# szpajder/dumphfdl

Measured on AMD Instinct MI355X. Metric: wideband I/Q Msamples/s (cf32 ingest -> decoded HFDL PDUs) at fixed channel count, higher is better.
Workload: dtype f32

## Files before the change

### dumphfdl_amd/csrc/fft_core.h

```cpp
#pragma once
#include "kernels.h"

namespace hfdl {

__device__ __forceinline__ float2 cmul(float2 a, float2 b)
{
	return make_float2(a.x * b.x - a.y * b.y, a.x * b.y + a.y * b.x);
}

template <int DIR, bool SKEW = false>
__device__ void lds_fft_columns(float2 *s, int R, int logR, int pitch, int log_cols, const float2 *tw)
{
	const int cols_mask = (1 << log_cols) - 1;
	int len = R, loglen = logR;
	while (len >= 4) {
		const int q = len >> 2, logq = loglen - 2;
		const int nb = (R >> 2) << log_cols;
		const int tstep = R >> loglen;
		for (int t = threadIdx.x; t < nb; t += blockDim.x) {
			const int col = t & cols_mask, b = t >> log_cols;
			const int j = b & (q - 1), blk = b >> logq;
			const int r0 = (blk << loglen) + j;
			float2 *p = s + (size_t)r0 * pitch + (SKEW ? 0 : col);
			const int qs = q * pitch;
			const int c0 = SKEW ? ((col + r0) & cols_mask) : 0, c1 = SKEW ? ((col + r0 + q) & cols_mask) : qs;
			const int c2 = SKEW ? (2 * qs + ((col + r0 + 2 * q) & cols_mask)) : 2 * qs, c3 = SKEW ? (3 * qs + ((col + r0 + 3 * q) & cols_mask)) : 3 * qs;
			const int c1s = SKEW ? qs + c1 : c1;
			float2 a = p[c0], bb = p[c1s], c = p[c2], d = p[c3];
			float2 w1 = tw[j * tstep], w2 = tw[2 * j * tstep], w3 = tw[3 * j * tstep];
			if (DIR > 0) { w1.y = -w1.y; w2.y = -w2.y; w3.y = -w3.y; }
			float2 apc = make_float2(a.x + c.x, a.y + c.y), amc = make_float2(a.x - c.x, a.y - c.y);
			float2 bpd = make_float2(bb.x + d.x, bb.y + d.y), bmd = make_float2(bb.x - d.x, bb.y - d.y);
			float2 jb = (DIR < 0) ? make_float2(bmd.y, -bmd.x) : make_float2(-bmd.y, bmd.x);
			float2 y0 = make_float2(apc.x + bpd.x, apc.y + bpd.y);
			float2 y2 = cmul(make_float2(apc.x - bpd.x, apc.y - bpd.y), w2);
			float2 y1 = cmul(make_float2(amc.x + jb.x, amc.y + jb.y), w1);
			float2 y3 = cmul(make_float2(amc.x - jb.x, amc.y - jb.y), w3);
			p[c0] = y0; p[c1s] = y2; p[c2] = y1; p[c3] = y3;
		}
		__syncthreads();
		len = q; loglen = logq;
	}
	if (len == 2) {
		const int nb = (R >> 1) << log_cols;
		for (int t = threadIdx.x; t < nb; t += blockDim.x) {
			const int col = t & cols_mask, b = t >> log_cols;
			float2 *p = s + (size_t)(2 * b) * pitch + (SKEW ? 0 : col);
			const int c0 = SKEW ? ((col + 2 * b) & cols_mask) : 0, c1 = pitch + (SKEW ? ((col + 2 * b + 1) & cols_mask) : 0);
			float2 a = p[c0], bb = p[c1];
			p[c0] = make_float2(a.x + bb.x, a.y + bb.y);
			p[c1] = make_float2(a.x - bb.x, a.y - bb.y);
		}
		__syncthreads();
	}
}

__device__ __forceinline__ int bitrev(int x, int bits) { return bits ? (int)(__brev((unsigned)x) >> (32 - bits)) : 0; }

__device__ __forceinline__ float2 unit_twiddle(unsigned e, int logn)
{
	float frac = (float)e * __builtin_ldexpf(1.0f, -logn + 1);
	float sn, cs;
	sincospif(-frac, &sn, &cs);
	return make_float2(cs, sn);
}

__device__ __forceinline__ void nco_phasor_step(float &cphi, float &sphi, float cd, float sd)
{
#pragma clang fp contract(off)
	const float c0 = cphi, s0 = sphi;
	cphi = c0 * cd - s0 * sd;
	sphi = s0 * cd + c0 * sd;
}

__device__ __forceinline__ float2 nco_phasor_seed(float starting_phase)
{
	return make_float2((float)cos((double)starting_phase), (float)sin((double)starting_phase));
}

__device__ __forceinline__ int nco_output_count(const NcoState &st, int input_size, int q)
{
	return st.decimation_remain < input_size ? (input_size - st.decimation_remain + q - 1) / q : 0;
}

__device__ __forceinline__ void nco_advance(NcoState &st, int cnt, int q, int input_size, float rate)
{
	const int last = st.decimation_remain + q * cnt;
	st.decimation_remain = last - input_size;
	const double phase = (double)st.starting_phase + (double)rate * M_PI * (double)cnt;
	float fp = (float)phase;
	while ((double)fp > M_PI) fp = (float)((double)fp - 2 * M_PI);
	while ((double)fp < -M_PI) fp = (float)((double)fp + 2 * M_PI);
	st.starting_phase = fp;
	st.output_size = cnt;
}

__device__ __forceinline__ void nco_table_segment(const NcoJob &job, int c)
{
	if (c >= job.nch) return;
	const ChanConst k = job.cc[c];
	NcoState st = job.chain[c];
	if (job.seg == 0) job.snap[c] = st;
	const int cnt = nco_output_count(st, job.post_input_size, job.post);
	const int per = (job.outs + job.nseg - 1) / job.nseg;
	const int i0 = job.seg * per, i1 = (job.seg + 1) * per < cnt ? (job.seg + 1) * per : cnt;
	float2 p = job.seg == 0 ? nco_phasor_seed(st.starting_phase) : job.cont[c];
	float2 *dst = job.ph + (size_t)i0 * job.nch + c;
	for (int i = i0; i < i1; i++, dst += job.nch) {
		*dst = p;
		nco_phasor_step(p.x, p.y, k.nco_cosdelta, k.nco_sindelta);
	}
	job.cont[c] = p;
	if (job.seg == job.nseg - 1) {
		nco_advance(st, cnt, job.post, job.post_input_size, k.nco_rate);
		job.chain[c] = st;
	}
}

}
```

### dumphfdl_amd/csrc/fft_kernels.hip

```cpp
#include <hip/hip_ext.h>
#include "kernels.h"
#include "retune_launch.h"
#include "fft_core.h"
#include "fft_regs.h"

namespace hfdl {

template <int FMT>
__device__ __forceinline__ float2 load_sample(const void *__restrict__ raw, int i)
{
	if (FMT == SFMT_CS16) {
		const short2 v = ((const short2 *)raw)[i];
		return make_float2((float)v.x / 32767.5f, (float)v.y / 32767.5f);
	} else if (FMT == SFMT_CU8) {
		const uchar2 v = ((const uchar2 *)raw)[i];
		return make_float2(((float)v.x - 63.5f) / 127.0f, ((float)v.y - 63.5f) / 127.0f);
	}
	return ((const float2 *)raw)[i];
}

__device__ __forceinline__ void store_out(float2 *out, const FftOutLayout &lay, unsigned i, size_t at, float2 v)
{
	if (lay.kind == TAPL_PLAIN) { out[at] = v; return; }
	float *o = (float *)out + tap_index_f(lay.kind, 1 << lay.row_log, (size_t)(2 * lay.row_stride), lay.chan, (int)(i >> lay.row_log), (int)(i & ((1u << lay.row_log) - 1u)), 0);
	o[0] = v.x;
	o[4] = v.y;
}

template <int FMT>
__global__ __launch_bounds__(FFT_THREADS) void fft_pass1(const float2 *__restrict__ hist, FftInputs in,
		int split, float2 *__restrict__ hist_next, float2 *__restrict__ out, FftPlan p, NcoJob job, int riders)
{
	if ((int)blockIdx.x < riders) { if (blockIdx.y == 0) nco_table_segment(job, (int)blockIdx.x * FFT_THREADS + (int)threadIdx.x); return; }
	const int bid = (int)blockIdx.x - riders;
	const int rx = (int)blockIdx.y;
	const void *__restrict__ fresh = in.fresh[rx];
	if (hist != nullptr) hist += rx * in.hist_stride;
	if (hist_next != nullptr) hist_next += rx * in.hist_stride;
	out += (size_t)rx * (size_t)p.n;
	extern __shared__ float2 sm[];
	const int cs = p.n >> p.l1;
	const int c0 = bid * FFT_TILE;
	const int total = p.r1 * FFT_TILE;
	for (int e = threadIdx.x; e < total; e += FFT_THREADS) {
		const int r = e >> FFT_TILE_LOG, col = e & (FFT_TILE - 1);
		const int c = c0 + col;
		float2 v = make_float2(0.f, 0.f);
		if (c < cs) {
			const int idx = r * cs + c;
			v = idx < split ? hist[idx] : load_sample<FMT>(fresh, idx - split);
			if (hist_next != nullptr && idx >= p.n - split) hist_next[idx - (p.n - split)] = v;
		}
		sm[e] = v;
	}
	float2 *ltw = sm + total;
	for (int t = threadIdx.x; t < p.r1; t += FFT_THREADS) ltw[t] = p.tw1[t];
	__syncthreads();
	lds_fft_columns<-1>(sm, p.r1, p.l1, FFT_TILE, FFT_TILE_LOG, ltw);
	for (int e = threadIdx.x; e < total; e += FFT_THREADS) {
		const int k1 = e >> FFT_TILE_LOG, col = e & (FFT_TILE - 1);
		const int c = c0 + col;
		if (c >= cs) continue;
		float2 v = sm[bitrev(k1, p.l1) * FFT_TILE + col];
		const unsigned ex = ((unsigned)k1 * (unsigned)c) & (unsigned)(p.n - 1);
		out[(size_t)k1 * cs + c] = cmul(v, unit_twiddle(ex, p.logn));
	}
}

__global__ __launch_bounds__(FFT_THREADS) void fft_pass2(float2 *__restrict__ buf, FftPlan p, NcoJob job, int riders)
{
	if ((int)blockIdx.x < riders) { if (blockIdx.y == 0) nco_table_segment(job, (int)blockIdx.x * FFT_THREADS + (int)threadIdx.x); return; }
	const int bid = (int)blockIdx.x - riders;
	buf += (size_t)blockIdx.y * (size_t)p.n;
	extern __shared__ float2 sm[];
	const int r23 = p.n >> p.l1, ncol = p.r1 * p.r3;
	const int cc0 = bid * FFT_TILE;
	const int total = p.r2 * FFT_TILE;
	for (int e = threadIdx.x; e < total; e += FFT_THREADS) {
		const int r = e >> FFT_TILE_LOG, col = e & (FFT_TILE - 1);
		const int cc = cc0 + col;
		float2 v = make_float2(0.f, 0.f);
		if (cc < ncol) {
			const int k1 = cc >> p.l3, n3 = cc & (p.r3 - 1);
			v = buf[(size_t)k1 * r23 + (size_t)r * p.r3 + n3];
		}
		sm[e] = v;
	}
	float2 *ltw = sm + total;
	for (int t = threadIdx.x; t < p.r2; t += FFT_THREADS) ltw[t] = p.tw2[t];
	__syncthreads();
	lds_fft_columns<-1>(sm, p.r2, p.l2, FFT_TILE, FFT_TILE_LOG, ltw);
	for (int e = threadIdx.x; e < total; e += FFT_THREADS) {
		const int k2 = e >> FFT_TILE_LOG, col = e & (FFT_TILE - 1);
		const int cc = cc0 + col;
		if (cc >= ncol) continue;
		const int k1 = cc >> p.l3, n3 = cc & (p.r3 - 1);
		float2 v = sm[bitrev(k2, p.l2) * FFT_TILE + col];
		const unsigned ex = ((unsigned)k2 * (unsigned)n3) & (unsigned)(r23 - 1);
		buf[(size_t)k1 * r23 + (size_t)k2 * p.r3 + n3] = cmul(v, unit_twiddle(ex, p.l2 + p.l3));
	}
}

__global__ __launch_bounds__(FFT_THREADS) void fft_pass3(const float2 *__restrict__ in, float2 *__restrict__ out, FftPlan p, int shifted,
		FftOutLayout lay, NcoJob job, int riders, int64_t out_rx_stride)
{
	if ((int)blockIdx.x < riders) { if (blockIdx.y == 0) nco_table_segment(job, (int)blockIdx.x * FFT_THREADS + (int)threadIdx.x); return; }
	const int bid = (int)blockIdx.x - riders;
	in += (size_t)blockIdx.y * (size_t)p.n;
	out += blockIdx.y * out_rx_stride;
	extern __shared__ float2 sm[];
	const int r23 = p.n >> p.l1, ncol = p.r1 * p.r2;
	const int cc0 = bid * FFT_TILE;
	const int total = p.r3 * FFT_TILE;
	for (int e = threadIdx.x; e < total; e += FFT_THREADS) {
		const int col = e >> p.l3, n3 = e & (p.r3 - 1);
		const int cc = cc0 + col;
		float2 v = make_float2(0.f, 0.f);
		if (cc < ncol) {
			const int k2 = cc >> p.l1, k1 = cc & (p.r1 - 1);
			v = in[(size_t)k1 * r23 + (size_t)k2 * p.r3 + n3];
		}
		sm[n3 * FFT_TILE + ((col + n3) & (FFT_TILE - 1))] = v;
	}
	float2 *ltw = sm + total;
	for (int t = threadIdx.x; t < p.r3; t += FFT_THREADS) ltw[t] = p.tw3[t];
	__syncthreads();
	lds_fft_columns<-1, true>(sm, p.r3, p.l3, FFT_TILE, FFT_TILE_LOG, ltw);
	const unsigned half = shifted ? (unsigned)(p.n >> 1) : 0u;
	for (int e = threadIdx.x; e < total; e += FFT_THREADS) {
		const int k3 = e >> FFT_TILE_LOG, col = e & (FFT_TILE - 1);
		const int cc = cc0 + col;
		if (cc >= ncol) continue;
		const int k2 = cc >> p.l1, k1 = cc & (p.r1 - 1);
		const unsigned k = (unsigned)k1 + ((unsigned)k2 << p.l1) + ((unsigned)k3 << (p.l1 + p.l2));
		const unsigned i = (k + half) & (unsigned)(p.n - 1);
		const size_t at = lay.row_log ? (size_t)(i >> lay.row_log) * (size_t)lay.row_stride + (i & ((1u << lay.row_log) - 1u)) : (size_t)i;
		const int r = bitrev(k3, p.l3);
		store_out(out, lay, i, at, sm[r * FFT_TILE + ((col + r) & (FFT_TILE - 1))]);
	}
}


template <int B, int FMT, bool AHEAD>
__global__ __launch_bounds__(16 * B) void fft_rpass1(const float2 *__restrict__ hist, FftInputs in,
		int split, float2 *__restrict__ hist_next, float2 *__restrict__ out, FftPlan p, NcoJob job, int riders, int tpw)
{
	constexpr int NT = 16 * B;
	if ((int)blockIdx.x < riders) { if (blockIdx.y == 0) nco_table_segment(job, (int)blockIdx.x * NT + (int)threadIdx.x); return; }
	const int rx = (int)blockIdx.y;
	const void *__restrict__ fresh = in.fresh[rx];
	if (hist != nullptr) hist += rx * in.hist_stride;
	if (hist_next != nullptr) hist_next += rx * in.hist_stride;
	out += (size_t)rx * (size_t)p.n;
	__shared__ float2 ex[B * FR_PITCH];
	__shared__ float2 ltw[16 * B];
	const int bid = ((int)blockIdx.x - riders) * tpw, tid = (int)threadIdx.x;
	const int cs = p.n >> p.l1;
	const int col = tid & 15, n2 = tid >> 4;
	float2 x[16], xn[16];
	auto load = [&](float2 (&v)[16], int tile) {
		const int c = tile * 16 + col;
#pragma unroll
		for (int n1 = 0; n1 < 16; n1++) {
			const int idx = (n2 + B * n1) * cs + c;
			v[n1] = idx < split ? hist[idx] : load_sample<FMT>(fresh, idx - split);
		}
	};
	load(x, bid);
	ltw[tid] = p.tw1[tid];
	for (int t = 0; t < (AHEAD ? tpw : 1); t++) {
		const int tile = bid + t;
		if (AHEAD && t + 1 < tpw) load(xn, tile + 1);
		if (hist_next != nullptr) {
			const int c = tile * 16 + col;
#pragma unroll
			for (int n1 = 0; n1 < 16; n1++) {
				const int idx = (n2 + B * n1) * cs + c;
				if (idx >= p.n - split) hist_next[idx - (p.n - split)] = x[n1];
			}
		}
		__syncthreads();
		stage_a(x, ex, ltw, n2, col);
		__syncthreads();
#pragma unroll
		for (int i = 0; i < 256 / NT; i++) {
			const int tt = tid + i * NT, tcol = tt & 15, k1 = tt >> 4, tc = tile * 16 + tcol;
			float2 z[B], w[B];
			stage_b<B>(z, ex, k1, tcol);
			twiddle_run<B>(w, (unsigned)k1 * (unsigned)tc, 16u * (unsigned)tc, p.logn);
#pragma unroll
			for (int k2 = 0; k2 < B; k2++) out[(size_t)(k1 + 16 * k2) * cs + tc] = cmul(z[slot_small<B>(k2)], w[k2]);
		}
		if (AHEAD) {
#pragma unroll
			for (int n1 = 0; n1 < 16; n1++) x[n1] = xn[n1];
		}
	}
}

template <int B, bool AHEAD>
__global__ __launch_bounds__(16 * B) void fft_rpass2(float2 *__restrict__ buf, FftPlan p, NcoJob job, int riders, int tpw)
{
	constexpr int NT = 16 * B;
	if ((int)blockIdx.x < riders) { if (blockIdx.y == 0) nco_table_segment(job, (int)blockIdx.x * NT + (int)threadIdx.x); return; }
	buf += (size_t)blockIdx.y * (size_t)p.n;
	__shared__ float2 ex[B * FR_PITCH];
	__shared__ float2 ltw[16 * B];
	const int bid = ((int)blockIdx.x - riders) * tpw, tid = (int)threadIdx.x;
	const int r23 = p.n >> p.l1;
	const int col = tid & 15, n2 = tid >> 4;
	auto base_of = [&](int tile) {
		const int cc0 = tile * 16;
		return buf + (size_t)(cc0 >> p.l3) * r23 + (cc0 & (p.r3 - 1));
	};
	float2 x[16], xn[16];
	auto load = [&](float2 (&v)[16], int tile) {
		const float2 *base = base_of(tile);
#pragma unroll
		for (int n1 = 0; n1 < 16; n1++) v[n1] = base[(size_t)(n2 + B * n1) * p.r3 + col];
	};
	load(x, bid);
	ltw[tid] = p.tw2[tid];
	for (int t = 0; t < (AHEAD ? tpw : 1); t++) {
		const int tile = bid + t;
		if (AHEAD && t + 1 < tpw) load(xn, tile + 1);
		float2 *base = base_of(tile);
		const int n30 = (tile * 16) & (p.r3 - 1);
		__syncthreads();
		stage_a(x, ex, ltw, n2, col);
		__syncthreads();
#pragma unroll
		for (int i = 0; i < 256 / NT; i++) {
			const int tt = tid + i * NT, tcol = tt & 15, k1 = tt >> 4, n3 = n30 + tcol;
			float2 z[B], w[B];
			stage_b<B>(z, ex, k1, tcol);
			twiddle_run<B>(w, (unsigned)k1 * (unsigned)n3, 16u * (unsigned)n3, p.l2 + p.l3);
#pragma unroll
			for (int k2 = 0; k2 < B; k2++) base[(size_t)(k1 + 16 * k2) * p.r3 + tcol] = cmul(z[slot_small<B>(k2)], w[k2]);
		}
		if (AHEAD) {
#pragma unroll
			for (int n1 = 0; n1 < 16; n1++) x[n1] = xn[n1];
		}
	}
}

template <int B>
__global__ __launch_bounds__(16 * B) void fft_rpass3(const float2 *__restrict__ in, float2 *__restrict__ out, FftPlan p, int shifted,
		FftOutLayout lay, NcoJob job, int riders, int tpw, int64_t out_rx_stride)
{
	constexpr int NT = 16 * B, R = 16 * B;
	if ((int)blockIdx.x < riders) { if (blockIdx.y == 0) nco_table_segment(job, (int)blockIdx.x * NT + (int)threadIdx.x); return; }
	in += (size_t)blockIdx.y * (size_t)p.n;
	out += blockIdx.y * out_rx_stride;
	__shared__ float2 ex[B * FR_PITCH];
	__shared__ float2 ltw[16 * B];
	const int bid = ((int)blockIdx.x - riders) * tpw, tid = (int)threadIdx.x;
	const int r23 = p.n >> p.l1;
	const int col = tid & 15, n2 = tid >> 4;
	float2 pre[16], pn[16];
	auto load = [&](float2 (&v)[16], int tile) {
		const int cc0 = tile * 16;
		const float2 *src = in + (size_t)(cc0 >> p.l1) * R + (size_t)(cc0 & (p.r1 - 1)) * r23;
#pragma unroll
		for (int i = 0; i < 16; i++) {
			const int e = tid + i * NT;
			v[i] = src[(size_t)(e / R) * r23 + (e % R)];
		}
	};
	load(pre, bid);
	ltw[tid] = p.tw3[tid];
	const unsigned half = shifted ? (unsigned)(p.n >> 1) : 0u;
	for (int t = 0; t < tpw; t++) {
		const int tile = bid + t;
		const int k2g = (tile * 16) >> p.l1, k10 = (tile * 16) & (p.r1 - 1);
		__syncthreads();
#pragma unroll
		for (int i = 0; i < 16; i++) {
			const int e = tid + i * NT, tcol = e / R, n3 = e % R;
			ex[n3 * 16 + ((tcol + n3) & 15)] = pre[i];
		}
		if (t + 1 < tpw) load(pn, tile + 1);
		__syncthreads();
		float2 x[16];
#pragma unroll
		for (int n1 = 0; n1 < 16; n1++) {
			const int r = n2 + B * n1;
			x[n1] = ex[r * 16 + ((col + r) & 15)];
		}
		__syncthreads();
		stage_a(x, ex, ltw, n2, col);
		__syncthreads();
#pragma unroll
		for (int i = 0; i < 256 / NT; i++) {
			const int tt = tid + i * NT, tcol = tt & 15, ka = tt >> 4;
			float2 z[B];
			stage_b<B>(z, ex, ka, tcol);
			const unsigned kbase = (unsigned)(k10 + tcol) + ((unsigned)k2g << p.l1);
#pragma unroll
			for (int kb = 0; kb < B; kb++) {
				const unsigned k = kbase + ((unsigned)(ka + 16 * kb) << (p.l1 + p.l2));
				const unsigned i2 = (k + half) & (unsigned)(p.n - 1);
				const size_t at = lay.row_log ? (size_t)(i2 >> lay.row_log) * (size_t)lay.row_stride + (i2 & ((1u << lay.row_log) - 1u)) : (size_t)i2;
				store_out(out, lay, i2, at, z[slot_small<B>(kb)]);
			}
		}
#pragma unroll
		for (int i = 0; i < 16; i++) pre[i] = pn[i];
	}
}

template <int B>
static void launch_rpass1(int fmt, dim3 grid, hipStream_t st, hipEvent_t start, hipEvent_t input_read, const float2 *hist, const FftInputs &in, int split, float2 *hist_next,
		float2 *work, const FftPlan &p, const NcoJob &nco, int riders, int tpw)
{
	const dim3 blk(16 * B);
	if (fmt == SFMT_CS16) hipExtLaunchKernelGGL((fft_rpass1<B, SFMT_CS16, false>), grid, blk, 0, st, start, input_read, 0, hist, in, split, hist_next, work, p, nco, riders, tpw);
	else if (fmt == SFMT_CU8) hipExtLaunchKernelGGL((fft_rpass1<B, SFMT_CU8, false>), grid, blk, 0, st, start, input_read, 0, hist, in, split, hist_next, work, p, nco, riders, tpw);
	else hipExtLaunchKernelGGL((fft_rpass1<B, SFMT_CF32, false>), grid, blk, 0, st, start, input_read, 0, hist, in, split, hist_next, work, p, nco, riders, tpw);
}

__global__ void retune_channelizer_kernel(ChanConst *cc, NcoState *chain, float2 *cont, int c, ChanConst k)
{
	if (blockIdx.x != 0 || threadIdx.x != 0) return;
	cc[c] = k;
	chain[c] = NcoState{ 0, 0.f, 0, 0 };
	cont[c] = make_float2(0.f, 0.f);
}

void launch_retune_channelizer(ChanConst *cc, NcoState *chain, float2 *cont, int c, const ChanConst &k, hipStream_t st, hipEvent_t done)
{
	hipExtLaunchKernelGGL(retune_channelizer_kernel, dim3(1), dim3(64), 0, st, nullptr, done, 0, cc, chain, cont, c, k);
}

static bool fast_plan(const FftPlan &p) { return p.l1 >= 6 && p.l1 <= 8 && p.l2 >= 6 && p.l2 <= 8 && p.l3 >= 6 && p.l3 <= 8; }

void launch_fft_forward(const FftPlan &p, const float2 *hist, const FftInputs &in, int fmt, int split, float2 *hist_next,
		float2 *work, float2 *out, bool shifted, hipStream_t st, FftOutLayout lay, hipEvent_t done, NcoJob nco, hipEvent_t input_read, hipEvent_t start)
{
	const unsigned nrx = (unsigned)in.nrx;
	const int64_t ors = in.out_stride;
	const int c1 = (p.n >> p.l1), c2 = p.r1 * p.r3, c3 = p.r1 * p.r2;
	const int g1 = (c1 + FFT_TILE - 1) / FFT_TILE, g2 = (c2 + FFT_TILE - 1) / FFT_TILE, g3 = (c3 + FFT_TILE - 1) / FFT_TILE;
	nco.nseg = 3;
	if (fast_plan(p)) {
		auto riders_of = [&](int l) { const int nt = 1 << l; return nco.cc ? (nco.nch + nt - 1) / nt : 0; };
		const int rd1 = riders_of(p.l1), rd2 = riders_of(p.l2), rd3 = riders_of(p.l3);
		auto tpw_of = [](int tiles) { return tiles % 4 == 0 && tiles >= 4096 ? 4 : tiles % 2 == 0 && tiles >= 1024 ? 2 : 1; };
		const int t1 = 1, t2 = 1, t3 = tpw_of(g3);
		nco.seg = 0;
		switch (p.l1) {
		case 6: launch_rpass1<4>(fmt, dim3(g1 / t1 + rd1, nrx), st, start, input_read, hist, in, split, hist_next, work, p, nco, rd1, t1); break;
		case 7: launch_rpass1<8>(fmt, dim3(g1 / t1 + rd1, nrx), st, start, input_read, hist, in, split, hist_next, work, p, nco, rd1, t1); break;
		default: launch_rpass1<16>(fmt, dim3(g1 / t1 + rd1, nrx), st, start, input_read, hist, in, split, hist_next, work, p, nco, rd1, t1); break;
		}
		nco.seg = 1;
		switch (p.l2) {
		case 6: hipLaunchKernelGGL((fft_rpass2<4, false>), dim3(g2 / t2 + rd2, nrx), dim3(64), 0, st, work, p, nco, rd2, t2); break;
		case 7: hipLaunchKernelGGL((fft_rpass2<8, false>), dim3(g2 / t2 + rd2, nrx), dim3(128), 0, st, work, p, nco, rd2, t2); break;
		default: hipLaunchKernelGGL((fft_rpass2<16, false>), dim3(g2 / t2 + rd2, nrx), dim3(256), 0, st, work, p, nco, rd2, t2); break;
		}
		nco.seg = 2;
		switch (p.l3) {
		case 6: hipExtLaunchKernelGGL(fft_rpass3<4>, dim3(g3 / t3 + rd3, nrx), dim3(64), 0, st, nullptr, done, 0, (const float2 *)work, out, p, shifted ? 1 : 0, lay, nco, rd3, t3, ors); break;
		case 7: hipExtLaunchKernelGGL(fft_rpass3<8>, dim3(g3 / t3 + rd3, nrx), dim3(128), 0, st, nullptr, done, 0, (const float2 *)work, out, p, shifted ? 1 : 0, lay, nco, rd3, t3, ors); break;
		default: hipExtLaunchKernelGGL(fft_rpass3<16>, dim3(g3 / t3 + rd3, nrx), dim3(256), 0, st, nullptr, done, 0, (const float2 *)work, out, p, shifted ? 1 : 0, lay, nco, rd3, t3, ors); break;
		}
		return;
	}
	const int riders = nco.cc ? (nco.nch + FFT_THREADS - 1) / FFT_THREADS : 0;
	const dim3 blk(FFT_THREADS);
	const size_t l1 = (size_t)p.r1 * (FFT_TILE + 1) * sizeof(float2), l2 = (size_t)p.r2 * (FFT_TILE + 1) * sizeof(float2);
	nco.seg = 0;
	if (fmt == SFMT_CS16) hipExtLaunchKernelGGL(fft_pass1<SFMT_CS16>, dim3(g1 + riders, nrx), blk, l1, st, start, input_read, 0, hist, in, split, hist_next, work, p, nco, riders);
	else if (fmt == SFMT_CU8) hipExtLaunchKernelGGL(fft_pass1<SFMT_CU8>, dim3(g1 + riders, nrx), blk, l1, st, start, input_read, 0, hist, in, split, hist_next, work, p, nco, riders);
	else hipExtLaunchKernelGGL(fft_pass1<SFMT_CF32>, dim3(g1 + riders, nrx), blk, l1, st, start, input_read, 0, hist, in, split, hist_next, work, p, nco, riders);
	nco.seg = 1;
	hipLaunchKernelGGL(fft_pass2, dim3(g2 + riders, nrx), blk, l2, st, work, p, nco, riders);
	nco.seg = 2;
	hipExtLaunchKernelGGL(fft_pass3, dim3(g3 + riders, nrx), blk, (size_t)p.r3 * (FFT_TILE + 1) * sizeof(float2), st, nullptr, done, 0,
			(const float2 *)work, out, p, shifted ? 1 : 0, lay, nco, riders, ors);
}

}
```

### dumphfdl_amd/csrc/fft_regs.h

```cpp
#pragma once
#include "kernels.h"
#include "fft_core.h"

namespace hfdl {

constexpr int FR_PITCH = 16 * 16 + 16;

__device__ __forceinline__ float2 cadd(float2 a, float2 b) { return make_float2(a.x + b.x, a.y + b.y); }
__device__ __forceinline__ float2 csub(float2 a, float2 b) { return make_float2(a.x - b.x, a.y - b.y); }
__device__ __forceinline__ float2 mul_mj(float2 a) { return make_float2(a.y, -a.x); }

__device__ __forceinline__ void dft4(float2 &a, float2 &b, float2 &c, float2 &d)
{
	const float2 t0 = cadd(a, c), t1 = csub(a, c), t2 = cadd(b, d), t3 = mul_mj(csub(b, d));
	a = cadd(t0, t2); c = csub(t0, t2);
	b = cadd(t1, t3); d = csub(t1, t3);
}

__device__ __forceinline__ void dft16(float2 (&x)[16])
{
	constexpr float C1 = 0.92387953251128674f, S1 = 0.38268343236508977f, H = 0.70710678118654752f;
#pragma unroll
	for (int b = 0; b < 4; b++) dft4(x[b], x[4 + b], x[8 + b], x[12 + b]);
	x[5] = cmul(x[5], make_float2(C1, -S1));  x[6] = cmul(x[6], make_float2(H, -H));    x[7] = cmul(x[7], make_float2(S1, -C1));
	x[9] = cmul(x[9], make_float2(H, -H));    x[10] = mul_mj(x[10]);                     x[11] = cmul(x[11], make_float2(-H, -H));
	x[13] = cmul(x[13], make_float2(S1, -C1)); x[14] = cmul(x[14], make_float2(-H, -H)); x[15] = cmul(x[15], make_float2(-C1, S1));
#pragma unroll
	for (int c = 0; c < 4; c++) dft4(x[4 * c], x[4 * c + 1], x[4 * c + 2], x[4 * c + 3]);
}
__device__ __forceinline__ constexpr int slot16(int k) { return 4 * (k & 3) + (k >> 2); }

__device__ __forceinline__ void dft8(float2 (&x)[8])
{
	constexpr float H = 0.70710678118654752f;
#pragma unroll
	for (int b = 0; b < 4; b++) { const float2 s = cadd(x[b], x[4 + b]), d = csub(x[b], x[4 + b]); x[b] = s; x[4 + b] = d; }
	x[5] = cmul(x[5], make_float2(H, -H)); x[6] = mul_mj(x[6]); x[7] = cmul(x[7], make_float2(-H, -H));
	dft4(x[0], x[1], x[2], x[3]);
	dft4(x[4], x[5], x[6], x[7]);
}
__device__ __forceinline__ constexpr int slot8(int k) { return 4 * (k & 1) + (k >> 1); }

template <int B> __device__ __forceinline__ void dft_small(float2 (&z)[B])
{
	if constexpr (B == 16) dft16(z);
	else if constexpr (B == 8) dft8(z);
	else { static_assert(B == 4, "B = 4, 8 or 16"); dft4(z[0], z[1], z[2], z[3]); }
}
template <int B> __device__ __forceinline__ constexpr int slot_small(int k) { return B == 16 ? slot16(k) : B == 8 ? slot8(k) : k; }

__device__ __forceinline__ void stage_a(float2 (&x)[16], float2 *ex, const float2 *ltw, int n2, int col)
{
	dft16(x);
	float2 *dst = ex + n2 * FR_PITCH + col;
	dst[0] = x[0];
#pragma unroll
	for (int k1 = 1; k1 < 16; k1++) dst[k1 * 16] = cmul(x[slot16(k1)], ltw[n2 * k1]);
}

template <int B> __device__ __forceinline__ void stage_b(float2 (&z)[B], const float2 *ex, int k1, int col)
{
	const float2 *src = ex + k1 * 16 + col;
#pragma unroll
	for (int n2 = 0; n2 < B; n2++) z[n2] = src[n2 * FR_PITCH];
	dft_small<B>(z);
}

template <int B> __device__ __forceinline__ void twiddle_run(float2 (&w)[B], unsigned e0, unsigned es, int logn)
{
	const unsigned mask = (1u << logn) - 1u;
	const float2 base = unit_twiddle(e0 & mask, logn), s1 = unit_twiddle(es & mask, logn);
	const float2 s2 = cmul(s1, s1), s3 = cmul(s2, s1);
	float2 s4 = make_float2(1.f, 0.f);
	if constexpr (B > 4) s4 = unit_twiddle((4u * es) & mask, logn);
	float2 q = base;
#pragma unroll
	for (int g = 0; g < B / 4; g++) {
		if (g > 0) q = cmul(q, s4);
		w[4 * g] = q; w[4 * g + 1] = cmul(q, s1); w[4 * g + 2] = cmul(q, s2); w[4 * g + 3] = cmul(q, s3);
	}
}

}
```

### dumphfdl_amd/csrc/fold_kernels.hip

```cpp
#include <hip/hip_ext.h>
#include <type_traits>
#include "kernels.h"
#include "fft_core.h"

namespace hfdl {

constexpr int FOLD_THREADS = 256;

typedef float v4f __attribute__((ext_vector_type(4)));
typedef float v2f __attribute__((ext_vector_type(2)));


__device__ __forceinline__ float2 tap_at(const float *taps, size_t row_stride_f, int m, int layout, int c, int row, int j)
{
	const float *p = taps + tap_index_f(layout, m, row_stride_f, c, row, j, 0);
	return make_float2(p[0], p[layout == TAPL_PLAIN ? 1 : 4]);
}

__device__ __forceinline__ void cmac_quad(float2 &a, const float2 *h, const float2 *x, int n)
{
	for (int k = 0; k < n; k++) { a.x = __builtin_fmaf(h[k].x, x[k].x, a.x); a.y = __builtin_fmaf(h[k].y, x[k].x, a.y); }
	for (int k = 0; k < n; k++) { a.x = __builtin_fmaf(-h[k].y, x[k].y, a.x); a.y = __builtin_fmaf(h[k].x, x[k].y, a.y); }
}

__device__ __forceinline__ int rx_of_channel(const int4 *__restrict__ rx_tab, int nrx, int c)
{
	int r = 0;
	while (r + 1 < nrx && c >= rx_tab[r + 1].z) r++;
	return r;
}

__global__ __launch_bounds__(FOLD_THREADS) void fold_ref_kernel(const float *__restrict__ taps, const float2 *__restrict__ spec, float2 *__restrict__ partial,
		size_t row_stride_f, size_t spec_stride, size_t partial_stride, int m, int slices, int rows, int layout, int nb,
		const int4 *__restrict__ rx_tab, int nrx, size_t spec_rx_stride)
{
	const int s = blockIdx.x % slices, c = blockIdx.x / slices;
	const int rxi = rx_of_channel(rx_tab, nrx, c);
	const int4 rt = rx_tab[rxi];
	const int slot = rt.x + (c - rt.z);
	spec += (size_t)rxi * spec_rx_stride;
	for (int b0 = 0; b0 < nb; b0 += 4)
		for (int j = threadIdx.x; j < m; j += FOLD_THREADS) {
			const float2 *sp = spec + (size_t)b0 * spec_stride + (size_t)s * rows * (size_t)m + j;
			float2 acc[4] = { make_float2(0.f, 0.f), make_float2(0.f, 0.f), make_float2(0.f, 0.f), make_float2(0.f, 0.f) };
			for (int r = 0; r < rows; r += 4) {
				const int n = rows - r < 4 ? rows - r : 4;
				float2 h[4], x[4];
				for (int k = 0; k < n; k++) h[k] = tap_at(taps, row_stride_f, m, layout, slot, s * rows + r + k, j);
#pragma unroll
				for (int b = 0; b < 4; b++)
					if (b0 + b < nb) {
						for (int k = 0; k < n; k++) x[k] = sp[(size_t)b * spec_stride + (size_t)(r + k) * m];
						cmac_quad(acc[b], h, x, n);
					}
			}
#pragma unroll
			for (int k = 0; k < 4; k++)
				if (b0 + k < nb) partial[(size_t)(b0 + k) * partial_stride + ((size_t)c * slices + s) * (size_t)m + j] = acc[k];
		}
}

__device__ __forceinline__ float rot90(float a, int sign_mask)
{
	const int v = __builtin_amdgcn_update_dpp(0, __float_as_int(a), 0xB1, 0xF, 0xF, true);
	return __int_as_float(v ^ sign_mask);
}

#ifdef HFDL_LAB
__device__ unsigned long long hfdl_fold_clk_probe[1024 * 4];
__device__ unsigned hfdl_fold_clk_probe_n;
#endif

constexpr int fold16_waves(int p, int w, int d, bool small = false, int cg = 1)
{
	const int loads = 8 * cg, mine = w >= loads ? 1 : loads / w;
	const int regs = (small ? 16 : 64) * p * cg + 16 * p * d + 4 * mine * d + 4 * mine + 8 + 28;
	if (small) return regs <= 168 ? 2 : 1;
	if (cg > 1) return 1;
	return regs <= 96 ? 5 : regs <= 128 ? 4 : regs <= 168 ? 3 : regs <= 256 ? 2 : 1;
}

template <int P, int W, int D, bool WIN = false, bool SMALL = false, int CG = 1>
__device__ __forceinline__ void fold_mfma16_body(
		const float *__restrict__ taps, const float2 *__restrict__ spec, float2 *__restrict__ partial,
		size_t row_stride_f, size_t spec_stride, size_t partial_stride, int m, int slices, int rows, int nb,
		const int2 *__restrict__ win, const int4 *__restrict__ grp_tab, size_t spec_rx_stride)
{
	static_assert(!WIN || W == 1, "windows are per wave: no spectrum tile is shared");
	static_assert(D == 2 || D == 4, "the LDS stage of a trip is a compile-time constant for even D");
	static_assert(CG == 1 || (CG == 2 && !SMALL && !WIN), "two column groups: the sixteen-column instruction, every row");
#ifdef HFDL_LAB
	unsigned long long clk_c0 = 0, clk_r0 = 0;
	const bool clk_me = blockIdx.x == gridDim.x / 2 && threadIdx.x == 0;
	if (clk_me) { clk_c0 = __builtin_amdgcn_s_memtime(); clk_r0 = __builtin_amdgcn_s_memrealtime(); }
#endif
	constexpr int NLOADS = 8 * CG;
	constexpr int MINE = W >= NLOADS ? 1 : NLOADS / W;
	constexpr int XPITCH = 64 * CG + 1;
	__shared__ v4f xt[2][8][XPITCH];
	const int ngrp = m >> 4;
	const int ntile = ngrp * slices, groups = (int)gridDim.x / ntile;
	int tile_id, grp;
	if ((ntile & 7) == 0) {
		const int xcd = (int)blockIdx.x & 7, i = (int)blockIdx.x >> 3;
		grp = i % groups;
		tile_id = (i / groups) * 8 + xcd;
	} else {
		tile_id = (int)blockIdx.x % ntile;
		grp = (int)blockIdx.x / ntile;
	}
	const int g = tile_id % ngrp, s = tile_id / ngrp;
	const int wave = __builtin_amdgcn_readfirstlane((int)(threadIdx.x >> 6)), lane = (int)(threadIdx.x & 63);
	const int n = lane & 15, k = lane >> 4;
	const int4 ge = grp_tab[grp];
	const int octet0 = __builtin_amdgcn_readfirstlane(ge.x) + wave * P;
	const int slot_end = __builtin_amdgcn_readfirstlane(ge.z), to_chan = __builtin_amdgcn_readfirstlane(ge.w);
	spec += (size_t)__builtin_amdgcn_readfirstlane(ge.y) * spec_rx_stride;
	const int sign_mask = (lane & 1) ? 0 : (int)0x80000000;
	const int quads = rows >> 2;
	int next_quad = 0, trips = quads;
	if constexpr (WIN) {
		const int2 wn = win[octet0 / P];
		next_quad = __builtin_amdgcn_readfirstlane(wn.x);
		trips = __builtin_amdgcn_readfirstlane(wn.y);
	}
	const char *tb = (const char *)(taps + (size_t)s * rows * row_stride_f + (size_t)octet0 * 64 * m + (size_t)g * 1024) + lane * 16;
	const size_t qs_b = row_stride_f * 16, os_b = (size_t)m * 256, xquad_b = (size_t)m * 32;
	const char *xp[MINE], *xp0[MINE];
	int xseg[MINE];
#pragma unroll
	for (int i = 0; i < MINE; i++) {
		const int item = (((wave * MINE) % NLOADS) + i) * 64 + lane, seg = item >> 3, part = item & 7;
		const int sn = (seg & 15) + 16 * (seg >> 6), sk = (seg >> 4) & 3;
		const int bi = sn < nb ? sn : nb - 1;
		xp[i] = xp0[i] = (const char *)(spec + (size_t)bi * spec_stride + ((size_t)s * rows + sk) * (size_t)m + g * 16 + 2 * part);
		xseg[i] = part * XPITCH + seg;
	}
	const char *const tb0 = tb;
	constexpr int NACC = SMALL ? 4 : 16;
	v4f acc[P * CG][NACC];
#pragma unroll
	for (int p = 0; p < P * CG; p++)
#pragma unroll
		for (int j = 0; j < NACC; j++) acc[p][j] = v4f{ 0.f, 0.f, 0.f, 0.f };
	v4f h[D][P][4];
	v4f xs[D][MINE];
	auto issue = [&](int slot) {
		if constexpr (WIN) {
			tb = tb0 + (size_t)next_quad * qs_b;
#pragma unroll
			for (int i = 0; i < MINE; i++) xp[i] = xp0[i] + (size_t)next_quad * xquad_b;
			next_quad = next_quad + 1 == quads ? 0 : next_quad + 1;
		}
#pragma unroll
		for (int i = 0; i < MINE; i++) xs[slot][i] = *(const v4f *)xp[i];
#pragma unroll
		for (int p = 0; p < P; p++)
#pragma unroll
			for (int q = 0; q < 4; q++) h[slot][p][q] = __builtin_nontemporal_load((const v4f *)(tb + (size_t)p * os_b + 1024 * q));
		if constexpr (!WIN) {
#pragma unroll
			for (int i = 0; i < MINE; i++) xp[i] += xquad_b;
			tb += qs_b;
		}
	};
	auto stash = [&](int slot, int stage) {
#pragma unroll
		for (int i = 0; i < MINE; i++) (&xt[stage][0][0])[xseg[i]] = xs[slot][i];
	};
	auto multiply = [&](int slot, int stage) {
		if constexpr (SMALL) {
			const float *xl = (const float *)&xt[stage][0][0] + (size_t)((k >> 1) * XPITCH + (lane & 3)) * 4 + 2 * (k & 1);
#pragma unroll
			for (int q = 0; q < 4; q++) {
				v2f x[4];
#pragma unroll
				for (int kk = 0; kk < 4; kk++) x[kk] = *(const v2f *)(xl + (size_t)(2 * q * XPITCH + 16 * kk) * 4);
#pragma unroll
				for (int p = 0; p < P; p++) {
					typedef unsigned v2u __attribute__((ext_vector_type(2)));
					const v4f hv = h[slot][p][q];
					const v2u a02 = __builtin_amdgcn_permlane32_swap(__float_as_uint(hv[0]), __float_as_uint(hv[2]), false, false);
					const v2u a13 = __builtin_amdgcn_permlane32_swap(__float_as_uint(hv[1]), __float_as_uint(hv[3]), false, false);
					const v2u t01 = __builtin_amdgcn_permlane16_swap(a02[0], a13[0], false, false);
					const v2u t23 = __builtin_amdgcn_permlane16_swap(a02[1], a13[1], false, false);
					const float t[4] = { __uint_as_float(t01[0]), __uint_as_float(t01[1]), __uint_as_float(t23[0]), __uint_as_float(t23[1]) };
#pragma unroll
					for (int kk = 0; kk < 4; kk++) acc[p][q] = __builtin_amdgcn_mfma_f32_4x4x1f32(t[kk], x[kk].x, acc[p][q], 0, 0, 0);
#pragma unroll
					for (int kk = 0; kk < 4; kk++) acc[p][q] = __builtin_amdgcn_mfma_f32_4x4x1f32(rot90(t[kk], sign_mask), x[kk].y, acc[p][q], 0, 0, 0);
				}
			}
			return;
		}
#pragma unroll
		for (int b = 0; b < 8; b++) {
			v4f x[CG];
#pragma unroll
			for (int cg = 0; cg < CG; cg++) x[cg] = xt[stage][b][64 * cg + lane];
#pragma unroll
			for (int p = 0; p < P; p++)
#pragma unroll
				for (int cg = 0; cg < CG; cg++) {
					v4f *a = acc[p * CG + cg];
					a[2 * b] = __builtin_amdgcn_mfma_f32_16x16x4f32(h[slot][p][b >> 1][(2 * b) & 3], x[cg][0], a[2 * b], 0, 0, 0);
					a[2 * b + 1] = __builtin_amdgcn_mfma_f32_16x16x4f32(h[slot][p][b >> 1][(2 * b + 1) & 3], x[cg][2], a[2 * b + 1], 0, 0, 0);
				}
#pragma unroll
			for (int p = 0; p < P; p++) {
				const float r0 = rot90(h[slot][p][b >> 1][(2 * b) & 3], sign_mask), r1 = rot90(h[slot][p][b >> 1][(2 * b + 1) & 3], sign_mask);
#pragma unroll
				for (int cg = 0; cg < CG; cg++) {
					v4f *a = acc[p * CG + cg];
					a[2 * b] = __builtin_amdgcn_mfma_f32_16x16x4f32(r0, x[cg][1], a[2 * b], 0, 0, 0);
					a[2 * b + 1] = __builtin_amdgcn_mfma_f32_16x16x4f32(r1, x[cg][3], a[2 * b + 1], 0, 0, 0);
				}
			}
		}
	};
#pragma unroll
	for (int d = 0; d < D; d++) {
		issue(d);
		__builtin_amdgcn_sched_barrier(0);
	}
	stash(0, 0);
	__syncthreads();
	for (int r = 0; r < trips - D; r += D) {
#pragma unroll
		for (int d = 0; d < D; d++) {
			multiply(d, d & 1);
			issue(d);
			stash((d + 1) % D, (d + 1) & 1);
			__builtin_amdgcn_sched_barrier(0);
			__syncthreads();
		}
	}
#pragma unroll
	for (int d = 0; d < D; d++) {
		multiply(d, d & 1);
		if (d + 1 < D) {
			stash(d + 1, (d + 1) & 1);
			__builtin_amdgcn_sched_barrier(0);
			__syncthreads();
		}
	}
	if constexpr (SMALL) {
		const int j = lane & 3, cpq = (lane >> 2) & 3;
		if (j < nb) {
#pragma unroll
			for (int p = 0; p < P; p++)
#pragma unroll
				for (int cp = 0; cp < 2; cp++) {
					const int sl = 8 * (octet0 + p) + 2 * cpq + cp;
					if (sl >= slot_end) continue;
					const int c = sl + to_chan;
					float2 *po = partial + (size_t)j * partial_stride + ((size_t)c * slices + s) * (size_t)m + g * 16 + k;
#pragma unroll
					for (int q = 0; q < 4; q++) po[4 * q] = make_float2(acc[p][q][2 * cp], acc[p][q][2 * cp + 1]);
				}
		}
	} else
	{
#pragma unroll
		for (int cg = 0; cg < CG; cg++) {
			const int blk = 16 * cg + n;
			if (blk >= nb) continue;
#pragma unroll
			for (int p = 0; p < P; p++)
#pragma unroll
				for (int cp = 0; cp < 2; cp++) {
					const int sl = 8 * (octet0 + p) + 2 * k + cp;
					if (sl >= slot_end) continue;
					const int c = sl + to_chan;
					const v4f *a = acc[p * CG + cg];
					float2 *po = partial + (size_t)blk * partial_stride + ((size_t)c * slices + s) * (size_t)m + g * 16;
#pragma unroll
					for (int j = 0; j < 16; j += 2)
						*(v4f *)(po + j) = v4f{ a[j][2 * cp], a[j][2 * cp + 1], a[j + 1][2 * cp], a[j + 1][2 * cp + 1] };
				}
		}
	}
#ifdef HFDL_LAB
	if (clk_me) {
		const unsigned slot = atomicAdd(&hfdl_fold_clk_probe_n, 1u) & 1023u;
		hfdl_fold_clk_probe[4 * slot] = (SMALL ? 4ull : 16ull * CG) * 100ull + (unsigned long long)nb;
		hfdl_fold_clk_probe[4 * slot + 1] = __builtin_amdgcn_s_memtime() - clk_c0;
		hfdl_fold_clk_probe[4 * slot + 2] = __builtin_amdgcn_s_memrealtime() - clk_r0;
		hfdl_fold_clk_probe[4 * slot + 3] = clk_r0;
	}
#endif
}

template <int P, int W, int D, bool WIN = false, bool SMALL = false, int CG = 1>
__global__ __launch_bounds__(64 * W) __attribute__((amdgpu_waves_per_eu(fold16_waves(P, W, D, SMALL, CG), fold16_waves(P, W, D, SMALL, CG)))) void fold_mfma16_kernel(
		const float *__restrict__ taps, const float2 *__restrict__ spec, float2 *__restrict__ partial,
		size_t row_stride_f, size_t spec_stride, size_t partial_stride, int m, int slices, int rows, int nb,
		const int2 *__restrict__ win, const int4 *__restrict__ grp_tab, size_t spec_rx_stride)
{
	fold_mfma16_body<P, W, D, WIN, SMALL, CG>(taps, spec, partial, row_stride_f, spec_stride, partial_stride, m, slices, rows, nb, win, grp_tab, spec_rx_stride);
}

#ifdef HFDL_LAB
__global__ __launch_bounds__(512) __attribute__((amdgpu_waves_per_eu(2, 2))) __attribute__((amdgpu_num_vgpr(104))) void fold32_two_waves_kernel(
		const float *__restrict__ taps, const float2 *__restrict__ spec, float2 *__restrict__ partial,
		size_t row_stride_f, size_t spec_stride, size_t partial_stride, int m, int slices, int rows, int nb,
		const int2 *__restrict__ win, const int4 *__restrict__ grp_tab, size_t spec_rx_stride)
{
	fold_mfma16_body<1, 8, 2, false, false, 2>(taps, spec, partial, row_stride_f, spec_stride, partial_stride, m, slices, rows, nb, win, grp_tab, spec_rx_stride);
}
#endif

#ifdef HFDL_LAB
template <int L, bool SPAN>
__global__ __launch_bounds__(FOLD_THREADS) void stream_read_kernel(const float4 *__restrict__ src, size_t chunks, float *__restrict__ sink)
{
	float acc = 0.f;
	const size_t per_block = chunks / gridDim.x;
	const size_t first = SPAN ? (size_t)blockIdx.x * per_block : blockIdx.x, step = SPAN ? 1 : gridDim.x;
	const size_t last = SPAN ? first + per_block : chunks;
	for (size_t ch = first; ch < last; ch += step) {
		const v4f *p = (const v4f *)src + ch * (L * FOLD_THREADS) + threadIdx.x;
		v4f v[L];
#pragma unroll
		for (int i = 0; i < L; i++) v[i] = __builtin_nontemporal_load(p + i * FOLD_THREADS);
#pragma unroll
		for (int i = 0; i < L; i++) acc += v[i].x + v[i].w;
	}
	if (acc == 1.2345e33f) *sink = acc;
}

hipError_t fold_clock_probe_ring(ClockProbeRing &r)
{
	r.len = 1024;
	const hipError_t e = hipGetSymbolAddress((void **)&r.records, HIP_SYMBOL(hfdl_fold_clk_probe));
	return e != hipSuccess ? e : hipGetSymbolAddress((void **)&r.count, HIP_SYMBOL(hfdl_fold_clk_probe_n));
}

int stream_read_variants() { return 4; }

void launch_stream_read(int variant, const float2 *src, size_t bytes, float *sink, hipStream_t st)
{
	const dim3 block(FOLD_THREADS);
	switch (variant) {
	case 0: hipLaunchKernelGGL((stream_read_kernel<4, false>), dim3(2048), block, 0, st, (const float4 *)src, bytes / (64 * FOLD_THREADS), sink); break;
	case 1: hipLaunchKernelGGL((stream_read_kernel<8, false>), dim3(2048), block, 0, st, (const float4 *)src, bytes / (128 * FOLD_THREADS), sink); break;
	case 2: hipLaunchKernelGGL((stream_read_kernel<4, true>), dim3((unsigned)(bytes >> 22)), block, 0, st, (const float4 *)src, bytes / (64 * FOLD_THREADS), sink); break;
	default: hipLaunchKernelGGL((stream_read_kernel<8, true>), dim3((unsigned)(bytes >> 22)), block, 0, st, (const float4 *)src, bytes / (128 * FOLD_THREADS), sink); break;
	}
}
#endif

struct FoldArgs {
	const float *taps;
	const float2 *spec;
	float2 *partial;
	size_t rs_f, ss, ps;
	int m, slices, rows, nch, ngroups, nb;
	const int4 *grp_tab, *rx_host;
	int nrx;
	size_t spec_rx_stride;
	void split(int pw, int &groups, int &rest) const
	{
		groups = rest = 0;
		for (int r = 0; r < nrx; r++) { const int noct = rx_host[r].y >> 3; groups += noct / pw; rest += noct % pw; }
	}
	const int4 *table(int pw) const { return grp_tab + (size_t)(pw - 1) * (size_t)(ngroups); }
	hipStream_t st;
	hipEvent_t start, stop;
};

template <int P, int W, int D, bool SMALL = false, int CG = 1>
static int fold16_go(const FoldArgs &a)
{
	static_assert(P * W <= FOLD_GROUP_MAX, "the group tables of the front end go up to FOLD_GROUP_MAX octets per workgroup");
	const int ntile = (a.m >> 4) * a.slices;
	int groups, rest;
	a.split(P * W, groups, rest);
	int launches = 0;
	if (groups > 0) {
		hipExtLaunchKernelGGL((fold_mfma16_kernel<P, W, D, false, SMALL, CG>), dim3((unsigned)(groups * ntile)), dim3(64 * W), 0, a.st, a.start, rest ? nullptr : a.stop, 0,
			a.taps, a.spec, a.partial, a.rs_f, a.ss, a.ps, a.m, a.slices, a.rows, a.nb, (const int2 *)nullptr, a.table(P * W), a.spec_rx_stride);
		launches++;
	}
	if (rest > 0) {
		constexpr int DR = CG > 1 ? 2 : D;
		hipExtLaunchKernelGGL((fold_mfma16_kernel<1, 1, DR, false, SMALL, CG>), dim3((unsigned)(rest * ntile)), dim3(64), 0, a.st, groups > 0 ? nullptr : a.start, a.stop, 0,
			a.taps, a.spec, a.partial, a.rs_f, a.ss, a.ps, a.m, a.slices, a.rows, a.nb, (const int2 *)nullptr, a.table(P * W) + groups, a.spec_rx_stride);
		launches++;
	}
	return launches;
}

#ifdef HFDL_LAB
static int fold32_two_waves_go(const FoldArgs &a)
{
	const int ntile = (a.m >> 4) * a.slices;
	int groups, rest;
	a.split(8, groups, rest);
	int launches = 0;
	if (groups > 0) {
		hipExtLaunchKernelGGL(fold32_two_waves_kernel, dim3((unsigned)(groups * ntile)), dim3(512), 0, a.st, a.start, rest ? nullptr : a.stop, 0,
			a.taps, a.spec, a.partial, a.rs_f, a.ss, a.ps, a.m, a.slices, a.rows, a.nb, (const int2 *)nullptr, a.table(8), a.spec_rx_stride);
		launches++;
	}
	if (rest > 0) {
		hipExtLaunchKernelGGL((fold_mfma16_kernel<1, 1, 2, false, false, 2>), dim3((unsigned)(rest * ntile)), dim3(64), 0, a.st, groups > 0 ? nullptr : a.start, a.stop, 0,
			a.taps, a.spec, a.partial, a.rs_f, a.ss, a.ps, a.m, a.slices, a.rows, a.nb, (const int2 *)nullptr, a.table(8) + groups, a.spec_rx_stride);
		launches++;
	}
	return launches;
}
#endif

template <int D>
static int fold16_go_win(const FoldArgs &a, const int2 *win)
{
	const int ntile = a.m >> 4;
	hipExtLaunchKernelGGL((fold_mfma16_kernel<1, 1, D, true>), dim3((unsigned)(a.ngroups * ntile)), dim3(64), 0, a.st, a.start, a.stop, 0,
		a.taps, a.spec, a.partial, a.rs_f, a.ss, a.ps, a.m, 1, a.rows, a.nb, win, a.table(1), a.spec_rx_stride);
	return 1;
}

struct FoldVariant { int layout, p, q, w, d; int (*go)(const FoldArgs &); };
#define F16(P, W, D) { TAPL_OCTET, P, 4, W, D, fold16_go<P, W, D> }
#define F4(P, W, D) { TAPL_OCTET, P, 1, W, D, fold16_go<P, W, D, true> }
#define F32(P, W, D) { TAPL_OCTET, P, 8, W, D, fold16_go<P, W, D, false, 2> }
static const FoldVariant fold_variants[] = {
	F16(2, 4, 4), F16(2, 4, 2),
	F4(2, 4, 2),
	F32(1, 4, 4), F32(1, 4, 2),
#ifdef HFDL_LAB
	F32(1, 8, 2), F32(1, 8, 4), F32(1, 2, 2), F32(2, 4, 2),
	F4(2, 4, 4), F4(4, 4, 2), F4(1, 8, 4), F4(2, 8, 2), F4(2, 8, 4), F4(4, 2, 2), F4(1, 4, 4),
	F16(1, 4, 2), F16(1, 4, 4), F16(1, 8, 2), F16(1, 8, 4), F16(2, 2, 2), F16(2, 8, 2), F16(1, 2, 2), F16(1, 2, 4), F16(3, 4, 2),
	{ TAPL_OCTET, 1, 8, 8, 2, fold32_two_waves_go },
#endif
};
#undef F32
#undef F4
#undef F16
constexpr int N_FOLD_VARIANTS = (int)(sizeof(fold_variants) / sizeof(fold_variants[0]));

int fold_variant_count() { return N_FOLD_VARIANTS; }

int fold_variant_describe(int v, int desc[6])
{
	if (v < 0 || v >= N_FOLD_VARIANTS) return -1;
	const FoldVariant &f = fold_variants[v];
	desc[0] = f.p; desc[1] = f.q; desc[2] = f.w; desc[3] = f.d; desc[4] = 4 * f.q; desc[5] = f.layout;
	return 0;
}

static bool variant_fits(const FoldVariant &f, const Geometry &g)
{
	return g.tap_layout == f.layout && (g.rows_per_slice & 3) == 0 && (g.rows_per_slice >> 2) % f.d == 0;
}

static const FoldVariant *pick_variant(const Geometry &g, int nb)
{
	if (g.fold_tile >= 0 && g.fold_tile < N_FOLD_VARIANTS && 4 * fold_variants[g.fold_tile].q >= nb && variant_fits(fold_variants[g.fold_tile], g)) return &fold_variants[g.fold_tile];
	for (const FoldVariant &f : fold_variants)
		if (nb <= 4 && f.q == 1 && variant_fits(f, g)) return &f;
	for (const FoldVariant &f : fold_variants)
		if (f.q == (nb <= 16 ? 4 : 8) && variant_fits(f, g)) return &f;
	return nullptr;
}

int fold_launch_blocks(const Geometry &g, int remaining, int nb_max)
{
	int take = remaining < nb_max ? remaining : nb_max;
	if (take > FOLD_MAX_BLOCKS) take = FOLD_MAX_BLOCKS;
	if (take > 16 && g.fold_win && g.tap_layout == TAPL_OCTET) take = 16;
	if (take > 16 && take <= 20) take = 16;
	if (take > 16 && !pick_variant(g, take)) take = 16;
	return take;
}

static FoldArgs fold_args(const Geometry &g, const float2 *taps, const float2 *spectrum, size_t spec_stride, float2 *partial, size_t partial_stride,
		int nb, hipStream_t st, hipEvent_t start, hipEvent_t stop)
{
	FoldArgs a;
	a.taps = (const float *)taps; a.spec = spectrum; a.partial = partial;
	a.rs_f = (size_t)g.tap_row_stride * 2; a.ss = spec_stride; a.ps = partial_stride;
	a.m = g.m; a.slices = g.slices; a.rows = g.rows_per_slice; a.nch = g.nch; a.ngroups = g.nch_pad / tap_layout_group(g.tap_layout); a.nb = nb;
	a.grp_tab = g.grp_tab; a.rx_host = g.rx_host; a.nrx = g.nrx; a.spec_rx_stride = (size_t)g.spec_rx_stride;
	a.st = st; a.start = start; a.stop = stop;
	return a;
}

static void launch_fold_ref(const Geometry &g, const float2 *taps, const float2 *spectrum, size_t spec_stride, float2 *partial, size_t partial_stride,
		int nb, hipStream_t st, hipEvent_t start, hipEvent_t stop)
{
	hipExtLaunchKernelGGL(fold_ref_kernel, dim3((unsigned)(g.nch * g.slices)), dim3(FOLD_THREADS), 0, st, start, stop, 0,
		(const float *)taps, spectrum, partial, (size_t)g.tap_row_stride * 2, spec_stride, partial_stride, g.m, g.slices, g.rows_per_slice, g.tap_layout, nb,
		g.rx_tab, g.nrx, (size_t)g.spec_rx_stride);
}

int launch_fold_variant(int v, const Geometry &g, const float2 *taps, const float2 *spectrum, size_t spec_stride, float2 *partial,
		size_t partial_stride, int nb, hipStream_t st, hipEvent_t start, hipEvent_t stop)
{
	if (v == -1) { launch_fold_ref(g, taps, spectrum, spec_stride, partial, partial_stride, nb, st, start, stop); return 1; }
	if (v < 0 || v >= N_FOLD_VARIANTS || !variant_fits(fold_variants[v], g) || nb < 1 || nb > 4 * fold_variants[v].q) return -1;
	return fold_variants[v].go(fold_args(g, taps, spectrum, spec_stride, partial, partial_stride, nb, st, start, stop));
}

int launch_fold(const Geometry &g, const float2 *taps, const float2 *spectrum, size_t spec_stride, float2 *partial, size_t partial_stride,
		int nb, hipStream_t st, hipEvent_t start, hipEvent_t stop)
{
	if (nb < 1 || nb > fold_launch_blocks(g, nb, FOLD_MAX_BLOCKS)) return -1;
	const FoldArgs a = fold_args(g, taps, spectrum, spec_stride, partial, partial_stride, nb, st, start, stop);
	if (g.fold_win && g.tap_layout == TAPL_OCTET) return fold16_go_win<2>(a, g.fold_win);
	if (const FoldVariant *f = pick_variant(g, nb)) return f->go(a);
	launch_fold_ref(g, taps, spectrum, spec_stride, partial, partial_stride, nb, st, start, stop);
	return 1;
}

__global__ __launch_bounds__(FOLD_THREADS) void tap_row_energy_kernel(const float *__restrict__ taps, float *__restrict__ energy, size_t row_stride_f, int m, int noct, int nch_pad)
{
	const int oct = blockIdx.x % noct, quad = blockIdx.x / noct;
	const v4f *base = (const v4f *)(taps + (size_t)quad * 4 * row_stride_f + (size_t)oct * 64 * m);
	float acc = 0.f;
	for (int e = threadIdx.x; e < (m >> 2) * 64; e += FOLD_THREADS) {
		const v4f v = base[e];
		acc += v.x * v.x + v.y * v.y + v.z * v.z + v.w * v.w;
	}
	const int lane = threadIdx.x & 63;
	atomicAdd(energy + (size_t)(4 * quad + (lane >> 4)) * nch_pad + oct * 8 + ((lane & 15) >> 1), acc);
}

void launch_tap_row_energy(const float2 *taps, const Geometry &g, float *energy, hipStream_t st)
{
	const int noct = g.nch_pad / 8;
	hipLaunchKernelGGL(tap_row_energy_kernel, dim3((unsigned)((g.pre >> 2) * noct)), dim3(FOLD_THREADS), 0, st, (const float *)taps, energy, (size_t)g.tap_row_stride * 2, g.m, noct, g.nch_pad);
}

__global__ __launch_bounds__(FOLD_THREADS) void tap_extract_kernel(const float *__restrict__ taps, float2 *__restrict__ dst, size_t row_stride_f, int m, int pre, int layout, int c)
{
	const size_t n = (size_t)m * pre;
	for (size_t e = (size_t)blockIdx.x * FOLD_THREADS + threadIdx.x; e < n; e += (size_t)gridDim.x * FOLD_THREADS)
		dst[e] = tap_at(taps, row_stride_f, m, layout, c, (int)(e / m), (int)(e % m));
}

void launch_tap_extract(const float2 *taps, const Geometry &g, int slot, float2 *dst, hipStream_t st)
{
	hipLaunchKernelGGL(tap_extract_kernel, dim3(1024), dim3(FOLD_THREADS), 0, st, (const float *)taps, dst, (size_t)g.tap_row_stride * 2, g.m, g.pre, g.tap_layout, slot);
}

constexpr int IFFT_THREADS = 1024;

__device__ __forceinline__ void nco_phasor_run(float2 *ph, int cnt, float starting_phase, float cd, float sd)
{
	float2 p = nco_phasor_seed(starting_phase);
	for (int i = 0; i < cnt; i++) {
		ph[i] = p;
		nco_phasor_step(p.x, p.y, cd, sd);
	}
}

__device__ __forceinline__ float2 nco_rotate(float2 p, float2 v)
{
#pragma clang fp contract(off)
	const float re = p.x * v.x - p.y * v.y, im = p.y * v.x + p.x * v.y;
	return make_float2(re, im);
}

__global__ __launch_bounds__(IFFT_THREADS) void ifft_nco_kernel(const float2 *__restrict__ partial, size_t partial_stride, const ChanConst *__restrict__ cc,
		const NcoState *__restrict__ snap, const float2 *__restrict__ ph, size_t ph_stride, const float2 *__restrict__ tw, float2 *__restrict__ chan_out,
		int *__restrict__ out_count, Geometry g, int logm)
{
	extern __shared__ float2 sm[];
	const int c = blockIdx.x % g.nch, b = blockIdx.x / g.nch;
	const ChanConst k = cc[c];
	const int m = g.m, mask = m - 1;
	const NcoState st = snap[(size_t)b * g.nch + c];
	const int q = g.post;
	const int cnt = nco_output_count(st, g.post_input_size, q);
	{
		const int h0 = (int)(((long long)g.n - k.offsetbin + m / 2) % m);
		const float2 *pc = partial + (size_t)b * partial_stride + (size_t)c * g.slices * (size_t)m;
		for (int u = threadIdx.x; u < m; u += IFFT_THREADS) {
			const int j = (u - h0 - m / 2) & mask;
			float2 acc = make_float2(0.f, 0.f);
			for (int s = 0; s < g.slices; s++) {
				float2 v = pc[(size_t)s * m + j];
				acc.x += v.x; acc.y += v.y;
			}
			sm[u] = acc;
		}
	}
	__syncthreads();
	lds_fft_columns<+1>(sm, m, logm, 1, 0, tw);

	const float norm = (float)g.pre * (float)m;
	float2 *o = chan_out + ((size_t)b * g.nch + c) * g.outs;
	const float2 *phb = ph + (size_t)b * ph_stride;
	for (int i = threadIdx.x; i < cnt; i += IFFT_THREADS) {
		const int idx = g.scrap + st.decimation_remain + q * i;
		float2 v = sm[(int)(__brev((unsigned)idx) >> (32 - logm))];
		v.x = __fdiv_rn(v.x, norm); v.y = __fdiv_rn(v.y, norm);
		o[i] = nco_rotate(phb[(size_t)i * g.nch + c], v);
	}
	if (threadIdx.x == 0) out_count[(size_t)b * g.nch + c] = cnt;
}

__global__ __launch_bounds__(IFFT_THREADS) void nco_decimate_kernel(const float2 *__restrict__ in, int input_size, float cd, float sd, float rate,
		int q, NcoState *__restrict__ state, float2 *__restrict__ ph, float2 *__restrict__ out)
{
	NcoState st = *state;
	const int cnt = nco_output_count(st, input_size, q);
	if (threadIdx.x == 0) nco_phasor_run(ph, cnt, st.starting_phase, cd, sd);
	__syncthreads();
	for (int i = threadIdx.x; i < cnt; i += IFFT_THREADS) out[i] = nco_rotate(ph[i], in[st.decimation_remain + q * i]);
	__syncthreads();
	if (threadIdx.x == 0) {
		nco_advance(st, cnt, q, input_size, rate);
		*state = st;
	}
}

void launch_nco_decimate(const float2 *in, int input_size, float cd, float sd, float rate, int q, NcoState *state, float2 *ph, float2 *out, hipStream_t st)
{
	hipLaunchKernelGGL(nco_decimate_kernel, dim3(1), dim3(IFFT_THREADS), 0, st, in, input_size, cd, sd, rate, q, state, ph, out);
}

hipError_t prepare_ifft_nco(int m)
{
	const size_t lds = sizeof(float2) * ((size_t)m + 1);
	if (lds <= 64 * 1024) return hipSuccess;
	return hipFuncSetAttribute((const void *)ifft_nco_kernel, hipFuncAttributeMaxDynamicSharedMemorySize, (int)lds);
}

void launch_ifft_nco(const Geometry &g, const float2 *partial, size_t partial_stride, const ChanConst *cc, const NcoState *snap, const float2 *ph,
		size_t ph_stride, const float2 *tw_m, float2 *chan_out, int *out_count, int nb, hipStream_t st, hipEvent_t done, hipEvent_t start)
{
	int logm = 0;
	while ((1 << logm) < g.m) logm++;
	size_t lds = sizeof(float2) * ((size_t)g.m + 1);
	hipExtLaunchKernelGGL(ifft_nco_kernel, dim3((unsigned)(g.nch * nb)), dim3(IFFT_THREADS), (unsigned)lds, st, start, done, 0, partial, partial_stride, cc, snap, ph, ph_stride,
			tw_m, chan_out, out_count, g, logm);
}

}
```

### dumphfdl_amd/csrc/frontend.h

```cpp
#pragma once
#include <hip/hip_runtime.h>
#include <complex>
#include <deque>
#include <memory>
#include <vector>
#include "../../include/hfdl_gpu.h"
#include "hip_handles.h"
#include "kernels.h"
#include "planner.h"
#include "retune_launch.h"
#include "launch_timers.h"
#include "demod.h"
#include "spectrum.h"
#include "export_ring.h"
#include "blanker.h"
#include "notch.h"

namespace hfdl {

int select_device(int device);
int check_channel_span(int32_t sample_rate, int32_t nrx, int c, int32_t freq, int r, int32_t centre);
long env_long(const char *name, long lo, long hi, long otherwise);
inline int ilog2(int x) { int l = 0; while ((1 << l) < x) l++; return l; }
inline size_t sample_bytes(int fmt) { return fmt == SFMT_CS16 ? 4 : fmt == SFMT_CU8 ? 2 : 8; }
bool is_library_pinned(const void *p, size_t bytes);

struct LabConfig {
	int fold_tile = -1;
	int fold_slices = 0;
	int cu_split = 0;
	bool cu_partition = false;
	int fft_stream = -1;
	bool decode_stream = true;
	int fold_bound = -1;
	bool fold_ramp = true;
};
LabConfig read_lab_config();

struct HostFftPlan {
	FftPlan p{};
	DevBuf tw[3];
	int build(int n);
};
int upload_twiddles(int r, DevBuf &out);

int finish_stage();
struct StageFrames {
	DevBuf frames, data, scrambler;
	int upload(const float *symbols, const int32_t *modes, const int32_t *bitmask_lsb, int32_t nframes);
};


struct SpectrumHistory {
	static constexpr int CHUNK = 8;
	int rows = 0, interval = 0;
	DevBuf acc, peak;
	PinnedBuf<float> host;
	std::vector<Event> ev;
	std::vector<hfdl_gpu_spectrum_row> info;
	uint64_t open = 0;
	uint64_t open_first = 0;
	uint32_t open_blocks = 0;
	uint64_t oldest() const { const uint64_t kept = (uint64_t)rows - (open_blocks ? 1 : 0); return open > kept ? open - kept : 0; }
	void close()
	{
		info[open % (uint64_t)rows] = hfdl_gpu_spectrum_row{ open, open_first, open_blocks, 0 };
		open++;
		open_blocks = 0;
	}
};

struct SpectrumMonitor {
	int bins = 0;
	uint32_t flags = 0;
	DevBuf acc;
	DevBuf peak;
	PinnedBuf<float> host;
	Event ev;
	hipEvent_t last = nullptr;
	hipEvent_t newest() const { return last ? last : ev.e; }
	uint64_t fresh = 0;
	std::vector<uint64_t> blocks, first;
	std::unique_ptr<SpectrumHistory> hist;
};

struct ChannelExport {
	int nsel = 0, format = 0;
	float scale = 1.f;
	ExportRing ring;
	DevBuf channels;
	DevBuf samples, counts, power, clipped;
	size_t chunk = 1;
	PinnedBuf<char> host;
	std::vector<Event> ev;
	std::vector<uint64_t> last_of;
	hipEvent_t newest = nullptr;
};

struct Blanker {
	float k2 = 0.f;
	DevBuf scratch;
	DevBuf partial;
	DevBuf rec;
	PinnedBuf<BlankRecord> host;
	Event ev;
	uint64_t blocks = 0;
};

struct Notch {
	float mu = 0.f;
	int nsel = 0;
	std::vector<bool> selected;
	DevBuf out;
	DevBuf sel;
	DevBuf state;
	DevBuf rec;
	PinnedBuf<NotchRecord> host;
	PinnedBuf<int32_t> host_sel;
	Event staged;
	bool staging = false;
	Event ev;
	bool launched = false;
};

struct Retune {
	DevBuf pad, work;
	PinnedBuf<float2> stage[2];
	Event staged[2];
	DoneEvent done;
	uint64_t calls = 0;
	std::vector<float> lp;
	float lp_cut = -1.f;
};

}

bool design_channel(const hfdl_gpu_frontend *fe, int rx, int32_t freq, hfdl::ChanConst &k, std::complex<float> *taps, std::vector<float> &lp, float &lp_cut);

struct hfdl_gpu_frontend {
	int device = 0;
	hfdl::Stream stream;
	hfdl::Stream stream_b;
	hfdl::Stream stream_d;
	hfdl::Stream stream_c;
	hfdl::Stream stream_f;
	bool cu_partitioned = false;
	bool own_decode_stream() const { return stream_d.owned; }
	hfdl::FftRule fft_rule = hfdl::FFT_RULE_INPUT;
	hfdl::FftOrder order;
	int side_of(bool on_device) const { return hfdl::fft_side(fft_rule, on_device); }
	hipStream_t fft_stream(int side) const { return side == hfdl::FFT_SERIAL ? stream.s : stream_f.owned ? stream_f.s : stream_c.s; }
	static constexpr int MAX_HALF = hfdl::FOLD_MAX_BLOCKS;
	static constexpr int MAX_STAGE = HFDL_GPU_PREFETCH_MAX + 1;
	static_assert(MAX_HALF == hfdl::PLAN_MAX_HALF && MAX_STAGE == hfdl::PLAN_MAX_STAGE && HFDL_GPU_FOLD_BATCH_MAX == MAX_HALF, "include/hfdl_gpu.h, kernels.h and planner.h name the same limits");

	std::deque<hfdl::DevBuf> mem;
	template <typename T> hipError_t alloc(T *&view, size_t count)
	{
		mem.emplace_back();
		const hipError_t e = mem.back().alloc(sizeof(T) * count);
		view = mem.back().as<T>();
		return e;
	}
	hfdl::HostFftPlan fft;
	hfdl::Demod demod;
	int4 *d_rx = nullptr, *d_grp = nullptr;
	float2 *d_hist[2] = { nullptr, nullptr }, *d_work = nullptr, *d_spec = nullptr, *d_taps = nullptr, *d_partial = nullptr;
	float2 *d_tw_m = nullptr;
	int n_stage = 0;
	std::unique_ptr<hfdl::DevBuf> d_stage[MAX_STAGE];
	size_t stage_cap[MAX_STAGE] = {};
	float2 *d_chan_all = nullptr;
	int *d_cnt_all = nullptr;
	hfdl::ChanConst *d_cc = nullptr;
	int2 *d_win = nullptr;
	hfdl::NcoState *d_nco = nullptr;
	hfdl::NcoState *d_nco_snap = nullptr;
	float2 *d_ph = nullptr, *d_ph_cont = nullptr;
	std::unique_ptr<hfdl::SpectrumMonitor> mon;
	std::unique_ptr<hfdl::ChannelExport> exp;
	std::unique_ptr<hfdl::Retune> retune;
	std::unique_ptr<hfdl::Blanker> blank;
	std::unique_ptr<hfdl::Notch> notch;

	hfdl::DoneEvent chan[2];
	hfdl::DoneEvent fft_done;
	hfdl::DoneEvent spec[2];
	hfdl::Event ev_switch;
	hfdl::Event ev_stage_ready[MAX_STAGE];
	hfdl::Event ev_stage_free[MAX_STAGE];
	hfdl::LaunchTimers timers;
	int settle_events();

	uint64_t host_blocks = 0;
	uint64_t host_pushed = 0;
	const void *pf_ptr[MAX_STAGE] = {};
	int pf_fmt[MAX_STAGE] = {};
	hipEvent_t input_event(uint64_t host_block) const
	{
		const uint64_t newest = host_blocks - 1, span = (uint64_t)n_stage - 1;
		return ev_stage_ready[(newest - host_block <= span ? host_block : newest - span) % (uint64_t)n_stage];
	}
	int32_t sample_rate = 0, decimation = 0;
	float tbw = 0;
	hfdl::Plan plan{};
	hfdl::Geometry geo{};
	std::vector<int32_t> freqs;
	int nrx = 1;
	std::vector<int32_t> rx_center;
	std::vector<int32_t> rx_of;
	std::vector<hfdl::RxSpan> rx_span;
	std::vector<int4> rx_host;
	int slot_of(int c) const { return hfdl::receiver_slot(rx_span[(size_t)rx_of[(size_t)c]], c); }
	std::vector<hfdl::ChanConst> cc;
	int batch = 1;
	int fold_nb = 1;
	int half_blocks = 1;
	int half_first = 1, half_target = 1;
	int cur_half = 0, batch_fill = 0;
	int last_slot = 0;
	int last_index = 0;
	float2 *chan_slot(int slot) const { return d_chan_all + (size_t)slot * (size_t)geo.nch * (size_t)geo.outs; }
	int *cnt_slot(int slot) const { return d_cnt_all + (size_t)slot * (size_t)geo.nch; }
	int last_set = 0;
	float2 *spec_slot(int set, int i) const { return d_spec + ((size_t)set * (size_t)half_blocks + (size_t)i) * spec_stride(); }
	size_t spec_stride() const { return (size_t)nrx * (size_t)geo.n; }
	float2 *ph_slot(int set, int i) const { return d_ph + ((size_t)set * (size_t)half_blocks + (size_t)i) * ph_stride(); }
	hfdl::NcoState *snap_slot(int set, int i) const { return d_nco_snap + ((size_t)set * (size_t)half_blocks + (size_t)i) * (size_t)geo.nch; }
	size_t partial_stride() const { return (size_t)geo.nch * (size_t)geo.slices * (size_t)geo.m; }
	size_t ph_stride() const { return (size_t)geo.nch * (size_t)geo.outs; }
	double prune_tol = 0.0;
	int fold_rows_max = 0;
	bool fold_bound = false;
	uint64_t blocks = 0;
	hfdl::FftOutLayout tap_layout;
	int pending_demod_buf = -1;
	int pending_demod_nblk = 0;

	~hfdl_gpu_frontend();
};
```

### dumphfdl_amd/csrc/frontend_create.cpp

```cpp
#include <atomic>
#include <cmath>
#include <complex>
#include <cstring>
#include <thread>
#include "frontend.h"

using namespace hfdl;

extern "C" int hfdl_gpu_device_count(void)
{
	int n = 0;
	if (hipGetDeviceCount(&n) != hipSuccess) return 0;
	return n;
}

int hfdl::select_device(int device)
{
	int n = 0;
	if (hipGetDeviceCount(&n) != hipSuccess || n <= 0)
		return fail(HFDL_GPU_ENODEV, "no HIP device visible: the HFDL front end has no CPU fallback");
	if (device < 0 || device >= n) return fail(HFDL_GPU_EINVAL, "device %d out of range (%d visible)", device, n);
	HIP_TRY(hipSetDevice(device));
	hipDeviceProp_t prop;
	HIP_TRY(hipGetDeviceProperties(&prop, device));
	if (strncmp(prop.gcnArchName, "gfx950", 6) != 0)
		return fail(HFDL_GPU_ENODEV, "device %d is %s; this library carries gfx950 code only", device, prop.gcnArchName);
	return 0;
}


int hfdl::upload_twiddles(int r, DevBuf &out)
{
	std::vector<float2> h((size_t)r);
	for (int t = 0; t < r; t++) {
		double a = -2.0 * M_PI * (double)t / (double)r;
		h[t] = make_float2((float)std::cos(a), (float)std::sin(a));
	}
	HIP_TRY(out.alloc(sizeof(float2) * (size_t)r));
	HIP_TRY(hipMemcpy(out.p, h.data(), sizeof(float2) * (size_t)r, hipMemcpyHostToDevice));
	return 0;
}

int HostFftPlan::build(int n)
{
	int logn = ilog2(n);
	if ((1 << logn) != n || logn < 9 || logn > 24) return fail(HFDL_GPU_ERANGE, "fft size %d unsupported (need 2^9..2^24)", n);
	int l1 = (logn + 2) / 3, l2 = (logn - l1 + 1) / 2, l3 = logn - l1 - l2;
	p.n = n; p.logn = logn;
	p.l1 = l1; p.l2 = l2; p.l3 = l3;
	p.r1 = 1 << l1; p.r2 = 1 << l2; p.r3 = 1 << l3;
	const int radix[3] = { p.r1, p.r2, p.r3 };
	for (int i = 0; i < 3; i++) if (int rc = upload_twiddles(radix[i], tw[i])) return rc;
	p.tw1 = tw[0].as<float2>(); p.tw2 = tw[1].as<float2>(); p.tw3 = tw[2].as<float2>();
	return 0;
}


long hfdl::env_long(const char *name, long lo, long hi, long otherwise)
{
	const char *e = getenv(name);
	if (!e || !*e) return otherwise;
	char *end = nullptr;
	const long v = strtol(e, &end, 10);
	return (end != e && v >= lo && v <= hi) ? v : otherwise;
}

static double env_double(const char *name, double lo, double hi, double otherwise)
{
	const char *e = getenv(name);
	if (!e || !*e) return otherwise;
	char *end = nullptr;
	const double v = strtod(e, &end);
	return (end != e && v >= lo && v <= hi) ? v : otherwise;
}

static int build_fold_windows(hfdl_gpu_frontend *fe)
{
	Geometry &g = fe->geo;
	DevBuf d_en;
	std::vector<float> en((size_t)g.pre * (size_t)g.nch_pad);
	HIP_TRY(d_en.alloc(sizeof(float) * en.size()));
	HIP_TRY(hipMemsetAsync(d_en.p, 0, sizeof(float) * en.size(), fe->stream));
	launch_tap_row_energy(fe->d_taps, g, d_en.as<float>(), fe->stream);
	HIP_TRY(hipMemcpyAsync(en.data(), d_en.p, sizeof(float) * en.size(), hipMemcpyDeviceToHost, fe->stream));
	HIP_TRY(hipStreamSynchronize(fe->stream));
	const std::vector<RowWindow> w = fold_row_windows(en, g.pre, g.nch_pad, g.nch, fe->prune_tol, &fe->fold_rows_max);
	static_assert(sizeof(RowWindow) == sizeof(int2), "a window is what the fold kernels load as an int2 { first quad, count }");
	HIP_TRY(fe->alloc(fe->d_win, w.size()));
	HIP_TRY(hipMemcpy(fe->d_win, w.data(), sizeof(int2) * w.size(), hipMemcpyHostToDevice));
	g.fold_win = fe->d_win;
	return 0;
}

bool design_channel(const hfdl_gpu_frontend *fe, int rx, int32_t freq, ChanConst &k, std::complex<float> *taps, std::vector<float> &lp, float &lp_cut)
{
	float shift = (float)(fe->rx_center[(size_t)rx] - (freq + 1440)) / (float)fe->sample_rate;
	Plan cp;
	if (!plan_block(cp, fe->tbw, fe->decimation, shift)) return false;
	k = ChanConst{};
	k.offsetbin = cp.offsetbin;
	k.nco_sindelta = cp.sindelta; k.nco_cosdelta = cp.cosdelta; k.nco_rate = cp.rate;
	k.frequency = freq;
	if (taps == nullptr) return true;
	float half_bw = 0.5f / fe->decimation;
	design_bandpass(taps, fe->plan.taps_length, (-shift) - half_bw, (-shift) + half_bw, lp, lp_cut);
	return true;
}

static int build_taps(hfdl_gpu_frontend *fe)
{
	const Plan &pl = fe->plan;
	const int nch = (int)fe->freqs.size();
	const size_t n = (size_t)pl.n;
	std::vector<std::complex<float>> host((size_t)nch * (size_t)pl.taps_length);
	fe->cc.resize((size_t)nch);
	unsigned nthreads = std::max(1u, std::min((unsigned)nch, std::thread::hardware_concurrency()));
	nthreads = std::min(nthreads, (unsigned)env_long("HFDL_GPU_HOST_THREADS", 1, 1 << 16, (long)nthreads));
	std::atomic<int> next{0};
	std::atomic<int> bad{0};
	auto work = [&]() {
		std::vector<float> lp;
		float lp_cut = -1.f;
		for (;;) {
			int c = next.fetch_add(1);
			if (c >= nch) break;
			if (!design_channel(fe, fe->rx_of[(size_t)c], fe->freqs[c], fe->cc[c], host.data() + (size_t)c * pl.taps_length, lp, lp_cut)) bad++;
		}
	};
	std::vector<std::thread> pool;
	for (unsigned t = 1; t < nthreads; t++) pool.emplace_back(work);
	work();
	for (auto &t : pool) t.join();
	if (bad) return fail(HFDL_GPU_EINVAL, "fastddc planning failed for %d channel(s)", (int)bad);

	DevBuf pad;
	HIP_TRY(pad.alloc(sizeof(float2) * n));
	float2 *d_pad = pad.as<float2>();
	HIP_TRY(hipMemsetAsync(d_pad, 0, sizeof(float2) * n, fe->stream));
	if (fe->geo.nch_pad > nch)
		HIP_TRY(hipMemsetAsync(fe->d_taps, 0, sizeof(float2) * n * (size_t)fe->geo.nch_pad, fe->stream));
	for (int c = 0; c < nch; c++) {
		HIP_TRY(hipMemcpyAsync(d_pad, host.data() + (size_t)c * pl.taps_length, sizeof(float2) * (size_t)pl.taps_length,
				hipMemcpyHostToDevice, fe->stream));
		const int slot = fe->slot_of(c);
		FftOutLayout lay = fe->tap_layout;
		lay.chan = slot;
		float2 *dst = lay.kind == TAPL_PLAIN ? fe->d_taps + (size_t)slot * (size_t)fe->geo.tap_chan_stride : fe->d_taps;
		launch_fft_forward(fe->fft.p, nullptr, d_pad, SFMT_CF32, 0, nullptr, fe->d_work, dst, true, fe->stream, lay);
	}
	HIP_TRY(hipStreamSynchronize(fe->stream));
	HIP_TRY(hipGetLastError());
	return 0;
}

int hfdl::check_channel_span(int32_t sample_rate, int32_t nrx, int c, int32_t freq, int r, int32_t centre)
{
	if (std::abs((int64_t)centre - freq) < sample_rate / 2) return 0;
	return nrx == 1 ? fail(HFDL_GPU_EINVAL, "channel %d Hz outside +-fs/2 of centre %d", freq, centre)
	                : fail(HFDL_GPU_EINVAL, "channel %d (%d Hz) outside +-fs/2 of the centre %d of its receiver %d", c, freq, centre, r);
}

static int check_create_args(hfdl_gpu_frontend **out, int32_t sample_rate, int32_t nrx, const int32_t *centerfreqs, const int32_t *freqs,
		const int32_t *nch_per_rx)
{
	if (!out || !centerfreqs || !freqs || !nch_per_rx) return fail(HFDL_GPU_EINVAL, "bad arguments: null pointer");
	*out = nullptr;
	if (nrx < 1 || nrx > HFDL_GPU_RECEIVERS_MAX) return fail(HFDL_GPU_EINVAL, "bad arguments: %d receivers (1 .. %d)", nrx, HFDL_GPU_RECEIVERS_MAX);
	for (int r = 0; r < nrx; r++)
		if (nch_per_rx[r] <= 0) return fail(HFDL_GPU_EINVAL, "bad arguments: receiver %d has %d channels", r, nch_per_rx[r]);
	if (sample_rate < 5400) return fail(HFDL_GPU_EINVAL, "sample rate must be >= 5400 (src/main.c:638-641)");
	for (int r = 0, c = 0; r < nrx; r++)
		for (int i = 0; i < nch_per_rx[r]; i++, c++)
			if (int rc = check_channel_span(sample_rate, nrx, c, freqs[c], r, centerfreqs[r])) return rc;
	return 0;
}

extern "C" int hfdl_gpu_frontend_create(hfdl_gpu_frontend **out, int device, int32_t sample_rate, int32_t centerfreq,
		const int32_t *freqs, int32_t nch)
{
	if (!out || !freqs || nch <= 0) return fail(HFDL_GPU_EINVAL, "bad arguments");
	return hfdl_gpu_frontend_create_multi(out, device, sample_rate, 1, &centerfreq, freqs, &nch);
}

static int create_streams(hfdl_gpu_frontend *fe, const LabConfig &lab)
{
	CuPartition part = plan_cu_partition((int)fe->freqs.size(), Demod::workgroup_lds(), fe->fold_bound);
	if (!lab.cu_partition || lab.cu_split) part.on = false;
	if (part.on) {
		const hipError_t ea = fe->stream.create_on_cus(part.mask_fold), eb = fe->stream_b.create_on_cus(part.mask_demod);
		if (ea != hipSuccess || eb != hipSuccess) {
			fe->stream.reset(); fe->stream_b.reset();
			(void)hipGetLastError();
			(void)fail(0, "CU-masked streams refused (%s): the demodulators share the fold's CUs", hipGetErrorString(ea != hipSuccess ? ea : eb));
			part.on = false;
		}
	}
	fe->cu_partitioned = part.on;
	if (part.on) {
	} else if (lab.cu_split) {
		uint32_t mask_a[8] = {}, mask_b[8] = {};
		for (int i = 0; i < 256; i++)
			((((i >> 3) + i) % lab.cu_split) == 0 ? mask_b : mask_a)[i >> 5] |= 1u << (i & 31);
		CREATE_TRY(fe->stream.create_on_cus(mask_a));
		CREATE_TRY(fe->stream_b.create_on_cus(mask_b));
	} else {
		CREATE_TRY(fe->stream.create());
		CREATE_TRY(fe->stream_b.create());
	}
	if (lab.decode_stream) CREATE_TRY(fe->stream_d.create());
	else fe->stream_d.alias(fe->stream_b);
	fe->demod.order.own_decode = fe->own_decode_stream();
	if (lab.fft_stream < 0 ? part.on : lab.fft_stream != 0) {
		if (part.on) CREATE_TRY(fe->stream_f.create_on_cus(part.mask_fold));
		else CREATE_TRY(fe->stream_f.create());
		fe->fft_rule = FFT_RULE_OWN;
	} else if (lab.fft_stream == 0) fe->fft_rule = FFT_RULE_SERIAL;
	CREATE_TRY(fe->stream_c.create());
	return 0;
}

static int create_frontend(hfdl_gpu_frontend *fe, int32_t nrx, const int32_t *nch_per_rx)
{
	const int nch = (int)fe->freqs.size();
	const LabConfig lab = read_lab_config();
	if (!plan_block(fe->plan, fe->tbw, fe->decimation, 0.f)) return fail(HFDL_GPU_EINVAL, "fastddc planning failed");
	const Plan &pl = fe->plan;
	Geometry &g = fe->geo;
	g.n = pl.n; g.m = pl.m; g.pre = pl.pre; g.post = pl.post; g.scrap = pl.scrap; g.post_input_size = pl.post_input_size;
	g.overlap = pl.overlap; g.input_size = pl.input_size; g.outs = (pl.post_input_size + pl.post - 1) / pl.post + 1;
	g.nch = nch;
	g.tap_layout = (pl.m % 16) == 0 && (pl.pre % 8) == 0 ? TAPL_OCTET : TAPL_PLAIN;
	g.nch_pad = plan_receiver_slots(nch_per_rx, nrx, tap_layout_group(g.tap_layout), fe->rx_span);
	for (const RxSpan &r : fe->rx_span) fe->rx_host.push_back(make_int4(r.slot0, r.slots, r.chan0, r.nch));
	g.nrx = nrx;
	g.spec_rx_stride = pl.n;
	g.rx_host = fe->rx_host.data();
	g.tap_chan_stride = pl.m; g.tap_row_stride = (int64_t)g.nch_pad * pl.m;
	g.fold_tile = lab.fold_tile;
	fe->tap_layout.kind = g.tap_layout;
	fe->tap_layout.row_log = ilog2(pl.m); fe->tap_layout.row_stride = g.tap_row_stride;
	fe->prune_tol = g.tap_layout == TAPL_OCTET && nrx == 1 ? env_double("HFDL_GPU_FOLD_PRUNE", 1e-12, 1e-3, 0.0) : 0.0;
	fe->fold_bound = lab.fold_bound < 0 ? nch >= 128 : lab.fold_bound != 0;
	const float resamp_rate = (float)(1800 * 3) / ((float)fe->sample_rate / (float)fe->decimation);
	BatchOverrides ov;
	ov.demod_batch = (int)env_long("HFDL_GPU_DEMOD_BATCH", 1, hfdl_gpu_frontend::MAX_HALF, 0);
	ov.fold_batch = (int)env_long("HFDL_GPU_FOLD_BATCH", 1, hfdl_gpu_frontend::MAX_HALF, 0);
	ov.pruned = fe->prune_tol > 0;
	ov.fold_slices = lab.fold_slices;
	ov.no_ramp = !lab.fold_ramp;
	const BatchPlan bp = plan_batches(nch, nrx, pl.n, pl.input_size, fe->sample_rate, pl.pre, fe->fold_bound,
			[&](int want) { return Demod::fit_batch(g.outs, resamp_rate, want); }, ov);
	g.slices = bp.slices;
	g.rows_per_slice = pl.pre / g.slices;
	if (pl.m > 8192 || pl.m < 16) return fail(HFDL_GPU_ERANGE, "inverse FFT size %d unsupported", pl.m);

	if (int rc = create_streams(fe, lab)) return rc;
	for (int i = 0; i < 2; i++) {
		CREATE_TRY(fe->spec[i].own.create(EV_NO_TIMING));
		CREATE_TRY(fe->chan[i].own.create(EV_NO_TIMING));
	}
	CREATE_TRY(fe->fft_done.own.create(EV_NO_TIMING));
	CREATE_TRY(fe->ev_switch.create(EV_NO_TIMING));
	if (int rc = fe->fft.build(pl.n)) return rc;
	const size_t n = (size_t)pl.n;
	const size_t K = (size_t)nrx;
	for (int i = 0; i < 2; i++) {
		CREATE_TRY(fe->alloc(fe->d_hist[i], (size_t)pl.overlap * K));
		CREATE_TRY(hipMemsetAsync(fe->d_hist[i], 0, sizeof(float2) * (size_t)pl.overlap * K, fe->stream));
	}
	CREATE_TRY(fe->alloc(fe->d_work, n * K));
	CREATE_TRY(fe->alloc(fe->d_rx, K));
	CREATE_TRY(hipMemcpy(fe->d_rx, fe->rx_host.data(), sizeof(int4) * K, hipMemcpyHostToDevice));
	g.rx_tab = fe->d_rx;
	if (g.tap_layout == TAPL_OCTET) {
		static_assert(sizeof(FoldGroup) == sizeof(int4), "a FoldGroup entry is what the fold kernels load as an int4");
		const std::vector<FoldGroup> t = fold_group_tables(fe->rx_span, g.nch_pad / 8, FOLD_GROUP_MAX);
		CREATE_TRY(fe->alloc(fe->d_grp, t.size()));
		CREATE_TRY(hipMemcpy(fe->d_grp, t.data(), sizeof(int4) * t.size(), hipMemcpyHostToDevice));
		g.grp_tab = fe->d_grp;
	}
	CREATE_TRY(fe->alloc(fe->d_taps, n * (size_t)g.nch_pad));
	CREATE_TRY(fe->alloc(fe->d_nco, (size_t)nch));
	CREATE_TRY(hipMemsetAsync(fe->d_nco, 0, sizeof(NcoState) * (size_t)nch, fe->stream));
	CREATE_TRY(fe->alloc(fe->d_ph_cont, (size_t)nch));
	CREATE_TRY(hipMemsetAsync(fe->d_ph_cont, 0, sizeof(float2) * (size_t)nch, fe->stream));
	CREATE_TRY(fe->alloc(fe->d_cc, (size_t)nch));
	fe->mem.emplace_back();
	if (int rc = upload_twiddles(pl.m, fe->mem.back())) return rc;
	fe->d_tw_m = fe->mem.back().as<float2>();
	if (prepare_ifft_nco(pl.m) != hipSuccess)
		return fail(HFDL_GPU_EHIP, "inverse FFT of %d points: LDS attribute refused: %s", pl.m, hipGetErrorString(hipGetLastError()));
	if (int rc = build_taps(fe)) return rc;
	if (fe->prune_tol > 0 && g.tap_layout == TAPL_OCTET)
		if (int rc = build_fold_windows(fe)) return rc;
	CREATE_TRY(hipMemcpy(fe->d_cc, fe->cc.data(), sizeof(ChanConst) * (size_t)nch, hipMemcpyHostToDevice));
	fe->fold_nb = bp.fold_nb;
	if (int rc = fe->demod.init(nch, g.outs, resamp_rate, fe->freqs.data(), fe->stream, bp.batch_want)) return rc;
	fe->batch = fe->demod.batch;
	fe->half_blocks = bp.half_blocks;
	fe->half_first = fe->half_target = bp.half_first;
	fe->n_stage = bp.n_stage;
	for (int i = 0; i < fe->n_stage; i++) {
		CREATE_TRY(fe->ev_stage_ready[i].create(EV_NO_TIMING));
		CREATE_TRY(fe->ev_stage_free[i].create(EV_NO_TIMING));
	}
	const size_t hb = (size_t)fe->half_blocks;
	CREATE_TRY(fe->alloc(fe->d_spec, fe->spec_stride() * 2 * hb));
	CREATE_TRY(fe->alloc(fe->d_partial, fe->partial_stride() * hb));
	CREATE_TRY(fe->alloc(fe->d_ph, fe->ph_stride() * 2 * hb));
	CREATE_TRY(fe->alloc(fe->d_nco_snap, (size_t)nch * 2 * hb));
	CREATE_TRY(fe->alloc(fe->d_chan_all, 2 * hb * (size_t)nch * g.outs));
	CREATE_TRY(fe->alloc(fe->d_cnt_all, 2 * hb * (size_t)nch));
	CREATE_TRY(hipMemsetAsync(fe->d_cnt_all, 0, sizeof(int) * 2 * hb * (size_t)nch, fe->stream));
	CREATE_TRY(hipStreamSynchronize(fe->stream));
	return 0;
}

extern "C" int hfdl_gpu_frontend_create_multi(hfdl_gpu_frontend **out, int device, int32_t sample_rate, int32_t nrx,
		const int32_t *centerfreqs, const int32_t *freqs, const int32_t *nch_per_rx)
{
	int rc = check_create_args(out, sample_rate, nrx, centerfreqs, freqs, nch_per_rx);
	if (rc || (rc = select_device(device))) return rc;
	int32_t nch = 0;
	for (int r = 0; r < nrx; r++) nch += nch_per_rx[r];
	auto fe = std::make_unique<hfdl_gpu_frontend>();
	fe->device = device;
	fe->sample_rate = sample_rate;
	fe->decimation = fft_decimation_rate(sample_rate, 1800 * 3);
	fe->tbw = relative_transition_bw(sample_rate, 250);
	fe->freqs.assign(freqs, freqs + nch);
	fe->nrx = nrx;
	fe->rx_center.assign(centerfreqs, centerfreqs + nrx);
	for (int r = 0; r < nrx; r++) fe->rx_of.insert(fe->rx_of.end(), (size_t)nch_per_rx[r], r);
	if ((rc = create_frontend(fe.get(), nrx, nch_per_rx))) return rc;
	*out = fe.release();
	return 0;
}

hfdl_gpu_frontend::~hfdl_gpu_frontend()
{
	(void)hipSetDevice(device);
	for (const hfdl::Stream *s : { &stream, &stream_b, &stream_d, &stream_c, &stream_f, &demod.st_collect }) (void)s->sync();
	if (mon) (void)hipEventSynchronize(mon->newest());
}

extern "C" void hfdl_gpu_frontend_destroy(hfdl_gpu_frontend *fe) { delete fe; }
```

### dumphfdl_amd/csrc/frontend_query.cpp

```cpp
#include <algorithm>
#include <cstdarg>
#include <cstdio>
#include <cstring>
#include <mutex>
#include "frontend.h"
#include "demod_lds.h"

using namespace hfdl;

static thread_local char g_err[512] = "";

int hfdl::fail(int code, const char *fmt, ...)
{
	va_list ap;
	va_start(ap, fmt);
	vsnprintf(g_err, sizeof(g_err), fmt, ap);
	va_end(ap);
	return code;
}

int hfdl::fail_hip(hipError_t e, bool alloc, const char *expr, const char *file, int line)
{
	return fail(alloc && e == hipErrorOutOfMemory ? HFDL_GPU_ENOMEM : HFDL_GPU_EHIP, "%s: %s (%s:%d)", expr, hipGetErrorString(e), file, line);
}

extern "C" const char *hfdl_gpu_last_error(void) { return g_err; }


static void fill_block_geometry(const Plan &p, hfdl_gpu_geometry *g)
{
	g->pre_decimation = p.pre; g->post_decimation = p.post;
	g->taps_length = p.taps_length; g->overlap_length = p.overlap;
	g->fft_size = p.n; g->fft_inv_size = p.m; g->input_size = p.input_size;
	g->post_input_size = p.post_input_size; g->scrap = p.scrap;
	g->outputs_per_block = p.post_input_size / p.post;
	g->max_outputs_per_block = (p.post_input_size + p.post - 1) / p.post;
}

extern "C" int hfdl_gpu_frontend_geometry(const hfdl_gpu_frontend *fe, hfdl_gpu_geometry *g)
{
	if (!fe || !g) return fail(HFDL_GPU_EINVAL, "null argument");
	fill_block_geometry(fe->plan, g);
	g->sample_rate = fe->sample_rate; g->decimation = fe->decimation;
	g->channels = fe->geo.nch; g->fold_slices = fe->geo.slices;
	g->demod_batch = fe->batch;
	g->fold_batch = fe->fold_nb;
	g->prefetch_depth = fe->n_stage - 1;
	g->fold_rows = fe->fold_rows_max ? fe->fold_rows_max : fe->plan.pre;
	g->transition_bw = fe->tbw;
	g->resamp_rate = (float)(1800 * 3) / ((float)fe->sample_rate / (float)fe->decimation);
	return 0;
}

extern "C" int hfdl_gpu_plan_geometry(int32_t decimation, float transition_bw, hfdl_gpu_geometry *g)
{
	if (!g || decimation < 1 || !(transition_bw > 0.f)) return fail(HFDL_GPU_EINVAL, "bad arguments");
	Plan p;
	if (!plan_block(p, transition_bw, decimation, 0.f)) return fail(HFDL_GPU_EINVAL, "fastddc planning failed");
	memset(g, 0, sizeof(*g));
	fill_block_geometry(p, g);
	g->decimation = decimation;
	g->transition_bw = transition_bw;
	return 0;
}

extern "C" int hfdl_gpu_frontend_channel_receiver(const hfdl_gpu_frontend *fe, int32_t channel, int32_t *rx, int32_t *centerfreq)
{
	if (!fe || !rx || !centerfreq) return fail(HFDL_GPU_EINVAL, "null argument");
	if (channel < 0 || channel >= fe->geo.nch) return fail(HFDL_GPU_EINVAL, "channel %d out of range (%d channels)", channel, fe->geo.nch);
	*rx = fe->rx_of[(size_t)channel];
	*centerfreq = fe->rx_center[(size_t)*rx];
	return 0;
}


static std::mutex g_pinned_lock;
static std::vector<std::pair<const char *, size_t>> g_pinned;

bool hfdl::is_library_pinned(const void *p, size_t bytes)
{
	std::lock_guard<std::mutex> lk(g_pinned_lock);
	for (auto &r : g_pinned)
		if ((const char *)p >= r.first && (const char *)p + bytes <= r.first + r.second) return true;
	return false;
}

extern "C" int hfdl_gpu_host_alloc(void **ptr, size_t bytes)
{
	if (!ptr || !bytes) return fail(HFDL_GPU_EINVAL, "bad arguments");
	HIP_TRY(hipHostMalloc(ptr, bytes, hipHostMallocDefault));
	std::lock_guard<std::mutex> lk(g_pinned_lock);
	g_pinned.emplace_back((const char *)*ptr, bytes);
	return 0;
}

extern "C" void hfdl_gpu_host_free(void *ptr)
{
	if (!ptr) return;
	{
		std::lock_guard<std::mutex> lk(g_pinned_lock);
		for (size_t i = 0; i < g_pinned.size(); i++)
			if (g_pinned[i].first == (const char *)ptr) { g_pinned.erase(g_pinned.begin() + (long)i); break; }
	}
	(void)hipHostFree(ptr);
}


extern "C" int hfdl_gpu_frontend_input_done(hfdl_gpu_frontend *fe)
{
	if (!fe) return fail(HFDL_GPU_EINVAL, "null argument");
	HIP_TRY(hipSetDevice(fe->device));
	if (fe->host_blocks) HIP_TRY(hipEventSynchronize(fe->input_event(fe->host_blocks - 1)));
	return 0;
}

static int check_host_block(const hfdl_gpu_frontend *fe, uint64_t host_block)
{
	if (!fe) return fail(HFDL_GPU_EINVAL, "null argument");
	if (host_block >= fe->host_blocks) return fail(HFDL_GPU_EINVAL, "host block %llu has not been pushed (%llu so far)", (unsigned long long)host_block, (unsigned long long)fe->host_blocks);
	HIP_TRY(hipSetDevice(fe->device));
	return 0;
}

extern "C" int hfdl_gpu_frontend_input_done_upto(hfdl_gpu_frontend *fe, uint64_t host_block)
{
	if (int rc = check_host_block(fe, host_block)) return rc;
	HIP_TRY(hipEventSynchronize(fe->input_event(host_block)));
	return 0;
}

extern "C" int hfdl_gpu_frontend_input_copied(hfdl_gpu_frontend *fe, uint64_t host_block)
{
	if (int rc = check_host_block(fe, host_block)) return rc;
	const hipError_t e = hipEventQuery(fe->input_event(host_block));
	if (e == hipSuccess) return 1;
	if (e == hipErrorNotReady) { (void)hipGetLastError(); return 0; }
	return fail(HFDL_GPU_EHIP, "hipEventQuery: %s", hipGetErrorString(e));
}


static int sync_to_read(hfdl_gpu_frontend *fe, bool args_ok = true)
{
	if (!fe || !args_ok) return fail(HFDL_GPU_EINVAL, "null argument");
	return hfdl_gpu_frontend_sync(fe);
}

extern "C" int hfdl_gpu_frontend_reset_timers(hfdl_gpu_frontend *fe, int enable)
{
	if (int rc = sync_to_read(fe)) return rc;
	return fe->timers.reset(enable != 0);
}

static int stage_totals(hfdl_gpu_frontend *fe, Stage s, double *ms, int64_t *launches, int64_t *blocks)
{
	if (int rc = sync_to_read(fe)) return rc;
	const LaunchTimers::Totals &t = fe->timers.stage[s];
	if (ms) *ms = t.ms;
	if (launches) *launches = t.launches;
	if (blocks) *blocks = t.blocks;
	return 0;
}

extern "C" int hfdl_gpu_frontend_fold_time_ms(hfdl_gpu_frontend *fe, double *total_ms, int64_t *launches) { return stage_totals(fe, ST_FOLD, total_ms, launches, nullptr); }

extern "C" int hfdl_gpu_frontend_fold_blocks(hfdl_gpu_frontend *fe, int64_t *blocks)
{
	if (!blocks) return fail(HFDL_GPU_EINVAL, "null argument");
	return stage_totals(fe, ST_FOLD, nullptr, nullptr, blocks);
}

extern "C" int hfdl_gpu_frontend_demod_time_ms(hfdl_gpu_frontend *fe, double *total_ms, int64_t *launches, int64_t *blocks) { return stage_totals(fe, ST_DEMOD, total_ms, launches, blocks); }

extern "C" int hfdl_gpu_frontend_fold_launch_shapes(hfdl_gpu_frontend *fe, int64_t counts[HFDL_GPU_FOLD_BATCH_MAX + 1], double ms[HFDL_GPU_FOLD_BATCH_MAX + 1])
{
	if (int rc = sync_to_read(fe, counts)) return rc;
	for (int i = 0; i <= FOLD_MAX_BLOCKS; i++) counts[i] = fe->timers.fold_shapes[i];
	if (ms) for (int i = 0; i <= FOLD_MAX_BLOCKS; i++) ms[i] = fe->timers.fold_shape_ms[i];
	return 0;
}

extern "C" int hfdl_gpu_frontend_stage_times(hfdl_gpu_frontend *fe, double ms[5], int64_t launches[5])
{
	if (int rc = sync_to_read(fe, ms && launches)) return rc;
	for (int s = 0; s < ST_N; s++) { ms[s] = fe->timers.stage[s].ms; launches[s] = fe->timers.stage[s].launches; }
	return 0;
}

extern "C" int hfdl_gpu_frontend_step_period_ms(hfdl_gpu_frontend *fe, double *period_ms)
{
	if (int rc = sync_to_read(fe, period_ms)) return rc;
	const LaunchTimers &t = fe->timers;
	const int64_t covered = t.stage[ST_FOLD].blocks - t.fold_last_blocks;
	*period_ms = (t.stage[ST_FOLD].launches > 1 && covered > 0) ? t.span_ms / (double)covered : 0.0;
	return 0;
}


extern "C" int hfdl_gpu_frontend_all_channel_stats(hfdl_gpu_frontend *fe, hfdl_gpu_channel_stats *out, int32_t cap, int32_t *n)
{
	if (!fe || !out || !n) return fail(HFDL_GPU_EINVAL, "null argument");
	if (cap < fe->geo.nch) return fail(HFDL_GPU_ERANGE, "%d channels, buffer holds %d", fe->geo.nch, cap);
	HIP_TRY(hipSetDevice(fe->device));
	memset(out, 0, sizeof(*out) * (size_t)fe->geo.nch);
	if (int rc = fe->demod.stats_all(out, fe->geo.nch)) return rc;
	for (int i = 0; i < fe->geo.nch; i++) out[i].freq = fe->freqs[(size_t)i];
	*n = fe->geo.nch;
	return 0;
}

extern "C" int hfdl_gpu_frontend_channel_stats(hfdl_gpu_frontend *fe, int32_t channel, hfdl_gpu_channel_stats *out)
{
	if (!fe || !out) return fail(HFDL_GPU_EINVAL, "null argument");
	if (channel < 0 || channel >= fe->geo.nch) return fail(HFDL_GPU_EINVAL, "channel out of range");
	int rc = hfdl_gpu_frontend_sync(fe);
	if (rc) return rc;
	memset(out, 0, sizeof(*out));
	out->freq = fe->freqs[(size_t)channel];
	return fe->demod.stats(channel, out);
}

extern "C" int hfdl_gpu_frontend_counters(hfdl_gpu_frontend *fe, hfdl_gpu_frontend_counters_t *out)
{
	if (!fe || !out) return fail(HFDL_GPU_EINVAL, "null argument");
	memset(out, 0, sizeof(*out));
	out->blocks = fe->blocks;
	out->pdus_taken = fe->demod.taken;
	out->pdus_dropped = fe->demod.dropped;
	out->pdu_ring_capacity = (uint32_t)fe->demod.pdu_cap;
	return 0;
}

extern "C" int hfdl_gpu_frontend_enable_taps(hfdl_gpu_frontend *fe, int enable)
{
	if (int rc = sync_to_read(fe)) return rc;
	fe->demod.taps_enabled = enable != 0;
	return 0;
}

extern "C" int hfdl_gpu_frontend_read_tap_block(hfdl_gpu_frontend *fe, int what, int32_t channel, int32_t back, float *dst, size_t cap, size_t *n_floats)
{
	if (int rc = sync_to_read(fe, dst && n_floats)) return rc;
	const Geometry &g = fe->geo;
	if (back < 0 || back > fe->last_index) return fail(HFDL_GPU_ERANGE, "block %d back is not held any more (%d are)", back, fe->last_index);
	if (back && what != HFDL_GPU_TAP_SPECTRUM && what != HFDL_GPU_TAP_CHAN_OUT && what != HFDL_GPU_TAP_NCO_PHASORS && what != HFDL_GPU_TAP_NOTCH_OUT)
		return fail(HFDL_GPU_EINVAL, "tap %d holds the last launch only", what);
	const int slot = fe->last_slot - back, index = fe->last_index - back;
	if ((what != HFDL_GPU_TAP_SPECTRUM || fe->nrx > 1) && (channel < 0 || channel >= g.nch)) return fail(HFDL_GPU_EINVAL, "channel out of range");
	const void *src = nullptr;
	size_t nf = 0;
	switch (what) {
	case HFDL_GPU_TAP_SPECTRUM:
		src = fe->spec_slot(fe->last_set, index) + (fe->nrx > 1 ? (size_t)fe->rx_of[(size_t)channel] * (size_t)g.n : 0);
		nf = 2 * (size_t)g.n;
		break;
	case HFDL_GPU_TAP_FILTER: {
		if (2 * (size_t)g.n > cap) return fail(HFDL_GPU_ERANGE, "tap needs %zu floats, buffer holds %zu", 2 * (size_t)g.n, cap);
		DevBuf plain;
		HIP_TRY(plain.alloc(sizeof(float2) * (size_t)g.n));
		launch_tap_extract(fe->d_taps, g, fe->slot_of(channel), plain.as<float2>(), fe->stream);
		HIP_TRY(hipStreamSynchronize(fe->stream));
		HIP_TRY(hipMemcpy(dst, plain.p, sizeof(float2) * (size_t)g.n, hipMemcpyDeviceToHost));
		*n_floats = 2 * (size_t)g.n;
		return 0; }
	case HFDL_GPU_TAP_CHAN_OUT:
	case HFDL_GPU_TAP_NOTCH_OUT: {
		const Notch *nt = fe->notch.get();
		if (what == HFDL_GPU_TAP_NOTCH_OUT && !(nt && nt->mu > 0.f)) return fail(HFDL_GPU_EINVAL, "tap %d: the canceller is off", what);
		int cnt = 0;
		HIP_TRY(hipMemcpy(&cnt, fe->cnt_slot(slot) + channel, sizeof(cnt), hipMemcpyDeviceToHost));
		src = (what == HFDL_GPU_TAP_CHAN_OUT ? fe->chan_slot(slot) : nt->out.as<float2>() + (size_t)slot * (size_t)g.nch * (size_t)g.outs) + (size_t)channel * g.outs;
		nf = 2 * (size_t)cnt; break; }
	case HFDL_GPU_TAP_NCO_PHASORS: {
		int cnt = 0;
		HIP_TRY(hipMemcpy(&cnt, fe->cnt_slot(slot) + channel, sizeof(cnt), hipMemcpyDeviceToHost));
		if (2 * (size_t)cnt > cap) return fail(HFDL_GPU_ERANGE, "tap needs %zu floats, buffer holds %zu", 2 * (size_t)cnt, cap);
		if (cnt) HIP_TRY(hipMemcpy2D(dst, sizeof(float2), fe->ph_slot(fe->last_set, index) + channel, sizeof(float2) * (size_t)g.nch, sizeof(float2), (size_t)cnt, hipMemcpyDeviceToHost));
		*n_floats = 2 * (size_t)cnt;
		return 0; }
	case HFDL_GPU_TAP_PHASE_CYCLES: src = fe->demod.d_tap_lvl + (size_t)channel * fe->demod.cap + phase_slot(fe->demod.cap, PHASE_AHEAD); nf = DM_PHASE_SLOTS; break;
	default:
		if (int rc = fe->demod.tap(what, channel, &src, &nf)) return rc;
	}
	if (nf > cap) return fail(HFDL_GPU_ERANGE, "tap needs %zu floats, buffer holds %zu", nf, cap);
	if (nf) HIP_TRY(hipMemcpy(dst, src, sizeof(float) * nf, hipMemcpyDeviceToHost));
	*n_floats = nf;
	return 0;
}

extern "C" int hfdl_gpu_frontend_read_tap(hfdl_gpu_frontend *fe, int what, int32_t channel, float *dst, size_t cap, size_t *n_floats)
{
	return hfdl_gpu_frontend_read_tap_block(fe, what, channel, 0, dst, cap, n_floats);
}


static_assert(HFDL_GPU_SPECTRUM_HANN == SPECMON_HANN && HFDL_GPU_SPECTRUM_MAXHOLD == SPECMON_MAXHOLD, "include/hfdl_gpu.h and spectrum.h name the same flags");
static_assert(HFDL_GPU_RECEIVERS_MAX <= 64, "SpecmonJob::fresh is one bit per receiver");

extern "C" int hfdl_gpu_frontend_spectrum_enable(hfdl_gpu_frontend *fe, int32_t bins, uint32_t flags)
{
	if (!fe) return fail(HFDL_GPU_EINVAL, "null argument");
	if (flags & ~(HFDL_GPU_SPECTRUM_HANN | HFDL_GPU_SPECTRUM_MAXHOLD)) return fail(HFDL_GPU_EINVAL, "unknown spectrum flags 0x%x", flags);
	if (bins != 0 && (bins < 16 || (bins & (bins - 1)) != 0)) return fail(HFDL_GPU_EINVAL, "spectrum bins %d: a power of two >= 16 (or 0 = off)", bins);
	if (bins > fe->geo.n / 16) return fail(HFDL_GPU_ERANGE, "spectrum bins %d: at most fft_size / 16 = %d", bins, fe->geo.n / 16);
	HIP_TRY(hipSetDevice(fe->device));
	if (fe->mon) (void)hipEventSynchronize(fe->mon->newest());
	fe->mon.reset();
	if (bins == 0) return 0;
	const size_t nb = (size_t)bins, K = (size_t)fe->nrx;
	auto mon = std::make_unique<SpectrumMonitor>();
	hipError_t e = mon->acc.alloc(sizeof(float2) * nb * K);
	if (e == hipSuccess && (flags & HFDL_GPU_SPECTRUM_MAXHOLD)) e = mon->peak.alloc(sizeof(float) * nb * K);
	if (e == hipSuccess) e = mon->host.alloc(3 * nb);
	if (e == hipSuccess) e = mon->ev.create(EV_NO_TIMING);
	if (e != hipSuccess) return fail(e == hipErrorOutOfMemory ? HFDL_GPU_ENOMEM : HFDL_GPU_EHIP, "spectrum monitor buffers: %s", hipGetErrorString(e));
	mon->bins = bins;
	mon->flags = flags;
	mon->fresh = ~(uint64_t)0;
	mon->blocks.assign(K, 0);
	mon->first.assign(K, 0);
	fe->mon = std::move(mon);
	return 0;
}

static void mean_of(const float *h, size_t nb, uint64_t T, float *mean)
{
	for (size_t b = 0; b < nb; b++) mean[b] = (float)(((double)h[2 * b] - (double)h[2 * b + 1]) / (double)T);
}

extern "C" int hfdl_gpu_frontend_spectrum_read(hfdl_gpu_frontend *fe, int32_t rx, float *mean, float *peak, int32_t cap,
		uint64_t *blocks, uint64_t *first_block, int reset)
{
	if (!fe || !mean || !blocks || !first_block) return fail(HFDL_GPU_EINVAL, "null argument");
	SpectrumMonitor *mon = fe->mon.get();
	if (!mon) return fail(HFDL_GPU_EINVAL, "the spectrum monitor is off: hfdl_gpu_frontend_spectrum_enable() first");
	if (rx < 0 || rx >= fe->nrx) return fail(HFDL_GPU_EINVAL, "receiver %d out of range (%d receivers)", rx, fe->nrx);
	if (peak && !(mon->flags & HFDL_GPU_SPECTRUM_MAXHOLD)) return fail(HFDL_GPU_EINVAL, "peak asked for, but the monitor was enabled without HFDL_GPU_SPECTRUM_MAXHOLD");
	if (cap < mon->bins) return fail(HFDL_GPU_ERANGE, "%d bands, buffer holds %d", mon->bins, cap);
	const bool pending = (mon->fresh >> rx) & 1;
	const uint64_t T = pending ? 0 : mon->blocks[(size_t)rx];
	*blocks = T;
	*first_block = pending ? fe->blocks : mon->first[(size_t)rx];
	if (T == 0) return 0;
	HIP_TRY(hipSetDevice(fe->device));
	const size_t nb = (size_t)mon->bins;
	float *h = mon->host.p;
	hipStream_t st = fe->demod.st_collect;
	HIP_TRY(hipStreamWaitEvent(st, mon->newest(), 0));
	HIP_TRY(hipMemcpyAsync(h, mon->acc.as<float2>() + (size_t)rx * nb, sizeof(float2) * nb, hipMemcpyDeviceToHost, st));
	if (peak) HIP_TRY(hipMemcpyAsync(h + 2 * nb, mon->peak.as<float>() + (size_t)rx * nb, sizeof(float) * nb, hipMemcpyDeviceToHost, st));
	HIP_TRY(hipStreamSynchronize(st));
	mean_of(h, nb, T, mean);
	if (peak) memcpy(peak, h + 2 * nb, sizeof(float) * nb);
	if (reset) mon->fresh |= (uint64_t)1 << rx;
	return 0;
}


extern "C" int hfdl_gpu_frontend_spectrum_history(hfdl_gpu_frontend *fe, int32_t rows, int32_t interval_blocks)
{
	if (rows != 0 && (rows < 2 || rows > HFDL_GPU_SPECTRUM_ROWS_MAX)) return fail(HFDL_GPU_EINVAL, "spectrum history rows %d: 2 .. %d (or 0 = off)", rows, HFDL_GPU_SPECTRUM_ROWS_MAX);
	if (interval_blocks < 0) return fail(HFDL_GPU_EINVAL, "spectrum history interval of %d blocks", interval_blocks);
	if (!fe) return fail(HFDL_GPU_EINVAL, "null argument");
	SpectrumMonitor *mon = fe->mon.get();
	if (!mon) return fail(HFDL_GPU_EINVAL, "the spectrum monitor is off: hfdl_gpu_frontend_spectrum_enable() first");
	const size_t set = (size_t)fe->nrx * (size_t)mon->bins, R = (size_t)rows;
	if (R * set * 12 > ((size_t)1 << 30)) return fail(HFDL_GPU_ERANGE, "spectrum history of %d rows x %d receivers x %d bands: more than 1 GiB", rows, fe->nrx, mon->bins);
	HIP_TRY(hipSetDevice(fe->device));
	if (mon->hist) {
		(void)hipEventSynchronize(mon->newest());
		mon->last = nullptr;
		mon->hist.reset();
	}
	if (rows == 0) return 0;
	auto h = std::make_unique<SpectrumHistory>();
	hipError_t e = h->acc.alloc(sizeof(float2) * R * set);
	if (e == hipSuccess && (mon->flags & HFDL_GPU_SPECTRUM_MAXHOLD)) e = h->peak.alloc(sizeof(float) * R * set);
	if (e == hipSuccess) e = h->host.alloc((size_t)SpectrumHistory::CHUNK * 3 * (size_t)mon->bins);
	h->ev.resize(R);
	for (size_t i = 0; i < R && e == hipSuccess; i++) e = h->ev[i].create(EV_NO_TIMING);
	if (e != hipSuccess) return fail(e == hipErrorOutOfMemory ? HFDL_GPU_ENOMEM : HFDL_GPU_EHIP, "spectrum history buffers: %s", hipGetErrorString(e));
	h->rows = rows;
	h->interval = interval_blocks;
	h->info.resize(R);
	mon->hist = std::move(h);
	return 0;
}

extern "C" int hfdl_gpu_frontend_spectrum_row_close(hfdl_gpu_frontend *fe, uint64_t *row)
{
	if (!fe || !row) return fail(HFDL_GPU_EINVAL, "null argument");
	SpectrumHistory *h = fe->mon ? fe->mon->hist.get() : nullptr;
	if (!h) return fail(HFDL_GPU_EINVAL, "the spectrum history is off: hfdl_gpu_frontend_spectrum_history() first");
	*row = h->open;
	if (h->open_blocks) h->close();
	return 0;
}

extern "C" int hfdl_gpu_frontend_spectrum_rows(hfdl_gpu_frontend *fe, int32_t rx, uint64_t from_row, int32_t max_rows,
		float *mean, float *peak, hfdl_gpu_spectrum_row *info, int32_t *n, uint64_t *next_row, int wait)
{
	if (!fe || !n || !next_row) return fail(HFDL_GPU_EINVAL, "null argument");
	SpectrumMonitor *mon = fe->mon.get();
	SpectrumHistory *h = mon ? mon->hist.get() : nullptr;
	if (!h) return fail(HFDL_GPU_EINVAL, "the spectrum history is off: hfdl_gpu_frontend_spectrum_history() first");
	if (rx < 0 || rx >= fe->nrx) return fail(HFDL_GPU_EINVAL, "receiver %d out of range (%d receivers)", rx, fe->nrx);
	if (max_rows < 0) return fail(HFDL_GPU_EINVAL, "max_rows %d", max_rows);
	if (max_rows > 0 && (!mean || !info)) return fail(HFDL_GPU_EINVAL, "null argument");
	if (peak && !(mon->flags & HFDL_GPU_SPECTRUM_MAXHOLD)) return fail(HFDL_GPU_EINVAL, "peak asked for, but the monitor was enabled without HFDL_GPU_SPECTRUM_MAXHOLD");
	const uint64_t R = (uint64_t)h->rows;
	uint64_t from = std::min(std::max(from_row, h->oldest()), h->open);
	uint64_t end = std::min(h->open, from + (uint64_t)max_rows);
	*n = 0;
	*next_row = from;
	if (end == from) return 0;
	HIP_TRY(hipSetDevice(fe->device));
	if (wait) HIP_TRY(hipEventSynchronize(h->ev[(end - 1) % R]));
	else for (uint64_t r = from; r < end; r++) {
		const hipError_t e = hipEventQuery(h->ev[r % R]);
		if (e == hipSuccess) continue;
		if (e != hipErrorNotReady) return fail(HFDL_GPU_EHIP, "hipEventQuery: %s", hipGetErrorString(e));
		(void)hipGetLastError();
		end = r;
	}
	const size_t nb = (size_t)mon->bins, K = (size_t)fe->nrx;
	hipStream_t st = fe->demod.st_collect;
	for (uint64_t r0 = from; r0 < end; r0 += SpectrumHistory::CHUNK) {
		const size_t cnt = (size_t)std::min<uint64_t>(SpectrumHistory::CHUNK, end - r0);
		for (size_t i = 0; i < cnt; i++) {
			const size_t at = ((size_t)((r0 + i) % R) * K + (size_t)rx) * nb;
			float *hb = h->host.p + i * 3 * nb;
			HIP_TRY(hipMemcpyAsync(hb, h->acc.as<float2>() + at, sizeof(float2) * nb, hipMemcpyDeviceToHost, st));
			if (peak) HIP_TRY(hipMemcpyAsync(hb + 2 * nb, h->peak.as<float>() + at, sizeof(float) * nb, hipMemcpyDeviceToHost, st));
		}
		HIP_TRY(hipStreamSynchronize(st));
		for (size_t i = 0; i < cnt; i++) {
			const size_t o = (size_t)(r0 + i - from);
			const float *hb = h->host.p + i * 3 * nb;
			info[o] = h->info[(size_t)((r0 + i) % R)];
			mean_of(hb, nb, info[o].blocks, mean + o * nb);
			if (peak) memcpy(peak + o * nb, hb + 2 * nb, sizeof(float) * nb);
		}
	}
	*n = (int32_t)(end - from);
	*next_row = end;
	return 0;
}


extern "C" int hfdl_gpu_frontend_blanker_enable(hfdl_gpu_frontend *fe, float threshold_db)
{
	if (!(threshold_db == 0.f || (threshold_db >= BLANK_DB_MIN && threshold_db <= BLANK_DB_MAX))) return fail(HFDL_GPU_EINVAL, "blanker threshold %g dB", (double)threshold_db);
	if (!fe) return fail(HFDL_GPU_EINVAL, "null argument");
	if (!fe->blank) {
		if (threshold_db == 0.f) return 0;
		HIP_TRY(hipSetDevice(fe->device));
		const size_t K = (size_t)fe->nrx, n = (size_t)fe->geo.input_size;
		auto b = std::make_unique<Blanker>();
		hipError_t e = b->scratch.alloc(sizeof(float2) * K * n);
		if (e == hipSuccess) e = b->partial.alloc(sizeof(float) * K * (size_t)blank_chunks((int)n));
		if (e == hipSuccess) e = b->rec.zeroed(sizeof(BlankRecord) * K);
		if (e == hipSuccess) e = hipStreamSynchronize(nullptr);
		if (e == hipSuccess) e = b->host.alloc(1);
		if (e == hipSuccess) e = b->ev.create(EV_NO_TIMING);
		if (e != hipSuccess) return fail(e == hipErrorOutOfMemory ? HFDL_GPU_ENOMEM : HFDL_GPU_EHIP, "blanker buffers: %s", hipGetErrorString(e));
		fe->blank = std::move(b);
	}
	fe->blank->k2 = threshold_db == 0.f ? 0.f : blank_k2(threshold_db);
	return 0;
}

extern "C" int hfdl_gpu_frontend_blanker_stats(hfdl_gpu_frontend *fe, int32_t rx, hfdl_gpu_blanker_stats *out)
{
	if (!fe || !out) return fail(HFDL_GPU_EINVAL, "null argument");
	Blanker *b = fe->blank.get();
	if (!b) return fail(HFDL_GPU_EINVAL, "the blanker was never enabled");
	if (rx < 0 || rx >= fe->nrx) return fail(HFDL_GPU_EINVAL, "receiver %d out of range (%d receivers)", rx, fe->nrx);
	memset(out, 0, sizeof(*out));
	if (b->blocks == 0) return 0;
	HIP_TRY(hipSetDevice(fe->device));
	hipStream_t st = fe->demod.st_collect;
	hipError_t e = hipStreamWaitEvent(st, b->ev, 0);
	if (e == hipSuccess) e = hipMemcpyAsync(b->host.p, b->rec.as<BlankRecord>() + rx, sizeof(BlankRecord), hipMemcpyDeviceToHost, st);
	if (e == hipSuccess) e = hipStreamSynchronize(st);
	HIP_TRY(e);
	out->blocks = b->blocks;
	out->samples_blanked = b->host.p->blanked;
	out->last_power = b->host.p->power;
	out->last_threshold = b->host.p->threshold;
	return 0;
}


static_assert(HFDL_GPU_NOTCH_STATE_FLOATS == NOTCH_STATE_FLOATS, "include/hfdl_gpu.h and notch.h name the same state");

extern "C" int hfdl_gpu_frontend_notch_stats(hfdl_gpu_frontend *fe, int32_t channel, hfdl_gpu_notch_stats *out)
{
	if (!fe || !out) return fail(HFDL_GPU_EINVAL, "null argument");
	Notch *n = fe->notch.get();
	if (!n) return fail(HFDL_GPU_EINVAL, "the canceller was never enabled");
	if (channel < 0 || channel >= fe->geo.nch || !n->selected[(size_t)channel]) return fail(HFDL_GPU_EINVAL, "channel %d is out of range or not selected", channel);
	memset(out, 0, sizeof(*out));
	if (!n->launched) return 0;
	HIP_TRY(hipSetDevice(fe->device));
	hipStream_t st = fe->demod.st_collect;
	hipError_t e = hipStreamWaitEvent(st, n->ev, 0);
	if (e == hipSuccess) e = hipMemcpyAsync(n->host.p, n->rec.as<NotchRecord>() + channel, sizeof(NotchRecord), hipMemcpyDeviceToHost, st);
	if (e == hipSuccess) e = hipStreamSynchronize(st);
	HIP_TRY(e);
	out->blocks = n->host.p->blocks;
	out->resets = n->host.p->resets;
	out->last_in_power = n->host.p->in_power;
	out->last_out_power = n->host.p->out_power;
	out->tap_energy = n->host.p->tap_energy;
	return 0;
}


static_assert(HFDL_GPU_EXPORT_CF32 == EXPORT_CF32 && HFDL_GPU_EXPORT_CS16 == EXPORT_CS16, "include/hfdl_gpu.h and spectrum.h name the same formats");

extern "C" int hfdl_gpu_frontend_export_enable(hfdl_gpu_frontend *fe, const int32_t *channels, int32_t nsel, int format, float scale, int32_t ring_blocks)
{
	if (!fe || (!channels && nsel > 0)) return fail(HFDL_GPU_EINVAL, "null argument");
	const size_t S = (size_t)nsel, R = (size_t)ring_blocks, P = (size_t)fe->geo.outs - 1;
	const size_t es = format == HFDL_GPU_EXPORT_CS16 ? sizeof(short2) : sizeof(float2);
	if (nsel > 0) {
		bool ok = nsel <= fe->geo.nch && (format == HFDL_GPU_EXPORT_CF32 || format == HFDL_GPU_EXPORT_CS16) && ring_blocks >= 2 && ring_blocks <= HFDL_GPU_EXPORT_RING_MAX
			&& (format == HFDL_GPU_EXPORT_CF32 || (scale > 0.f && scale <= 3.402823466e38f));
		std::vector<bool> seen((size_t)fe->geo.nch);
		for (size_t i = 0; ok && i < S; i++) {
			ok = channels[i] >= 0 && channels[i] < fe->geo.nch && !seen[(size_t)channels[i]];
			if (ok) seen[(size_t)channels[i]] = true;
		}
		if (!ok) return fail(HFDL_GPU_EINVAL, "export: bad channels, format, scale or ring");
		if (R * S * (P * es + 12) > ((size_t)1 << 30)) return fail(HFDL_GPU_ERANGE, "export ring above 1 GiB");
	} else if (nsel < 0) return fail(HFDL_GPU_EINVAL, "export: nsel %d", nsel);
	HIP_TRY(hipSetDevice(fe->device));
	std::unique_ptr<ChannelExport> x;
	if (nsel > 0) {
		x = std::make_unique<ChannelExport>();
		x->chunk = std::max<size_t>(1, std::min(R, ((size_t)4 << 20) / (S * P * es)));
		hipError_t e = x->channels.alloc(sizeof(int32_t) * S);
		if (e == hipSuccess) e = x->samples.alloc(R * S * P * es);
		if (e == hipSuccess) e = x->counts.alloc(R * S * 4);
		if (e == hipSuccess) e = x->power.alloc(R * S * 4);
		if (e == hipSuccess) e = x->clipped.alloc(R * S * 4);
		if (e == hipSuccess) e = x->host.alloc(x->chunk * S * (P * es + 12));
		x->ev.resize(R);
		for (size_t i = 0; i < R && e == hipSuccess; i++) e = x->ev[i].create(EV_NO_TIMING);
		if (e == hipSuccess) e = hipMemcpy(x->channels.p, channels, sizeof(int32_t) * S, hipMemcpyHostToDevice);
		if (e != hipSuccess) return fail(e == hipErrorOutOfMemory ? HFDL_GPU_ENOMEM : HFDL_GPU_EHIP, "export buffers: %s", hipGetErrorString(e));
		x->nsel = nsel; x->format = format; x->scale = scale;
		x->last_of.resize(R);
		x->ring.start((uint32_t)ring_blocks, fe->blocks);
	}
	if (fe->exp && fe->exp->newest) (void)hipEventSynchronize(fe->exp->newest);
	fe->exp = std::move(x);
	return 0;
}

extern "C" int hfdl_gpu_frontend_export_read(hfdl_gpu_frontend *fe, uint64_t from_block, int32_t max_blocks, void *samples, int32_t *counts,
		float *power, uint32_t *clipped, hfdl_gpu_export_block *info, int32_t *n, uint64_t *next_block, int wait)
{
	if (!fe || !n || !next_block) return fail(HFDL_GPU_EINVAL, "null argument");
	ChannelExport *x = fe->exp.get();
	if (!x || max_blocks < 0 || (max_blocks > 0 && (!samples || !counts || !info))) return fail(HFDL_GPU_EINVAL, "export off, or bad arguments");
	HIP_TRY(hipSetDevice(fe->device));
	ExportRing &ring = x->ring;
	if (wait && x->newest) HIP_TRY(hipEventSynchronize(x->newest));
	hipError_t bad = hipSuccess;
	ring.settle(x->last_of.data(), [&](uint32_t at) {
		const hipError_t e = hipEventQuery(x->ev[at]);
		if (e == hipSuccess) return true;
		if (e == hipErrorNotReady) (void)hipGetLastError(); else bad = e;
		return false;
	});
	if (bad != hipSuccess) return fail(HFDL_GPU_EHIP, "hipEventQuery: %s", hipGetErrorString(bad));
	uint64_t from = 0, end = 0;
	ring.range(from_block, (uint64_t)max_blocks, from, end);
	const size_t S = (size_t)x->nsel, row = S * ((size_t)fe->geo.outs - 1) * (x->format == HFDL_GPU_EXPORT_CS16 ? sizeof(short2) : sizeof(float2));
	hipStream_t st = fe->demod.st_collect;
	for (uint64_t b = from, run = 0; b < end; b += run) {
		const size_t slot = ring.slot(b), o = (size_t)(b - from);
		run = std::min<uint64_t>(std::min<uint64_t>(x->chunk, end - b), ring.R - slot);
		char *h = x->host.p, *meta = h + x->chunk * row;
		const void *src[3] = { x->counts.p, power ? x->power.p : nullptr, clipped ? x->clipped.p : nullptr };
		void *dst[3] = { counts + o * S, power ? power + o * S : nullptr, clipped ? clipped + o * S : nullptr };
		HIP_TRY(hipMemcpyAsync(h, (const char *)x->samples.p + slot * row, run * row, hipMemcpyDeviceToHost, st));
		for (int k = 0; k < 3; k++)
			if (src[k]) HIP_TRY(hipMemcpyAsync(meta + k * x->chunk * S * 4, (const char *)src[k] + slot * S * 4, run * S * 4, hipMemcpyDeviceToHost, st));
		HIP_TRY(hipStreamSynchronize(st));
		memcpy((char *)samples + o * row, h, run * row);
		for (int k = 0; k < 3; k++)
			if (src[k]) memcpy(dst[k], meta + k * x->chunk * S * 4, run * S * 4);
		for (uint64_t i = 0; i < run; i++) info[o + i].block = b + i;
	}
	*n = (int32_t)(end - from);
	*next_block = end;
	return 0;
}
```

### dumphfdl_amd/csrc/hfdl_gpu.cpp

```cpp
#include <algorithm>
#include "frontend.h"

using namespace hfdl;


int LaunchTimers::arm(Stage s, int blocks, hipEvent_t &start, hipEvent_t &stop)
{
	if (!on) return 0;
	Timed t;
	if (!pool.empty()) {
		t = std::move(pool.back());
		pool.pop_back();
	} else {
		HIP_TRY(t.start.create(EV_TIMING));
		HIP_TRY(t.stop.create(EV_TIMING));
	}
	t.blocks = blocks;
	start = t.start;
	stop = t.stop;
	stage[s].pending.push_back(std::move(t));
	return 0;
}

int LaunchTimers::drain()
{
	for (int s = 0; s < ST_N; s++) {
		for (Timed &t : stage[s].pending) {
			float ms = 0;
			HIP_TRY(hipEventElapsedTime(&ms, t.start, t.stop));
			stage[s].ms += ms;
			stage[s].launches++;
			stage[s].blocks += t.blocks;
			if (s == ST_FOLD) {
				fold_last_blocks = t.blocks;
				if (t.blocks >= 1 && t.blocks <= FOLD_MAX_BLOCKS) { fold_shapes[t.blocks]++; fold_shape_ms[t.blocks] += ms; }
				if (!first_fold) {
					first_fold = std::move(t.start);
					HIP_TRY(t.start.create(EV_TIMING));
				} else {
					HIP_TRY(hipEventElapsedTime(&ms, first_fold, t.start));
					span_ms = ms;
				}
			}
			pool.push_back(std::move(t));
		}
		stage[s].pending.clear();
	}
	return 0;
}

int LaunchTimers::reset(bool enable)
{
	on = enable;
	for (Totals &t : stage) { t.ms = 0; t.launches = 0; t.blocks = 0; }
	for (auto &c : fold_shapes) c = 0;
	for (auto &c : fold_shape_ms) c = 0;
	first_fold = Event();
	span_ms = 0;
	fold_last_blocks = 0;
	while (enable && pool.size() < 1280) {
		Timed t;
		HIP_TRY(t.start.create(EV_TIMING));
		HIP_TRY(t.stop.create(EV_TIMING));
		pool.push_back(std::move(t));
	}
	return 0;
}

int hfdl_gpu_frontend::settle_events()
{
	if (int rc = timers.drain()) return rc;
	demod.settle();
	for (DoneEvent *d : { &chan[0], &chan[1], &fft_done, &spec[0], &spec[1] }) d->settle();
	return 0;
}


extern "C" void *hfdl_gpu_frontend_stream(hfdl_gpu_frontend *fe) { return fe ? (void *)fe->fft_stream(fe->side_of(true)) : nullptr; }

static int check_block(const hfdl_gpu_frontend *fe, size_t nsamples, int fmt)
{
	if (fmt != SFMT_CF32 && fmt != SFMT_CS16 && fmt != SFMT_CU8) return fail(HFDL_GPU_EINVAL, "unknown sample format %d", fmt);
	if (nsamples != (size_t)fe->plan.input_size)
		return fail(HFDL_GPU_EINVAL, "a block is exactly %d samples (got %zu)", fe->plan.input_size, nsamples);
	return 0;
}

static int queue_input_copy(hfdl_gpu_frontend *fe, const void *const *iq, size_t nsamples, int fmt, int *sb_out)
{
	if (fe->host_blocks - fe->host_pushed >= (uint64_t)fe->n_stage)
		return fail(HFDL_GPU_ERANGE, "%d uploads are queued ahead of their blocks: push the oldest first", fe->n_stage);
	const uint64_t j = fe->host_blocks;
	const int sb = (int)(j % (uint64_t)fe->n_stage);
	const size_t need = nsamples * (size_t)fe->nrx;
	if (fe->stage_cap[sb] < need) {
		HIP_TRY(hipStreamSynchronize(fe->stream_c));
		HIP_TRY(hipStreamSynchronize(fe->fft_stream(fe->side_of(false))));
		fe->stage_cap[sb] = 0;
		fe->d_stage[sb] = std::make_unique<DevBuf>();
		HIP_TRY(fe->d_stage[sb]->alloc(sizeof(float2) * need));
		fe->stage_cap[sb] = need;
	}
	HIP_TRY(hipStreamWaitEvent(fe->stream_c, fe->ev_stage_free[sb], 0));
	const size_t bytes = sample_bytes(fmt) * nsamples;
	bool pinned = true;
	for (int r = 0; r < fe->nrx; r++) {
		HIP_TRY(hipMemcpyAsync(fe->d_stage[sb]->as<char>() + (size_t)r * bytes, iq[r], bytes, hipMemcpyHostToDevice, fe->stream_c));
		pinned = pinned && is_library_pinned(iq[r], bytes);
	}
	HIP_TRY(hipEventRecord(fe->ev_stage_ready[sb], fe->stream_c));
	fe->host_blocks = j + 1;
	if (!pinned) HIP_TRY(hipEventSynchronize(fe->ev_stage_ready[sb]));
	*sb_out = sb;
	return 0;
}

static int stage_input(hfdl_gpu_frontend *fe, const void *const *iq, size_t nsamples, int fmt, int on_device, FftInputs &in, int *stage_idx)
{
	*stage_idx = -1;
	if (!fe || !iq) return fail(HFDL_GPU_EINVAL, "null argument");
	for (int r = 0; r < fe->nrx; r++) if (!iq[r]) return fail(HFDL_GPU_EINVAL, "null argument: the block of receiver %d", r);
	if (int rc = check_block(fe, nsamples, fmt)) return rc;
	HIP_TRY(hipSetDevice(fe->device));
	const bool queued = fe->host_pushed < fe->host_blocks;
	if (on_device) {
		if (queued) return fail(HFDL_GPU_EINVAL, "a prefetched block is pending: push it or call hfdl_gpu_frontend_prefetch_cancel()");
		for (int r = 0; r < fe->nrx; r++) in.fresh[r] = iq[r];
		return 0;
	}
	int sb;
	if (queued) {
		sb = (int)(fe->host_pushed % (uint64_t)fe->n_stage);
		if (fe->pf_ptr[sb] != iq[0] || fe->pf_fmt[sb] != fmt) return fail(HFDL_GPU_EINVAL, "the block pushed after a prefetch must be the (oldest) prefetched one");
	} else {
		int rc = queue_input_copy(fe, iq, nsamples, fmt, &sb);
		if (rc) return rc;
	}
	fe->host_pushed++;
	HIP_TRY(hipStreamWaitEvent(fe->fft_stream(fe->side_of(false)), fe->ev_stage_ready[sb], 0));
	for (int r = 0; r < fe->nrx; r++) in.fresh[r] = fe->d_stage[sb]->as<const char>() + (size_t)r * sample_bytes(fmt) * nsamples;
	*stage_idx = sb;
	return 0;
}

static int single_receiver_only(const hfdl_gpu_frontend *fe, const char *what)
{
	if (fe && fe->nrx > 1)
		return fail(HFDL_GPU_EINVAL, "%s: this front end has %d receivers -- push a block of every receiver with hfdl_gpu_frontend_push_blocks_raw()", what, fe->nrx);
	return 0;
}

extern "C" int hfdl_gpu_frontend_prefetch_block_raw(hfdl_gpu_frontend *fe, const void *raw, size_t nsamples, int sample_format)
{
	if (!fe || !raw) return fail(HFDL_GPU_EINVAL, "null argument");
	if (int rc = single_receiver_only(fe, "hfdl_gpu_frontend_prefetch_block_raw")) return rc;
	if (int rc = check_block(fe, nsamples, sample_format)) return rc;
	if (fe->host_blocks - fe->host_pushed >= (uint64_t)(fe->n_stage - 1))
		return fail(HFDL_GPU_ERANGE, "%d blocks are prefetched already (geometry.prefetch_depth): push the oldest first", fe->n_stage - 1);
	if (!is_library_pinned(raw, sample_bytes(sample_format) * nsamples)) return fail(HFDL_GPU_EINVAL, "only buffers from hfdl_gpu_host_alloc() can be prefetched");
	HIP_TRY(hipSetDevice(fe->device));
	int sb = -1;
	const void *one[1] = { raw };
	int rc = queue_input_copy(fe, one, nsamples, sample_format, &sb);
	if (rc) return rc;
	fe->pf_ptr[sb] = raw; fe->pf_fmt[sb] = sample_format;
	return 0;
}

extern "C" int hfdl_gpu_frontend_prefetch_cancel(hfdl_gpu_frontend *fe)
{
	if (!fe) return fail(HFDL_GPU_EINVAL, "null argument");
	if (int rc = single_receiver_only(fe, "hfdl_gpu_frontend_prefetch_cancel")) return rc;
	if (fe->host_pushed == fe->host_blocks) return 0;
	HIP_TRY(hipSetDevice(fe->device));
	HIP_TRY(hipEventSynchronize(fe->input_event(fe->host_blocks - 1)));
	fe->host_pushed = fe->host_blocks;
	return 0;
}


static int launch_demod(hfdl_gpu_frontend *fe, int buf, int nblk, hipEvent_t ready)
{
	const int slot0 = buf * fe->half_blocks;
	if (Notch *n = fe->notch.get(); n && n->mu > 0.f) {
		const Geometry &g = fe->geo;
		const size_t at = (size_t)slot0 * (size_t)g.nch * (size_t)g.outs;
		float2 *out = n->out.as<float2>() + at;
		if (ready) HIP_TRY(hipStreamWaitEvent(fe->stream_b, ready, 0));
		if (n->nsel < g.nch) HIP_TRY(hipMemcpyAsync(out, fe->chan_slot(slot0), sizeof(float2) * (size_t)nblk * (size_t)g.nch * (size_t)g.outs, hipMemcpyDeviceToDevice, fe->stream_b));
		NotchJob j;
		j.in = fe->chan_slot(slot0); j.out = out; j.cnt = fe->cnt_slot(slot0); j.sel = n->sel.as<int32_t>();
		j.state = n->state.as<float>(); j.rec = n->rec.as<NotchRecord>();
		j.nch = g.nch; j.outs = g.outs; j.nblk = nblk; j.nsel = n->nsel; j.mu = n->mu;
		launch_notch(j, fe->stream_b, n->ev);
		n->launched = true;
		return fe->demod.launch_half(out, fe->cnt_slot(slot0), nblk, buf, nullptr, fe->stream_b, fe->stream_d, fe->timers);
	}
	return fe->demod.launch_half(fe->chan_slot(slot0), fe->cnt_slot(slot0), nblk, buf, ready, fe->stream_b, fe->stream_d, fe->timers);
}

static void leave_half(hfdl_gpu_frontend *fe, int nblk, bool with_demod)
{
	const int half = fe->cur_half;
	fe->last_slot = half * fe->half_blocks + nblk - 1;
	fe->last_index = nblk - 1;
	fe->cur_half ^= 1;
	if (with_demod) fe->demod.order.hand_over(half);
}

static int flush_pending_demod(hfdl_gpu_frontend *fe, bool after_fft)
{
	if (fe->pending_demod_buf < 0) return 0;
	const int buf = fe->pending_demod_buf, nblk = fe->pending_demod_nblk;
	fe->pending_demod_buf = -1;
	return launch_demod(fe, buf, nblk, after_fft ? fe->fft_done.event() : fe->chan[buf].event());
}

static int enqueue_fft(hfdl_gpu_frontend *fe, FftInputs &in, int fmt, int stage_idx, int on_device)
{
	const Geometry &g = fe->geo;
	const int i = fe->batch_fill, set = fe->cur_half;
	const FftPushPlan plan = fe->order.push(fe->side_of(on_device != 0), i, fe->half_target, fe->pending_demod_buf >= 0);
	const hipStream_t st = fe->fft_stream(plan.side);
	if (plan.flush_before)
		if (int rc = flush_pending_demod(fe, false)) return rc;
	if (plan.wait_switch) {
		HIP_TRY(hipEventRecord(fe->ev_switch, fe->fft_stream(plan.side ^ 1)));
		HIP_TRY(hipStreamWaitEvent(st, fe->ev_switch, 0));
	}
	if (plan.wait_set_free && fe->chan[set].pending()) HIP_TRY(hipStreamWaitEvent(st, fe->chan[set].event(), 0));
	if (plan.wait_first_fold) HIP_TRY(hipStreamWaitEvent(st, fe->chan[set ^ 1].event(), 0));
	if (plan.wait_retune) HIP_TRY(hipStreamWaitEvent(st, fe->retune->done.event(), 0));
	NcoJob job;
	job.cc = fe->d_cc; job.chain = fe->d_nco; job.snap = fe->snap_slot(set, i);
	job.ph = fe->ph_slot(set, i); job.cont = fe->d_ph_cont;
	job.nch = g.nch; job.outs = g.outs; job.post_input_size = g.post_input_size; job.post = g.post;
	hipEvent_t fft_start = nullptr, fft_done = nullptr;
	if (plan.side == FFT_BESIDE || plan.hold_after) {
		DoneEvent &done = plan.side == FFT_BESIDE ? fe->spec[set] : fe->fft_done;
		if (int rc = fe->timers.arm(ST_FFT, 1, done, fft_start)) return rc;
		fft_done = done.event();
	} else if (int rc = fe->timers.arm(ST_FFT, 1, fft_start, fft_done)) return rc;
	if (Blanker *b = fe->blank.get(); b && b->k2 > 0.f) {
		BlankJob j;
		for (int r = 0; r < fe->nrx; r++) j.fresh[r] = in.fresh[r];
		j.out = b->scratch.as<float2>(); j.out_stride = g.input_size; j.partial = b->partial.as<float>(); j.rec = b->rec.as<BlankRecord>();
		j.n = g.input_size; j.nrx = fe->nrx; j.fmt = fmt; j.k2 = b->k2;
		launch_blanker(j, st, b->ev);
		for (int r = 0; r < fe->nrx; r++) in.fresh[r] = j.out + (size_t)r * (size_t)g.input_size;
		fmt = SFMT_CF32;
		b->blocks++;
	}
	in.nrx = fe->nrx; in.hist_stride = g.overlap; in.out_stride = g.n;
	launch_fft_forward(fe->fft.p, fe->d_hist[fe->blocks & 1], in, fmt, g.overlap, fe->d_hist[(fe->blocks + 1) & 1], fe->d_work, fe->spec_slot(set, i), true, st,
			FftOutLayout(), fft_done, job,
			stage_idx >= 0 ? fe->ev_stage_free[stage_idx].e : nullptr,
			fft_start);
	if (SpectrumMonitor *mon = fe->mon.get()) {
		SpecmonJob m;
		m.spec = fe->spec_slot(set, i); m.rx_stride = g.n; m.n = g.n; m.bins = mon->bins; m.nrx = fe->nrx; m.flags = mon->flags;
		m.scale = (float)(1.0 / ((double)g.n * (double)g.n * ((mon->flags & SPECMON_HANN) ? 0.375 : 1.0)));
		m.fresh = mon->fresh; m.acc = mon->acc.as<float2>(); m.peak = mon->peak.as<float>();
		SpectrumHistory *h = mon->hist.get();
		hipEvent_t done = mon->ev;
		if (h) {
			const size_t slot = (size_t)(h->open % (uint64_t)h->rows), set = (size_t)fe->nrx * (size_t)mon->bins;
			m.row_acc = h->acc.as<float2>() + slot * set;
			if (mon->flags & SPECMON_MAXHOLD) m.row_peak = h->peak.as<float>() + slot * set;
			m.row_fresh = h->open_blocks == 0;
			done = h->ev[slot];
		}
		launch_spectrum_monitor(m, st, done);
		mon->last = done;
		for (int r = 0; r < fe->nrx; r++) {
			if ((mon->fresh >> r) & 1) { mon->blocks[(size_t)r] = 0; mon->first[(size_t)r] = fe->blocks; }
			mon->blocks[(size_t)r]++;
		}
		if (h) {
			if (h->open_blocks++ == 0) h->open_first = fe->blocks;
			if (h->interval > 0 && h->open_blocks == (uint32_t)h->interval) h->close();
		}
		mon->fresh = 0;
	}
	if (plan.hold_after) {
		int rc = flush_pending_demod(fe, true);
		if (rc) return rc;
	}
	HIP_TRY(hipGetLastError());
	fe->blocks++;
	fe->batch_fill++;
	return 0;
}

static int close_half(hfdl_gpu_frontend *fe, bool launch_now, bool with_demod = true)
{
	const int nblk = fe->batch_fill;
	if (nblk == 0) return 0;
	const Geometry &g = fe->geo;
	const int half = fe->cur_half;
	const HalfClosePlan plan = fe->order.close(launch_now);
	if (plan.wait_input) HIP_TRY(hipStreamWaitEvent(fe->stream, fe->spec[half].event(), 0));
	for (int done = 0, take = 0; done < nblk; done += take) {
		take = fold_launch_blocks(g, nblk - done, fe->fold_nb);
		hipEvent_t start = nullptr, stop = nullptr;
		if (int rc = fe->timers.arm(ST_FOLD, take, start, stop)) return rc;
		if (launch_fold(g, fe->d_taps, fe->spec_slot(half, done), fe->spec_stride(), fe->d_partial + (size_t)done * fe->partial_stride(), fe->partial_stride(),
				take, fe->stream, start, stop) < 0)
			return fail(HFDL_GPU_EINVAL, "no fold launch of %d blocks on this geometry", take);
	}
	if (hipEvent_t e = fe->demod.half_read_event(half)) HIP_TRY(hipStreamWaitEvent(fe->stream, e, 0));
	if (with_demod && fe->own_decode_stream() && !fe->fold_bound) {
		if (hipEvent_t e = fe->demod.frames_free_event()) HIP_TRY(hipStreamWaitEvent(fe->stream, e, 0));
	}
	const int slot0 = half * fe->half_blocks;
	hipEvent_t ifft_start = nullptr;
	if (int rc = fe->timers.arm(ST_IFFT, nblk, fe->chan[half], ifft_start)) return rc;
	launch_ifft_nco(g, fe->d_partial, fe->partial_stride(), fe->d_cc, fe->snap_slot(half, 0), fe->ph_slot(half, 0), fe->ph_stride(), fe->d_tw_m,
			fe->chan_slot(slot0), fe->cnt_slot(slot0), nblk, fe->stream, fe->chan[half].event(), ifft_start);
	if (ChannelExport *x = fe->exp.get()) {
		const uint32_t skip = x->ring.skip_of_half(fe->blocks - (uint64_t)nblk, (uint32_t)nblk);
		if (skip < (uint32_t)nblk) {
			ExportJob e;
			e.chan = fe->chan_slot(slot0 + (int)skip); e.cnt = fe->cnt_slot(slot0 + (int)skip); e.channels = x->channels.as<int32_t>();
			e.nch = g.nch; e.outs = g.outs; e.P = g.outs - 1; e.nsel = x->nsel; e.nblk = nblk - (int)skip; e.format = x->format; e.scale = x->scale;
			e.slot0 = x->ring.slot(fe->blocks - (uint64_t)e.nblk); e.R = x->ring.R;
			e.samples = x->samples.p; e.counts = x->counts.as<int32_t>(); e.power = x->power.as<float>(); e.clipped = x->clipped.as<uint32_t>();
			x->newest = x->ev[x->ring.push_launch(x->last_of.data(), fe->blocks - 1)];
			launch_export_pack(e, fe->stream, x->newest);
		}
	}
	HIP_TRY(hipGetLastError());
	fe->last_set = half;
	fe->batch_fill = 0;
	leave_half(fe, nblk, with_demod);
	if (!with_demod) return 0;
	if (!plan.hold_back) return launch_demod(fe, half, nblk, fe->chan[half].event());
	fe->pending_demod_buf = half;
	fe->pending_demod_nblk = nblk;
	return 0;
}

extern "C" int hfdl_gpu_frontend_channelize_block(hfdl_gpu_frontend *fe, const float *iq, size_t nsamples, int on_device)
{
	FftInputs in;
	int sidx = -1;
	int rc = single_receiver_only(fe, "hfdl_gpu_frontend_channelize_block");
	if (rc) return rc;
	const void *one[1] = { iq };
	if ((rc = stage_input(fe, one, nsamples, SFMT_CF32, on_device, in, &sidx))) return rc;
	if ((rc = flush_pending_demod(fe, false))) return rc;
	if ((rc = close_half(fe, true))) return rc;
	if ((rc = enqueue_fft(fe, in, SFMT_CF32, sidx, on_device))) return rc;
	return close_half(fe, false, false);
}

extern "C" int hfdl_gpu_frontend_push_baseband(hfdl_gpu_frontend *fe, const float *chan_out, const int32_t *counts)
{
	if (!fe || !chan_out || !counts) return fail(HFDL_GPU_EINVAL, "null argument");
	const Geometry &g = fe->geo;
	for (int c = 0; c < g.nch; c++)
		if (counts[c] < 0 || counts[c] > g.outs) return fail(HFDL_GPU_ERANGE, "channel %d: %d samples, a block holds at most %d", c, counts[c], g.outs);
	int rc = hfdl_gpu_frontend_sync(fe);
	if (rc) return rc;
	const int half = fe->cur_half, slot0 = half * fe->half_blocks;
	HIP_TRY(hipMemcpy(fe->chan_slot(slot0), chan_out, sizeof(float2) * (size_t)g.nch * (size_t)g.outs, hipMemcpyHostToDevice));
	HIP_TRY(hipMemcpy(fe->cnt_slot(slot0), counts, sizeof(int32_t) * (size_t)g.nch, hipMemcpyHostToDevice));
	leave_half(fe, 1, true);
	return launch_demod(fe, half, 1, nullptr);
}

static int push_any(hfdl_gpu_frontend *fe, const void *const *raw, size_t nsamples, int fmt, int on_device)
{
	FftInputs in;
	int sidx = -1;
	int rc = stage_input(fe, raw, nsamples, fmt, on_device, in, &sidx);
	if (rc) return rc;
	if ((rc = enqueue_fft(fe, in, fmt, sidx, on_device))) return rc;
	if (fe->batch_fill < fe->half_target) return 0;
	rc = close_half(fe, !fe->fold_bound);
	fe->half_target = fe->half_blocks;
	return rc;
}

extern "C" int hfdl_gpu_frontend_push_block(hfdl_gpu_frontend *fe, const float *iq, size_t nsamples, int on_device)
{
	if (int rc = single_receiver_only(fe, "hfdl_gpu_frontend_push_block")) return rc;
	const void *one[1] = { iq };
	return push_any(fe, one, nsamples, SFMT_CF32, on_device);
}

extern "C" int hfdl_gpu_frontend_push_block_raw(hfdl_gpu_frontend *fe, const void *raw, size_t nsamples, int sample_format, int on_device)
{
	if (int rc = single_receiver_only(fe, "hfdl_gpu_frontend_push_block_raw")) return rc;
	const void *one[1] = { raw };
	return push_any(fe, one, nsamples, sample_format, on_device);
}

extern "C" int hfdl_gpu_frontend_push_blocks_raw(hfdl_gpu_frontend *fe, const void *const *raw, size_t nsamples, int sample_format, int on_device)
{
	if (!fe || !raw) return fail(HFDL_GPU_EINVAL, "null argument");
	return push_any(fe, raw, nsamples, sample_format, on_device);
}


extern "C" int hfdl_gpu_frontend_retune_channel(hfdl_gpu_frontend *fe, int32_t channel, int32_t new_freq_hz)
{
	if (!fe) return fail(HFDL_GPU_EINVAL, "null argument");
	const int nch = fe->geo.nch;
	if (channel < 0 || channel >= nch) return fail(HFDL_GPU_EINVAL, "channel %d out of range (%d channels)", channel, nch);
	if (fe->prune_tol > 0) return fail(HFDL_GPU_EINVAL, "retune refused: HFDL_GPU_FOLD_PRUNE is set, and the pruned fold's row windows depend on the pass bands");
	const int rx = fe->rx_of[(size_t)channel];
	if (int rc = check_channel_span(fe->sample_rate, fe->nrx, channel, new_freq_hz, rx, fe->rx_center[(size_t)rx])) return rc;
	for (int c = 0; c < nch; c++)
		if (c != channel && fe->rx_of[(size_t)c] == rx && fe->freqs[(size_t)c] == new_freq_hz)
			return fail(HFDL_GPU_EINVAL, "channel %d of receiver %d already listens on %d Hz", c, rx, new_freq_hz);
	const size_t ntaps = (size_t)fe->plan.taps_length, n = (size_t)fe->plan.n;
	ChanConst k;
	{
		std::vector<float> none;
		float cut = -1.f;
		if (!design_channel(fe, rx, new_freq_hz, k, nullptr, none, cut)) return fail(HFDL_GPU_EINVAL, "fastddc planning failed for %d channel(s)", 1);
	}
	HIP_TRY(hipSetDevice(fe->device));
	if (!fe->retune) {
		auto r = std::make_unique<Retune>();
		CREATE_TRY(r->pad.alloc(sizeof(float2) * n));
		CREATE_TRY(r->work.alloc(sizeof(float2) * n));
		for (int i = 0; i < 2; i++) {
			CREATE_TRY(r->stage[i].alloc(ntaps));
			CREATE_TRY(r->staged[i].create(EV_NO_TIMING));
		}
		CREATE_TRY(r->done.own.create(EV_NO_TIMING));
		if (int rc = fe->demod.prepare_retune(fe->stream_b)) return rc;
		HIP_TRY(hipMemsetAsync(r->pad.p, 0, sizeof(float2) * n, fe->stream));
		fe->retune = std::move(r);
	}
	Retune &r = *fe->retune;
	const int sb = (int)(r.calls & 1);
	if (r.calls >= 2) HIP_TRY(hipEventSynchronize(r.staged[sb]));
	static_assert(sizeof(std::complex<float>) == sizeof(float2), "taps are copied as cf32");
	design_channel(fe, rx, new_freq_hz, k, (std::complex<float> *)r.stage[sb].p, r.lp, r.lp_cut);
	if (int rc = flush_pending_demod(fe, false)) return rc;
	if (int rc = close_half(fe, true)) return rc;
	HIP_TRY(hipMemcpyAsync(r.pad.p, r.stage[sb].p, sizeof(float2) * ntaps, hipMemcpyHostToDevice, fe->stream));
	const int slot = fe->slot_of(channel);
	FftOutLayout lay = fe->tap_layout;
	lay.chan = slot;
	float2 *dst = lay.kind == TAPL_PLAIN ? fe->d_taps + (size_t)slot * (size_t)fe->geo.tap_chan_stride : fe->d_taps;
	launch_fft_forward(fe->fft.p, nullptr, r.pad.p, SFMT_CF32, 0, nullptr, r.work.as<float2>(), dst, true, fe->stream, lay, nullptr, NcoJob(), r.staged[sb]);
	launch_retune_channelizer(fe->d_cc, fe->d_nco, fe->d_ph_cont, channel, k, fe->stream, r.done.signal());
	fe->demod.enqueue_retune(channel, new_freq_hz, fe->stream_b, fe->stream_d);
	if (Notch *n = fe->notch.get()) HIP_TRY(hipMemsetAsync(n->state.as<float>() + (size_t)channel * NOTCH_STATE_FLOATS, 0, sizeof(float) * NOTCH_STATE_FLOATS, fe->stream_b));
	HIP_TRY(hipGetLastError());
	fe->order.retune();
	fe->freqs[(size_t)channel] = new_freq_hz;
	fe->cc[(size_t)channel] = k;
	r.calls++;
	return 0;
}


extern "C" int hfdl_gpu_frontend_notch_enable(hfdl_gpu_frontend *fe, const int32_t *channels, int32_t nsel, float mu)
{
	if (!(mu == 0.f || notch_mu_valid(mu))) return fail(HFDL_GPU_EINVAL, "canceller step %g: 0 (off) or %g .. %g", (double)mu, (double)NOTCH_MU_MIN, (double)NOTCH_MU_MAX);
	if (!fe || nsel < 0 || (nsel > 0 && !channels)) return fail(HFDL_GPU_EINVAL, "null argument");
	const int nch = fe->geo.nch;
	std::vector<int32_t> sel;
	std::vector<bool> seen((size_t)nch, channels == nullptr || nsel == 0);
	if (channels && nsel > 0) {
		for (int i = 0; i < nsel; i++) {
			if (channels[i] < 0 || channels[i] >= nch || seen[(size_t)channels[i]]) return fail(HFDL_GPU_EINVAL, "canceller: channel %d out of range or listed twice", channels[i]);
			seen[(size_t)channels[i]] = true;
		}
		sel.assign(channels, channels + nsel);
	} else for (int c = 0; c < nch; c++) sel.push_back(c);
	if (!fe->notch && mu == 0.f) return 0;
	HIP_TRY(hipSetDevice(fe->device));
	if (!fe->notch) {
		auto n = std::make_unique<Notch>();
		hipError_t e = n->out.alloc(sizeof(float2) * 2 * (size_t)fe->half_blocks * (size_t)nch * (size_t)fe->geo.outs);
		if (e == hipSuccess) e = n->sel.alloc(sizeof(int32_t) * (size_t)nch);
		if (e == hipSuccess) e = n->state.alloc(sizeof(float) * NOTCH_STATE_FLOATS * (size_t)nch);
		if (e == hipSuccess) e = n->rec.alloc(sizeof(NotchRecord) * (size_t)nch);
		if (e == hipSuccess) e = n->host.alloc(1);
		if (e == hipSuccess) e = n->host_sel.alloc((size_t)nch);
		if (e == hipSuccess) e = n->staged.create(EV_NO_TIMING);
		if (e == hipSuccess) e = n->ev.create(EV_NO_TIMING);
		if (e != hipSuccess) return fail(e == hipErrorOutOfMemory ? HFDL_GPU_ENOMEM : HFDL_GPU_EHIP, "canceller buffers: %s", hipGetErrorString(e));
		fe->notch = std::move(n);
	}
	if (int rc = flush_pending_demod(fe, false)) return rc;
	if (int rc = close_half(fe, true)) return rc;
	Notch &n = *fe->notch;
	n.mu = mu;
	if (mu == 0.f) return 0;
	if (n.staging) HIP_TRY(hipEventSynchronize(n.staged));
	std::copy(sel.begin(), sel.end(), n.host_sel.p);
	HIP_TRY(hipMemcpyAsync(n.sel.p, n.host_sel.p, sizeof(int32_t) * sel.size(), hipMemcpyHostToDevice, fe->stream_b));
	HIP_TRY(hipEventRecord(n.staged, fe->stream_b));
	n.staging = true;
	HIP_TRY(hipMemsetAsync(n.state.p, 0, sizeof(float) * NOTCH_STATE_FLOATS * (size_t)nch, fe->stream_b));
	HIP_TRY(hipMemsetAsync(n.rec.p, 0, sizeof(NotchRecord) * (size_t)nch, fe->stream_b));
	n.nsel = (int)sel.size();
	n.selected = seen;
	n.launched = false;
	return 0;
}


extern "C" int hfdl_gpu_frontend_sync(hfdl_gpu_frontend *fe)
{
	if (!fe) return fail(HFDL_GPU_EINVAL, "null argument");
	HIP_TRY(hipSetDevice(fe->device));
	{ int rc = flush_pending_demod(fe, false); if (rc) return rc; }
	{ int rc = close_half(fe, true); if (rc) return rc; }
	fe->half_target = fe->half_first;
	for (const Stream *s : { &fe->stream_c, &fe->stream_f, &fe->stream, &fe->stream_b, &fe->stream_d }) HIP_TRY(s->sync());
	fe->order.drained();
	HIP_TRY(hipGetLastError());
	return fe->settle_events();
}

static int check_poll_args(const hfdl_gpu_frontend *fe, const hfdl_gpu_pdu *out, int32_t max, const int32_t *n)
{
	if (!fe || !n) return fail(HFDL_GPU_EINVAL, "null argument");
	if (!out && max > 0) return fail(HFDL_GPU_EINVAL, "null PDU buffer with max = %d", max);
	return 0;
}

extern "C" int hfdl_gpu_frontend_poll_pdus(hfdl_gpu_frontend *fe, hfdl_gpu_pdu *out, int32_t max, int32_t *n)
{
	int rc = check_poll_args(fe, out, max, n);
	if (rc || (rc = hfdl_gpu_frontend_sync(fe))) return rc;
	return fe->demod.collect(out, max, n, fe->stream_d);
}

extern "C" int hfdl_gpu_frontend_poll_pdus_ready(hfdl_gpu_frontend *fe, hfdl_gpu_pdu *out, int32_t max, int32_t *n, int32_t max_in_flight)
{
	if (max_in_flight <= 0) return hfdl_gpu_frontend_poll_pdus(fe, out, max, n);
	if (int rc = check_poll_args(fe, out, max, n)) return rc;
	*n = 0;
	HIP_TRY(hipSetDevice(fe->device));
	return fe->demod.collect_ready(max_in_flight < 2, out, max, n, fe->stream_d);
}
```

### dumphfdl_amd/csrc/kernels.h

```cpp
#pragma once
#include <hip/hip_runtime.h>
#include <stdint.h>

namespace hfdl {

constexpr int FFT_TILE_LOG = 4;
constexpr int FFT_TILE = 1 << FFT_TILE_LOG;
constexpr int FFT_THREADS = 512;

struct FftPlan {
	int n, logn;
	int r1, r2, r3, l1, l2, l3;
	const float2 *tw1, *tw2, *tw3;
};

struct ChanConst {
	int32_t offsetbin;
	float nco_sindelta, nco_cosdelta;
	float nco_rate;
	int32_t frequency;
};

struct NcoState {
	int32_t decimation_remain;
	float starting_phase;
	int32_t output_size;
	int32_t pad;
};

struct Geometry {
	int32_t n, m, pre, post, scrap, post_input_size, overlap, input_size, outs;
	int32_t slices, rows_per_slice, nch;
	int32_t nch_pad;
	int32_t tap_layout;
	int64_t tap_chan_stride, tap_row_stride;
	const int2 *fold_win = nullptr;
	int32_t fold_tile = -1;
	const int4 *rx_tab = nullptr, *rx_host = nullptr;
	int32_t nrx = 1;
	int64_t spec_rx_stride = 0;
	const int4 *grp_tab = nullptr;
};
constexpr int FOLD_GROUP_MAX = 16;

enum { TAPL_PLAIN = 0, TAPL_OCTET = 2 };
__host__ __device__ inline size_t tap_index_f(int layout, int m, size_t rs_f, int c, int row, int j, int comp)
{
	if (layout == TAPL_OCTET)
		return (size_t)(row >> 2) * 4 * rs_f + (size_t)(c >> 3) * 64 * m + (size_t)(j >> 2) * 256 + (size_t)(16 * (row & 3) + 2 * (c & 7) + comp) * 4 + (j & 3);
	return (size_t)row * rs_f + ((size_t)c * m + j) * 2 + comp;
}
inline int tap_layout_group(int layout) { return layout == TAPL_OCTET ? 8 : 1; }

constexpr int FOLD_MAX_BLOCKS = 32;

struct NcoJob {
	const ChanConst *cc = nullptr;
	NcoState *chain = nullptr;
	NcoState *snap = nullptr;
	float2 *ph = nullptr;
	float2 *cont = nullptr;
	int32_t nch = 0, outs = 0, post_input_size = 0, post = 0;
	int32_t seg = 0, nseg = 3;
};

constexpr int RECEIVERS_MAX = 64;
struct FftInputs {
	const void *fresh[RECEIVERS_MAX] = {};
	int64_t hist_stride = 0, out_stride = 0;
	int32_t nrx = 1;
};

struct DevBuf {
	void *p = nullptr;
	DevBuf() = default;
	DevBuf(const DevBuf &) = delete;
	DevBuf &operator=(const DevBuf &) = delete;
	~DevBuf() { if (p) (void)hipFree(p); }
	hipError_t alloc(size_t bytes) { return hipMalloc(&p, bytes ? bytes : 1); }
	hipError_t upload(const void *src, size_t bytes) { const hipError_t e = alloc(bytes); return e != hipSuccess || !bytes ? e : hipMemcpy(p, src, bytes, hipMemcpyHostToDevice); }
	hipError_t zeroed(size_t bytes) { const hipError_t e = alloc(bytes); return e != hipSuccess || !bytes ? e : hipMemset(p, 0, bytes); }
	hipError_t fetch(void *dst, size_t bytes) const { return hipMemcpy(dst, p, bytes, hipMemcpyDeviceToHost); }
	template <typename T> T *as() const { return (T *)p; }
};

enum { SFMT_CF32 = 0, SFMT_CS16 = 1, SFMT_CU8 = 2 };
struct FftOutLayout { int row_log = 0; int64_t row_stride = 0; int kind = 0; int chan = 0; };
void launch_fft_forward(const FftPlan &p, const float2 *hist, const FftInputs &in, int fmt, int split, float2 *hist_next,
		float2 *work, float2 *out, bool shifted, hipStream_t st, FftOutLayout lay = FftOutLayout(), hipEvent_t done = nullptr,
		NcoJob nco = NcoJob(), hipEvent_t input_read = nullptr, hipEvent_t start = nullptr);
inline void launch_fft_forward(const FftPlan &p, const float2 *hist, const void *fresh, int fmt, int split, float2 *hist_next,
		float2 *work, float2 *out, bool shifted, hipStream_t st, FftOutLayout lay = FftOutLayout(), hipEvent_t done = nullptr,
		NcoJob nco = NcoJob(), hipEvent_t input_read = nullptr, hipEvent_t start = nullptr)
{
	FftInputs in;
	in.fresh[0] = fresh;
	launch_fft_forward(p, hist, in, fmt, split, hist_next, work, out, shifted, st, lay, done, nco, input_read, start);
}
int fold_launch_blocks(const Geometry &g, int remaining, int nb_max);
int launch_fold(const Geometry &g, const float2 *taps, const float2 *spectrum, size_t spec_stride, float2 *partial, size_t partial_stride,
		int nb, hipStream_t st, hipEvent_t start = nullptr, hipEvent_t stop = nullptr);
int fold_variant_count();
int fold_variant_describe(int variant, int desc[6]);
int launch_fold_variant(int variant, const Geometry &g, const float2 *taps, const float2 *spectrum, size_t spec_stride, float2 *partial,
		size_t partial_stride, int nb, hipStream_t st, hipEvent_t start, hipEvent_t stop);
void launch_tap_extract(const float2 *taps, const Geometry &g, int slot, float2 *dst, hipStream_t st);
void launch_tap_row_energy(const float2 *taps, const Geometry &g, float *energy, hipStream_t st);
hipError_t prepare_ifft_nco(int m);
void launch_ifft_nco(const Geometry &g, const float2 *partial, size_t partial_stride, const ChanConst *cc, const NcoState *snap, const float2 *ph,
		size_t ph_stride, const float2 *tw_m, float2 *chan_out, int *out_count, int nb, hipStream_t st, hipEvent_t done = nullptr, hipEvent_t start = nullptr);
void launch_nco_decimate(const float2 *in, int input_size, float cosdelta, float sindelta, float rate, int decimation,
		NcoState *state, float2 *phasor_scratch, float2 *out, hipStream_t st);
#ifdef HFDL_LAB
struct ClockProbeRing { const unsigned long long *records; unsigned *count; unsigned len; };
hipError_t fold_clock_probe_ring(ClockProbeRing &r);
int stream_read_variants();
void launch_stream_read(int variant, const float2 *src, size_t bytes, float *sink, hipStream_t st);
#endif

}
```

Before: 21680.

## Fold channels on the mixed-radix intermediate spectrum and skip FFT pass 3

When the plan fits, the forward FFT stops after pass 2 and writes its output in a mixed-order block layout. The fold kernels consume that layout through new row and group strides. The channel taps are packed into the same permuted, twiddle-free domain, and the NCO phasor table is split across two segments instead of three. This removes the third FFT pass and its full read/write of the spectrum, at the cost of more layout complexity. The spectrum monitor and tap queries now need extra unpack kernels and a pass-3-only FFT.

Measured after the change: 22050, median of 6. +1.7%, better.

```diff
diff --git a/dumphfdl_amd/csrc/fft_core.h b/dumphfdl_amd/csrc/fft_core.h
--- a/dumphfdl_amd/csrc/fft_core.h
+++ b/dumphfdl_amd/csrc/fft_core.h
@@ -103,12 +103,14 @@
 	if (job.seg == 0) job.snap[c] = st;
 	const int cnt = nco_output_count(st, job.post_input_size, job.post);
 	const int per = (job.outs + job.nseg - 1) / job.nseg;
-	const int i0 = job.seg * per, i1 = (job.seg + 1) * per < cnt ? (job.seg + 1) * per : cnt;
+	const int i0 = job.seg * per, i1 = (job.seg + 1) * per < job.outs ? (job.seg + 1) * per : job.outs;
 	float2 p = job.seg == 0 ? nco_phasor_seed(st.starting_phase) : job.cont[c];
 	float2 *dst = job.ph + (size_t)i0 * job.nch + c;
-	for (int i = i0; i < i1; i++, dst += job.nch) {
+	const float cd = k.nco_cosdelta, sd = k.nco_sindelta;
+	const size_t row = (size_t)job.nch;
+	for (int i = i0; i < i1; i++, dst += row) {
 		*dst = p;
-		nco_phasor_step(p.x, p.y, k.nco_cosdelta, k.nco_sindelta);
+		nco_phasor_step(p.x, p.y, cd, sd);
 	}
 	job.cont[c] = p;
 	if (job.seg == job.nseg - 1) {
diff --git a/dumphfdl_amd/csrc/fft_kernels.hip b/dumphfdl_amd/csrc/fft_kernels.hip
--- a/dumphfdl_amd/csrc/fft_kernels.hip
+++ b/dumphfdl_amd/csrc/fft_kernels.hip
@@ -199,16 +199,20 @@
 }
 
 template <int B, bool AHEAD>
-__global__ __launch_bounds__(16 * B) void fft_rpass2(float2 *__restrict__ buf, FftPlan p, NcoJob job, int riders, int tpw)
+__global__ __launch_bounds__(16 * B) void fft_rpass2(float2 *__restrict__ buf, FftPlan p, NcoJob job, int riders, int tpw,
+		float2 *__restrict__ mix_out, int mix_q, int keep, int64_t mix_rx_stride)
 {
 	constexpr int NT = 16 * B;
 	if ((int)blockIdx.x < riders) { if (blockIdx.y == 0) nco_table_segment(job, (int)blockIdx.x * NT + (int)threadIdx.x); return; }
 	buf += (size_t)blockIdx.y * (size_t)p.n;
+	const bool mix = mix_out != nullptr;
+	if (mix) mix_out += blockIdx.y * mix_rx_stride;
 	__shared__ float2 ex[B * FR_PITCH];
 	__shared__ float2 ltw[16 * B];
 	const int bid = ((int)blockIdx.x - riders) * tpw, tid = (int)threadIdx.x;
 	const int r23 = p.n >> p.l1;
 	const int col = tid & 15, n2 = tid >> 4;
+	const int kp = mix ? 1 : 16, cp = mix ? FR_TPITCH : 1;
 	auto base_of = [&](int tile) {
 		const int cc0 = tile * 16;
 		return buf + (size_t)(cc0 >> p.l3) * r23 + (cc0 & (p.r3 - 1));
@@ -227,16 +231,29 @@
 		float2 *base = base_of(tile);
 		const int n30 = (tile * 16) & (p.r3 - 1);
 		__syncthreads();
-		stage_a(x, ex, ltw, n2, col);
+		stage_a(x, ex, ltw, n2, col, kp, cp);
 		__syncthreads();
 #pragma unroll
 		for (int i = 0; i < 256 / NT; i++) {
-			const int tt = tid + i * NT, tcol = tt & 15, k1 = tt >> 4, n3 = n30 + tcol;
+			const int tt = tid + i * NT, tlo = tt & 15, thi = tt >> 4;
+			const int tcol = mix ? thi : tlo, k1 = mix ? tlo : thi, n3 = n30 + tcol;
 			float2 z[B], w[B];
-			stage_b<B>(z, ex, k1, tcol);
+			stage_b<B>(z, ex, k1, tcol, kp, cp);
 			twiddle_run<B>(w, (unsigned)k1 * (unsigned)n3, 16u * (unsigned)n3, p.l2 + p.l3);
-#pragma unroll
-			for (int k2 = 0; k2 < B; k2++) base[(size_t)(k1 + 16 * k2) * p.r3 + tcol] = cmul(z[slot_small<B>(k2)], w[k2]);
+			const int K1 = (tile * 16) >> p.l3, qh = mix_q - 4, rows_log = p.l2 - mix_q + p.l3;
+			const unsigned lo = mix ? (1u << qh) - 1u : ~0u, hs = mix ? (unsigned)qh : 31u;
+			const unsigned s_lo = mix ? 1u << (p.l1 + rows_log + 4) : 16u << p.l3, s_hi = mix ? 1u << (p.l3 + 4) : 0u;
+			float2 *here = base + (size_t)k1 * p.r3 + tcol;
+			float2 *dst = mix ? mix_out + ((size_t)K1 << (rows_log + 4)) + (size_t)n3 * 16 + k1 : here;
+#pragma unroll
+			for (int kb = 0; kb < B; kb++) {
+				w[kb] = cmul(z[slot_small<B>(kb)], w[kb]);
+				dst[((unsigned)kb & lo) * s_lo + ((unsigned)kb >> hs) * s_hi] = w[kb];
+			}
+			if (keep) {
+#pragma unroll
+				for (int kb = 0; kb < B; kb++) here[(unsigned)kb * (16u << p.l3)] = w[kb];
+			}
 		}
 		if (AHEAD) {
 #pragma unroll
@@ -310,14 +327,13 @@
 	}
 }
 
-template <int B>
-static void launch_rpass1(int fmt, dim3 grid, hipStream_t st, hipEvent_t start, hipEvent_t input_read, const float2 *hist, const FftInputs &in, int split, float2 *hist_next,
-		float2 *work, const FftPlan &p, const NcoJob &nco, int riders, int tpw)
-{
-	const dim3 blk(16 * B);
-	if (fmt == SFMT_CS16) hipExtLaunchKernelGGL((fft_rpass1<B, SFMT_CS16, false>), grid, blk, 0, st, start, input_read, 0, hist, in, split, hist_next, work, p, nco, riders, tpw);
-	else if (fmt == SFMT_CU8) hipExtLaunchKernelGGL((fft_rpass1<B, SFMT_CU8, false>), grid, blk, 0, st, start, input_read, 0, hist, in, split, hist_next, work, p, nco, riders, tpw);
-	else hipExtLaunchKernelGGL((fft_rpass1<B, SFMT_CF32, false>), grid, blk, 0, st, start, input_read, 0, hist, in, split, hist_next, work, p, nco, riders, tpw);
+static void launch_rpass(const void *kernel, dim3 grid, int logr, hipStream_t st, hipEvent_t start, hipEvent_t stop, void **args)
+{
+	(void)hipExtLaunchKernel(kernel, grid, dim3(1u << logr), args, 0, st, start, stop, 0);
+}
+template <int B> static const void *rpass1_of(int fmt)
+{
+	return fmt == SFMT_CS16 ? (const void *)fft_rpass1<B, SFMT_CS16, false> : fmt == SFMT_CU8 ? (const void *)fft_rpass1<B, SFMT_CU8, false> : (const void *)fft_rpass1<B, SFMT_CF32, false>;
 }
 
 __global__ void retune_channelizer_kernel(ChanConst *cc, NcoState *chain, float2 *cont, int c, ChanConst k)
@@ -335,8 +351,35 @@
 
 static bool fast_plan(const FftPlan &p) { return p.l1 >= 6 && p.l1 <= 8 && p.l2 >= 6 && p.l2 <= 8 && p.l3 >= 6 && p.l3 <= 8; }
 
+__global__ __launch_bounds__(256) void mixed_copy_kernel(float2 *__restrict__ plain, float *__restrict__ taps, const float2 *__restrict__ block,
+		int dir, int l1, int l2, int l3, int q, int m, size_t rs_f, int slot)
+{
+	const size_t n = (size_t)1 << (l1 + l2 + l3);
+	for (size_t e = (size_t)blockIdx.x * 256 + threadIdx.x; e < n; e += (size_t)gridDim.x * 256) {
+		const int ka = (int)(e & 15), n3 = (int)(e >> 4) & ((1 << l3) - 1), kb = (int)(e >> (4 + l3)) & ((1 << (l2 - 4)) - 1), k1 = (int)(e >> (l2 + l3));
+		const int k2 = ka + 16 * kb, jp = mixed_bin(natural_bin_of(k1, k2, q, l1), l1);
+		float2 *pl = plain + ((size_t)k1 << (l2 + l3)) + ((size_t)k2 << l3) + n3;
+		if (dir == 2) {
+			*pl = block[((size_t)(jp >> 4) << (l2 - q + l3 + 4)) + (size_t)mixed_row(k2, n3, q, l3) * 16 + (jp & 15)];
+			continue;
+		}
+		float *t = taps + tap_index_f(TAPL_OCTET, m, rs_f, slot, mixed_tap_row(k2, n3, q, l3), jp, 0);
+		const float r3 = (float)(1 << l3), ir3 = 1.0f / r3;
+		if (dir == 0) { const float2 v = *pl; t[0] = v.x * r3; t[4] = v.y * r3; }
+		else *pl = make_float2(t[0] * ir3, t[4] * ir3);
+	}
+}
+
+static void launch_mixed_copy(const FftPlan &p, const Geometry &g, float2 *plain, float *taps, const float2 *block, int dir, int slot, hipStream_t st)
+{
+	hipLaunchKernelGGL(mixed_copy_kernel, dim3(2048), dim3(256), 0, st, plain, taps, block, dir, p.l1, p.l2, p.l3, g.mix_q, g.m, (size_t)g.tap_row_stride * 2, slot);
+}
+void launch_mixed_tap_pack(const FftPlan &p, const Geometry &g, const float2 *plain, float2 *taps, int slot, hipStream_t st) { launch_mixed_copy(p, g, (float2 *)plain, (float *)taps, nullptr, 0, slot, st); }
+void launch_mixed_tap_unpack(const FftPlan &p, const Geometry &g, const float2 *taps, int slot, float2 *plain, hipStream_t st) { launch_mixed_copy(p, g, plain, (float *)taps, nullptr, 1, slot, st); }
+void launch_mixed_block_unpack(const FftPlan &p, const Geometry &g, const float2 *slot, float2 *plain, hipStream_t st) { launch_mixed_copy(p, g, plain, nullptr, slot, 2, 0, st); }
+
 void launch_fft_forward(const FftPlan &p, const float2 *hist, const FftInputs &in, int fmt, int split, float2 *hist_next,
-		float2 *work, float2 *out, bool shifted, hipStream_t st, FftOutLayout lay, hipEvent_t done, NcoJob nco, hipEvent_t input_read, hipEvent_t start)
+		float2 *work, float2 *out, bool shifted, hipStream_t st, FftOutLayout lay, hipEvent_t done, NcoJob nco, hipEvent_t input_read, hipEvent_t start, FftVariant var)
 {
 	const unsigned nrx = (unsigned)in.nrx;
 	const int64_t ors = in.out_stride;
@@ -344,27 +387,32 @@
 	const int g1 = (c1 + FFT_TILE - 1) / FFT_TILE, g2 = (c2 + FFT_TILE - 1) / FFT_TILE, g3 = (c3 + FFT_TILE - 1) / FFT_TILE;
 	nco.nseg = 3;
 	if (fast_plan(p)) {
+		const bool mix = var.mix_out != nullptr, run1 = var.passes & 1, run2 = var.passes & 2, run3 = var.passes & 4;
+		if (mix) nco.nseg = 2;
 		auto riders_of = [&](int l) { const int nt = 1 << l; return nco.cc ? (nco.nch + nt - 1) / nt : 0; };
-		const int rd1 = riders_of(p.l1), rd2 = riders_of(p.l2), rd3 = riders_of(p.l3);
+		const int rd1 = riders_of(p.l1), rd2 = riders_of(p.l2), rd3 = mix ? 0 : riders_of(p.l3);
 		auto tpw_of = [](int tiles) { return tiles % 4 == 0 && tiles >= 4096 ? 4 : tiles % 2 == 0 && tiles >= 1024 ? 2 : 1; };
-		const int t1 = 1, t2 = 1, t3 = tpw_of(g3);
+		const int t3 = tpw_of(g3);
+		FftPlan plan = p;
+		FftInputs inputs = in;
+		int tpw = 1, shift = shifted ? 1 : 0, keep = mix && run3 ? 1 : 0;
+		int64_t out_stride = ors;
 		nco.seg = 0;
-		switch (p.l1) {
-		case 6: launch_rpass1<4>(fmt, dim3(g1 / t1 + rd1, nrx), st, start, input_read, hist, in, split, hist_next, work, p, nco, rd1, t1); break;
-		case 7: launch_rpass1<8>(fmt, dim3(g1 / t1 + rd1, nrx), st, start, input_read, hist, in, split, hist_next, work, p, nco, rd1, t1); break;
-		default: launch_rpass1<16>(fmt, dim3(g1 / t1 + rd1, nrx), st, start, input_read, hist, in, split, hist_next, work, p, nco, rd1, t1); break;
+		if (run1) {
+			void *args[] = { &hist, &inputs, &split, &hist_next, &work, &plan, &nco, (void *)&rd1, &tpw };
+			launch_rpass(p.l1 == 6 ? rpass1_of<4>(fmt) : p.l1 == 7 ? rpass1_of<8>(fmt) : rpass1_of<16>(fmt), dim3(g1 + rd1, nrx), p.l1, st, start, input_read, args);
 		}
 		nco.seg = 1;
-		switch (p.l2) {
-		case 6: hipLaunchKernelGGL((fft_rpass2<4, false>), dim3(g2 / t2 + rd2, nrx), dim3(64), 0, st, work, p, nco, rd2, t2); break;
-		case 7: hipLaunchKernelGGL((fft_rpass2<8, false>), dim3(g2 / t2 + rd2, nrx), dim3(128), 0, st, work, p, nco, rd2, t2); break;
-		default: hipLaunchKernelGGL((fft_rpass2<16, false>), dim3(g2 / t2 + rd2, nrx), dim3(256), 0, st, work, p, nco, rd2, t2); break;
+		if (run2) {
+			void *args[] = { &work, &plan, &nco, (void *)&rd2, &tpw, &var.mix_out, &var.mix_q, &keep, &var.mix_rx_stride };
+			launch_rpass(p.l2 == 6 ? (const void *)fft_rpass2<4, false> : p.l2 == 7 ? (const void *)fft_rpass2<8, false> : (const void *)fft_rpass2<16, false>,
+					dim3(g2 + rd2, nrx), p.l2, st, nullptr, mix || !run3 ? done : nullptr, args);
 		}
 		nco.seg = 2;
-		switch (p.l3) {
-		case 6: hipExtLaunchKernelGGL(fft_rpass3<4>, dim3(g3 / t3 + rd3, nrx), dim3(64), 0, st, nullptr, done, 0, (const float2 *)work, out, p, shifted ? 1 : 0, lay, nco, rd3, t3, ors); break;
-		case 7: hipExtLaunchKernelGGL(fft_rpass3<8>, dim3(g3 / t3 + rd3, nrx), dim3(128), 0, st, nullptr, done, 0, (const float2 *)work, out, p, shifted ? 1 : 0, lay, nco, rd3, t3, ors); break;
-		default: hipExtLaunchKernelGGL(fft_rpass3<16>, dim3(g3 / t3 + rd3, nrx), dim3(256), 0, st, nullptr, done, 0, (const float2 *)work, out, p, shifted ? 1 : 0, lay, nco, rd3, t3, ors); break;
+		if (run3) {
+			void *args[] = { &work, &out, &plan, &shift, &lay, &nco, (void *)&rd3, (void *)&t3, &out_stride };
+			launch_rpass(p.l3 == 6 ? (const void *)fft_rpass3<4> : p.l3 == 7 ? (const void *)fft_rpass3<8> : (const void *)fft_rpass3<16>,
+					dim3(g3 / t3 + rd3, nrx), p.l3, st, nullptr, mix ? nullptr : done, args);
 		}
 		return;
 	}
diff --git a/dumphfdl_amd/csrc/fft_regs.h b/dumphfdl_amd/csrc/fft_regs.h
--- a/dumphfdl_amd/csrc/fft_regs.h
+++ b/dumphfdl_amd/csrc/fft_regs.h
@@ -49,18 +49,19 @@
 }
 template <int B> __device__ __forceinline__ constexpr int slot_small(int k) { return B == 16 ? slot16(k) : B == 8 ? slot8(k) : k; }
 
-__device__ __forceinline__ void stage_a(float2 (&x)[16], float2 *ex, const float2 *ltw, int n2, int col)
+constexpr int FR_TPITCH = 17;
+__device__ __forceinline__ void stage_a(float2 (&x)[16], float2 *ex, const float2 *ltw, int n2, int col, int kp = 16, int cp = 1)
 {
 	dft16(x);
-	float2 *dst = ex + n2 * FR_PITCH + col;
+	float2 *dst = ex + n2 * FR_PITCH + col * cp;
 	dst[0] = x[0];
 #pragma unroll
-	for (int k1 = 1; k1 < 16; k1++) dst[k1 * 16] = cmul(x[slot16(k1)], ltw[n2 * k1]);
+	for (int k1 = 1; k1 < 16; k1++) dst[k1 * kp] = cmul(x[slot16(k1)], ltw[n2 * k1]);
 }
 
-template <int B> __device__ __forceinline__ void stage_b(float2 (&z)[B], const float2 *ex, int k1, int col)
+template <int B> __device__ __forceinline__ void stage_b(float2 (&z)[B], const float2 *ex, int k1, int col, int kp = 16, int cp = 1)
 {
-	const float2 *src = ex + k1 * 16 + col;
+	const float2 *src = ex + k1 * kp + col * cp;
 #pragma unroll
 	for (int n2 = 0; n2 < B; n2++) z[n2] = src[n2 * FR_PITCH];
 	dft_small<B>(z);
diff --git a/dumphfdl_amd/csrc/fold_domain.h b/dumphfdl_amd/csrc/fold_domain.h
--- /dev/null
+++ b/dumphfdl_amd/csrc/fold_domain.h
@@ -0,0 +1,34 @@
+#pragma once
+#include <stdint.h>
+
+#if defined(__HIPCC__)
+#define HFDL_FOLD_HD __host__ __device__
+#else
+#define HFDL_FOLD_HD
+#endif
+
+namespace hfdl {
+
+HFDL_FOLD_HD inline int mixed_bin(int j, int l1)
+{
+	if (l1 == 0) return j;
+	const int mask = (1 << (l1 + 4)) - 1, f = j & mask;
+	return (j & ~mask) | ((f & ((1 << l1) - 1)) << 4) | (f >> l1);
+}
+HFDL_FOLD_HD inline int natural_bin(int jp, int l1)
+{
+	if (l1 == 0) return jp;
+	const int mask = (1 << (l1 + 4)) - 1, f = jp & mask;
+	return (jp & ~mask) | ((f & 15) << l1) | (f >> 4);
+}
+HFDL_FOLD_HD inline int mixed_row(int k2, int n3, int q, int l3) { return ((k2 >> q) << l3) | n3; }
+HFDL_FOLD_HD inline int natural_bin_of(int k1, int k2, int q, int l1) { return k1 | ((k2 & ((1 << q) - 1)) << l1); }
+HFDL_FOLD_HD inline int mixed_tap_row(int k2, int n3, int q, int l3) { return mixed_row(k2, (-n3) & ((1 << l3) - 1), q, l3); }
+
+HFDL_FOLD_HD inline bool mixed_fold_fits(int l1, int l2, int l3, int logm, bool pruned)
+{
+	const bool fast = l1 >= 6 && l1 <= 8 && l2 >= 6 && l2 <= 8 && l3 >= 6 && l3 <= 8;
+	return fast && logm - l1 >= 4 && logm <= l1 + l2 && !pruned;
+}
+
+}
diff --git a/dumphfdl_amd/csrc/fold_kernels.hip b/dumphfdl_amd/csrc/fold_kernels.hip
--- a/dumphfdl_amd/csrc/fold_kernels.hip
+++ b/dumphfdl_amd/csrc/fold_kernels.hip
@@ -32,7 +32,7 @@
 
 __global__ __launch_bounds__(FOLD_THREADS) void fold_ref_kernel(const float *__restrict__ taps, const float2 *__restrict__ spec, float2 *__restrict__ partial,
 		size_t row_stride_f, size_t spec_stride, size_t partial_stride, int m, int slices, int rows, int layout, int nb,
-		const int4 *__restrict__ rx_tab, int nrx, size_t spec_rx_stride)
+		const int4 *__restrict__ rx_tab, int nrx, size_t spec_rx_stride, size_t row_stride, size_t group_stride)
 {
 	const int s = blockIdx.x % slices, c = blockIdx.x / slices;
 	const int rxi = rx_of_channel(rx_tab, nrx, c);
@@ -41,7 +41,7 @@
 	spec += (size_t)rxi * spec_rx_stride;
 	for (int b0 = 0; b0 < nb; b0 += 4)
 		for (int j = threadIdx.x; j < m; j += FOLD_THREADS) {
-			const float2 *sp = spec + (size_t)b0 * spec_stride + (size_t)s * rows * (size_t)m + j;
+			const float2 *sp = spec + (size_t)b0 * spec_stride + (size_t)s * rows * row_stride + (size_t)(j >> 4) * group_stride + (j & 15);
 			float2 acc[4] = { make_float2(0.f, 0.f), make_float2(0.f, 0.f), make_float2(0.f, 0.f), make_float2(0.f, 0.f) };
 			for (int r = 0; r < rows; r += 4) {
 				const int n = rows - r < 4 ? rows - r : 4;
@@ -50,7 +50,7 @@
 #pragma unroll
 				for (int b = 0; b < 4; b++)
 					if (b0 + b < nb) {
-						for (int k = 0; k < n; k++) x[k] = sp[(size_t)b * spec_stride + (size_t)(r + k) * m];
+						for (int k = 0; k < n; k++) x[k] = sp[(size_t)b * spec_stride + (size_t)(r + k) * row_stride];
 						cmac_quad(acc[b], h, x, n);
 					}
 			}
@@ -84,7 +84,7 @@
 __device__ __forceinline__ void fold_mfma16_body(
 		const float *__restrict__ taps, const float2 *__restrict__ spec, float2 *__restrict__ partial,
 		size_t row_stride_f, size_t spec_stride, size_t partial_stride, int m, int slices, int rows, int nb,
-		const int2 *__restrict__ win, const int4 *__restrict__ grp_tab, size_t spec_rx_stride)
+		const int2 *__restrict__ win, const int4 *__restrict__ grp_tab, size_t spec_rx_stride, size_t row_stride, size_t group_stride)
 {
 	static_assert(!WIN || W == 1, "windows are per wave: no spectrum tile is shared");
 	static_assert(D == 2 || D == 4, "the LDS stage of a trip is a compile-time constant for even D");
@@ -125,7 +125,7 @@
 		trips = __builtin_amdgcn_readfirstlane(wn.y);
 	}
 	const char *tb = (const char *)(taps + (size_t)s * rows * row_stride_f + (size_t)octet0 * 64 * m + (size_t)g * 1024) + lane * 16;
-	const size_t qs_b = row_stride_f * 16, os_b = (size_t)m * 256, xquad_b = (size_t)m * 32;
+	const size_t qs_b = row_stride_f * 16, os_b = (size_t)m * 256, xquad_b = row_stride * 32;
 	const char *xp[MINE], *xp0[MINE];
 	int xseg[MINE];
 #pragma unroll
@@ -133,7 +133,7 @@
 		const int item = (((wave * MINE) % NLOADS) + i) * 64 + lane, seg = item >> 3, part = item & 7;
 		const int sn = (seg & 15) + 16 * (seg >> 6), sk = (seg >> 4) & 3;
 		const int bi = sn < nb ? sn : nb - 1;
-		xp[i] = xp0[i] = (const char *)(spec + (size_t)bi * spec_stride + ((size_t)s * rows + sk) * (size_t)m + g * 16 + 2 * part);
+		xp[i] = xp0[i] = (const char *)(spec + (size_t)bi * spec_stride + ((size_t)s * rows + sk) * row_stride + (size_t)g * group_stride + 2 * part);
 		xseg[i] = part * XPITCH + seg;
 	}
 	const char *const tb0 = tb;
@@ -295,18 +295,18 @@
 __global__ __launch_bounds__(64 * W) __attribute__((amdgpu_waves_per_eu(fold16_waves(P, W, D, SMALL, CG), fold16_waves(P, W, D, SMALL, CG)))) void fold_mfma16_kernel(
 		const float *__restrict__ taps, const float2 *__restrict__ spec, float2 *__restrict__ partial,
 		size_t row_stride_f, size_t spec_stride, size_t partial_stride, int m, int slices, int rows, int nb,
-		const int2 *__restrict__ win, const int4 *__restrict__ grp_tab, size_t spec_rx_stride)
-{
-	fold_mfma16_body<P, W, D, WIN, SMALL, CG>(taps, spec, partial, row_stride_f, spec_stride, partial_stride, m, slices, rows, nb, win, grp_tab, spec_rx_stride);
+		const int2 *__restrict__ win, const int4 *__restrict__ grp_tab, size_t spec_rx_stride, size_t row_stride, size_t group_stride)
+{
+	fold_mfma16_body<P, W, D, WIN, SMALL, CG>(taps, spec, partial, row_stride_f, spec_stride, partial_stride, m, slices, rows, nb, win, grp_tab, spec_rx_stride, row_stride, group_stride);
 }
 
 #ifdef HFDL_LAB
 __global__ __launch_bounds__(512) __attribute__((amdgpu_waves_per_eu(2, 2))) __attribute__((amdgpu_num_vgpr(104))) void fold32_two_waves_kernel(
 		const float *__restrict__ taps, const float2 *__restrict__ spec, float2 *__restrict__ partial,
 		size_t row_stride_f, size_t spec_stride, size_t partial_stride, int m, int slices, int rows, int nb,
-		const int2 *__restrict__ win, const int4 *__restrict__ grp_tab, size_t spec_rx_stride)
-{
-	fold_mfma16_body<1, 8, 2, false, false, 2>(taps, spec, partial, row_stride_f, spec_stride, partial_stride, m, slices, rows, nb, win, grp_tab, spec_rx_stride);
+		const int2 *__restrict__ win, const int4 *__restrict__ grp_tab, size_t spec_rx_stride, size_t row_stride, size_t group_stride)
+{
+	fold_mfma16_body<1, 8, 2, false, false, 2>(taps, spec, partial, row_stride_f, spec_stride, partial_stride, m, slices, rows, nb, win, grp_tab, spec_rx_stride, row_stride, group_stride);
 }
 #endif
 
@@ -359,6 +359,7 @@
 	const int4 *grp_tab, *rx_host;
 	int nrx;
 	size_t spec_rx_stride;
+	size_t row_stride, group_stride;
 	void split(int pw, int &groups, int &rest) const
 	{
 		groups = rest = 0;
@@ -368,6 +369,12 @@
 	hipStream_t st;
 	hipEvent_t start, stop;
 };
+
+static void fold_launch(const void *kernel, unsigned blocks, unsigned threads, FoldArgs a, int slices, const int2 *win, const int4 *table, hipEvent_t start, hipEvent_t stop)
+{
+	void *args[] = { &a.taps, &a.spec, &a.partial, &a.rs_f, &a.ss, &a.ps, &a.m, &slices, &a.rows, &a.nb, &win, &table, &a.spec_rx_stride, &a.row_stride, &a.group_stride };
+	(void)hipExtLaunchKernel(kernel, dim3(blocks), dim3(threads), args, 0, a.st, start, stop, 0);
+}
 
 template <int P, int W, int D, bool SMALL = false, int CG = 1>
 static int fold16_go(const FoldArgs &a)
@@ -378,14 +385,12 @@
 	a.split(P * W, groups, rest);
 	int launches = 0;
 	if (groups > 0) {
-		hipExtLaunchKernelGGL((fold_mfma16_kernel<P, W, D, false, SMALL, CG>), dim3((unsigned)(groups * ntile)), dim3(64 * W), 0, a.st, a.start, rest ? nullptr : a.stop, 0,
-			a.taps, a.spec, a.partial, a.rs_f, a.ss, a.ps, a.m, a.slices, a.rows, a.nb, (const int2 *)nullptr, a.table(P * W), a.spec_rx_stride);
+		fold_launch((const void *)fold_mfma16_kernel<P, W, D, false, SMALL, CG>, (unsigned)(groups * ntile), 64 * W, a, a.slices, (const int2 *)nullptr, a.table(P * W), a.start, rest ? nullptr : a.stop);
 		launches++;
 	}
 	if (rest > 0) {
 		constexpr int DR = CG > 1 ? 2 : D;
-		hipExtLaunchKernelGGL((fold_mfma16_kernel<1, 1, DR, false, SMALL, CG>), dim3((unsigned)(rest * ntile)), dim3(64), 0, a.st, groups > 0 ? nullptr : a.start, a.stop, 0,
-			a.taps, a.spec, a.partial, a.rs_f, a.ss, a.ps, a.m, a.slices, a.rows, a.nb, (const int2 *)nullptr, a.table(P * W) + groups, a.spec_rx_stride);
+		fold_launch((const void *)fold_mfma16_kernel<1, 1, DR, false, SMALL, CG>, (unsigned)(rest * ntile), 64, a, a.slices, (const int2 *)nullptr, a.table(P * W) + groups, groups > 0 ? nullptr : a.start, a.stop);
 		launches++;
 	}
 	return launches;
@@ -399,13 +404,11 @@
 	a.split(8, groups, rest);
 	int launches = 0;
 	if (groups > 0) {
-		hipExtLaunchKernelGGL(fold32_two_waves_kernel, dim3((unsigned)(groups * ntile)), dim3(512), 0, a.st, a.start, rest ? nullptr : a.stop, 0,
-			a.taps, a.spec, a.partial, a.rs_f, a.ss, a.ps, a.m, a.slices, a.rows, a.nb, (const int2 *)nullptr, a.table(8), a.spec_rx_stride);
+		fold_launch((const void *)fold32_two_waves_kernel, (unsigned)(groups * ntile), 512, a, a.slices, (const int2 *)nullptr, a.table(8), a.start, rest ? nullptr : a.stop);
 		launches++;
 	}
 	if (rest > 0) {
-		hipExtLaunchKernelGGL((fold_mfma16_kernel<1, 1, 2, false, false, 2>), dim3((unsigned)(rest * ntile)), dim3(64), 0, a.st, groups > 0 ? nullptr : a.start, a.stop, 0,
-			a.taps, a.spec, a.partial, a.rs_f, a.ss, a.ps, a.m, a.slices, a.rows, a.nb, (const int2 *)nullptr, a.table(8) + groups, a.spec_rx_stride);
+		fold_launch((const void *)fold_mfma16_kernel<1, 1, 2, false, false, 2>, (unsigned)(rest * ntile), 64, a, a.slices, (const int2 *)nullptr, a.table(8) + groups, groups > 0 ? nullptr : a.start, a.stop);
 		launches++;
 	}
 	return launches;
@@ -416,8 +419,7 @@
 static int fold16_go_win(const FoldArgs &a, const int2 *win)
 {
 	const int ntile = a.m >> 4;
-	hipExtLaunchKernelGGL((fold_mfma16_kernel<1, 1, D, true>), dim3((unsigned)(a.ngroups * ntile)), dim3(64), 0, a.st, a.start, a.stop, 0,
-		a.taps, a.spec, a.partial, a.rs_f, a.ss, a.ps, a.m, 1, a.rows, a.nb, win, a.table(1), a.spec_rx_stride);
+	fold_launch((const void *)fold_mfma16_kernel<1, 1, D, true>, (unsigned)(a.ngroups * ntile), 64, a, 1, win, a.table(1), a.start, a.stop);
 	return 1;
 }
 
@@ -476,6 +478,8 @@
 	return take;
 }
 
+static size_t fold_row_stride(const Geometry &g) { return g.spec_row_stride ? (size_t)g.spec_row_stride : (size_t)g.m; }
+
 static FoldArgs fold_args(const Geometry &g, const float2 *taps, const float2 *spectrum, size_t spec_stride, float2 *partial, size_t partial_stride,
 		int nb, hipStream_t st, hipEvent_t start, hipEvent_t stop)
 {
@@ -484,6 +488,7 @@
 	a.rs_f = (size_t)g.tap_row_stride * 2; a.ss = spec_stride; a.ps = partial_stride;
 	a.m = g.m; a.slices = g.slices; a.rows = g.rows_per_slice; a.nch = g.nch; a.ngroups = g.nch_pad / tap_layout_group(g.tap_layout); a.nb = nb;
 	a.grp_tab = g.grp_tab; a.rx_host = g.rx_host; a.nrx = g.nrx; a.spec_rx_stride = (size_t)g.spec_rx_stride;
+	a.row_stride = fold_row_stride(g); a.group_stride = (size_t)g.spec_group_stride;
 	a.st = st; a.start = start; a.stop = stop;
 	return a;
 }
@@ -493,7 +498,7 @@
 {
 	hipExtLaunchKernelGGL(fold_ref_kernel, dim3((unsigned)(g.nch * g.slices)), dim3(FOLD_THREADS), 0, st, start, stop, 0,
 		(const float *)taps, spectrum, partial, (size_t)g.tap_row_stride * 2, spec_stride, partial_stride, g.m, g.slices, g.rows_per_slice, g.tap_layout, nb,
-		g.rx_tab, g.nrx, (size_t)g.spec_rx_stride);
+		g.rx_tab, g.nrx, (size_t)g.spec_rx_stride, fold_row_stride(g), (size_t)g.spec_group_stride);
 }
 
 int launch_fold_variant(int v, const Geometry &g, const float2 *taps, const float2 *spectrum, size_t spec_stride, float2 *partial,
@@ -580,9 +585,10 @@
 		const float2 *pc = partial + (size_t)b * partial_stride + (size_t)c * g.slices * (size_t)m;
 		for (int u = threadIdx.x; u < m; u += IFFT_THREADS) {
 			const int j = (u - h0 - m / 2) & mask;
+			const int jp = mixed_bin(j, g.mix_l1);
 			float2 acc = make_float2(0.f, 0.f);
 			for (int s = 0; s < g.slices; s++) {
-				float2 v = pc[(size_t)s * m + j];
+				float2 v = pc[(size_t)s * m + jp];
 				acc.x += v.x; acc.y += v.y;
 			}
 			sm[u] = acc;
diff --git a/dumphfdl_amd/csrc/frontend.h b/dumphfdl_amd/csrc/frontend.h
--- a/dumphfdl_amd/csrc/frontend.h
+++ b/dumphfdl_amd/csrc/frontend.h
@@ -76,6 +76,7 @@
 	DevBuf acc;
 	DevBuf peak;
 	PinnedBuf<float> host;
+	DevBuf scratch;
 	Event ev;
 	hipEvent_t last = nullptr;
 	hipEvent_t newest() const { return last ? last : ev.e; }
diff --git a/dumphfdl_amd/csrc/frontend_create.cpp b/dumphfdl_amd/csrc/frontend_create.cpp
--- a/dumphfdl_amd/csrc/frontend_create.cpp
+++ b/dumphfdl_amd/csrc/frontend_create.cpp
@@ -146,7 +146,12 @@
 		FftOutLayout lay = fe->tap_layout;
 		lay.chan = slot;
 		float2 *dst = lay.kind == TAPL_PLAIN ? fe->d_taps + (size_t)slot * (size_t)fe->geo.tap_chan_stride : fe->d_taps;
-		launch_fft_forward(fe->fft.p, nullptr, d_pad, SFMT_CF32, 0, nullptr, fe->d_work, dst, true, fe->stream, lay);
+		if (fe->geo.mix_l1) {
+			FftVariant v;
+			v.passes = FFT_PASSES_12;
+			launch_fft_forward(fe->fft.p, nullptr, d_pad, SFMT_CF32, 0, nullptr, fe->d_work, nullptr, true, fe->stream, FftOutLayout(), nullptr, NcoJob(), nullptr, nullptr, v);
+			launch_mixed_tap_pack(fe->fft.p, fe->geo, fe->d_work, fe->d_taps, slot, fe->stream);
+		} else launch_fft_forward(fe->fft.p, nullptr, d_pad, SFMT_CF32, 0, nullptr, fe->d_work, dst, true, fe->stream, lay);
 	}
 	HIP_TRY(hipStreamSynchronize(fe->stream));
 	HIP_TRY(hipGetLastError());
@@ -262,6 +267,13 @@
 	CREATE_TRY(fe->fft_done.own.create(EV_NO_TIMING));
 	CREATE_TRY(fe->ev_switch.create(EV_NO_TIMING));
 	if (int rc = fe->fft.build(pl.n)) return rc;
+	{
+		const FftPlan &fp = fe->fft.p;
+		if (g.tap_layout == TAPL_OCTET && mixed_fold_fits(fp.l1, fp.l2, fp.l3, ilog2(pl.m), fe->prune_tol > 0) && env_long("HFDL_GPU_FOLD_SPECTRUM", 0, 1, 1) == 0) {
+			g.mix_l1 = fp.l1; g.mix_q = ilog2(pl.m) - fp.l1;
+			g.spec_row_stride = 16; g.spec_group_stride = 16 * (int64_t)pl.pre;
+		}
+	}
 	const size_t n = (size_t)pl.n;
 	const size_t K = (size_t)nrx;
 	for (int i = 0; i < 2; i++) {
diff --git a/dumphfdl_amd/csrc/frontend_query.cpp b/dumphfdl_amd/csrc/frontend_query.cpp
--- a/dumphfdl_amd/csrc/frontend_query.cpp
+++ b/dumphfdl_amd/csrc/frontend_query.cpp
@@ -252,12 +252,20 @@
 	case HFDL_GPU_TAP_SPECTRUM:
 		src = fe->spec_slot(fe->last_set, index) + (fe->nrx > 1 ? (size_t)fe->rx_of[(size_t)channel] * (size_t)g.n : 0);
 		nf = 2 * (size_t)g.n;
-		break;
+		if (!g.mix_l1) break;
+		[[fallthrough]];
 	case HFDL_GPU_TAP_FILTER: {
 		if (2 * (size_t)g.n > cap) return fail(HFDL_GPU_ERANGE, "tap needs %zu floats, buffer holds %zu", 2 * (size_t)g.n, cap);
-		DevBuf plain;
+		DevBuf plain, mid;
 		HIP_TRY(plain.alloc(sizeof(float2) * (size_t)g.n));
-		launch_tap_extract(fe->d_taps, g, fe->slot_of(channel), plain.as<float2>(), fe->stream);
+		if (g.mix_l1) {
+			HIP_TRY(mid.alloc(sizeof(float2) * (size_t)g.n));
+			if (what == HFDL_GPU_TAP_SPECTRUM) launch_mixed_block_unpack(fe->fft.p, g, (const float2 *)src, mid.as<float2>(), fe->stream);
+			else launch_mixed_tap_unpack(fe->fft.p, g, fe->d_taps, fe->slot_of(channel), mid.as<float2>(), fe->stream);
+			FftVariant v;
+			v.passes = FFT_PASS_3;
+			launch_fft_forward(fe->fft.p, nullptr, (const void *)nullptr, SFMT_CF32, 0, nullptr, mid.as<float2>(), plain.as<float2>(), true, fe->stream, FftOutLayout(), nullptr, NcoJob(), nullptr, nullptr, v);
+		} else launch_tap_extract(fe->d_taps, g, fe->slot_of(channel), plain.as<float2>(), fe->stream);
 		HIP_TRY(hipStreamSynchronize(fe->stream));
 		HIP_TRY(hipMemcpy(dst, plain.p, sizeof(float2) * (size_t)g.n, hipMemcpyDeviceToHost));
 		*n_floats = 2 * (size_t)g.n;
@@ -311,6 +319,7 @@
 	hipError_t e = mon->acc.alloc(sizeof(float2) * nb * K);
 	if (e == hipSuccess && (flags & HFDL_GPU_SPECTRUM_MAXHOLD)) e = mon->peak.alloc(sizeof(float) * nb * K);
 	if (e == hipSuccess) e = mon->host.alloc(3 * nb);
+	if (e == hipSuccess && fe->geo.mix_l1) e = mon->scratch.alloc(sizeof(float2) * K * (size_t)fe->geo.n);
 	if (e == hipSuccess) e = mon->ev.create(EV_NO_TIMING);
 	if (e != hipSuccess) return fail(e == hipErrorOutOfMemory ? HFDL_GPU_ENOMEM : HFDL_GPU_EHIP, "spectrum monitor buffers: %s", hipGetErrorString(e));
 	mon->bins = bins;
diff --git a/dumphfdl_amd/csrc/hfdl_gpu.cpp b/dumphfdl_amd/csrc/hfdl_gpu.cpp
--- a/dumphfdl_amd/csrc/hfdl_gpu.cpp
+++ b/dumphfdl_amd/csrc/hfdl_gpu.cpp
@@ -252,13 +252,21 @@
 		b->blocks++;
 	}
 	in.nrx = fe->nrx; in.hist_stride = g.overlap; in.out_stride = g.n;
-	launch_fft_forward(fe->fft.p, fe->d_hist[fe->blocks & 1], in, fmt, g.overlap, fe->d_hist[(fe->blocks + 1) & 1], fe->d_work, fe->spec_slot(set, i), true, st,
+	SpectrumMonitor *mon = fe->mon.get();
+	FftVariant var;
+	float2 *spectrum = fe->spec_slot(set, i);
+	if (g.mix_l1) {
+		var.mix_out = spectrum; var.mix_q = g.mix_q; var.mix_rx_stride = g.n;
+		var.passes = mon ? FFT_PASSES_ALL : FFT_PASSES_12;
+		spectrum = mon ? mon->scratch.as<float2>() : nullptr;
+	}
+	launch_fft_forward(fe->fft.p, fe->d_hist[fe->blocks & 1], in, fmt, g.overlap, fe->d_hist[(fe->blocks + 1) & 1], fe->d_work, spectrum, true, st,
 			FftOutLayout(), fft_done, job,
 			stage_idx >= 0 ? fe->ev_stage_free[stage_idx].e : nullptr,
-			fft_start);
-	if (SpectrumMonitor *mon = fe->mon.get()) {
+			fft_start, var);
+	if (mon) {
 		SpecmonJob m;
-		m.spec = fe->spec_slot(set, i); m.rx_stride = g.n; m.n = g.n; m.bins = mon->bins; m.nrx = fe->nrx; m.flags = mon->flags;
+		m.spec = spectrum; m.rx_stride = g.n; m.n = g.n; m.bins = mon->bins; m.nrx = fe->nrx; m.flags = mon->flags;
 		m.scale = (float)(1.0 / ((double)g.n * (double)g.n * ((mon->flags & SPECMON_HANN) ? 0.375 : 1.0)));
 		m.fresh = mon->fresh; m.acc = mon->acc.as<float2>(); m.peak = mon->peak.as<float>();
 		SpectrumHistory *h = mon->hist.get();
@@ -447,7 +455,12 @@
 	FftOutLayout lay = fe->tap_layout;
 	lay.chan = slot;
 	float2 *dst = lay.kind == TAPL_PLAIN ? fe->d_taps + (size_t)slot * (size_t)fe->geo.tap_chan_stride : fe->d_taps;
-	launch_fft_forward(fe->fft.p, nullptr, r.pad.p, SFMT_CF32, 0, nullptr, r.work.as<float2>(), dst, true, fe->stream, lay, nullptr, NcoJob(), r.staged[sb]);
+	if (fe->geo.mix_l1) {
+		FftVariant v;
+		v.passes = FFT_PASSES_12;
+		launch_fft_forward(fe->fft.p, nullptr, r.pad.p, SFMT_CF32, 0, nullptr, r.work.as<float2>(), nullptr, true, fe->stream, FftOutLayout(), nullptr, NcoJob(), r.staged[sb], nullptr, v);
+		launch_mixed_tap_pack(fe->fft.p, fe->geo, r.work.as<float2>(), fe->d_taps, slot, fe->stream);
+	} else launch_fft_forward(fe->fft.p, nullptr, r.pad.p, SFMT_CF32, 0, nullptr, r.work.as<float2>(), dst, true, fe->stream, lay, nullptr, NcoJob(), r.staged[sb]);
 	launch_retune_channelizer(fe->d_cc, fe->d_nco, fe->d_ph_cont, channel, k, fe->stream, r.done.signal());
 	fe->demod.enqueue_retune(channel, new_freq_hz, fe->stream_b, fe->stream_d);
 	if (Notch *n = fe->notch.get()) HIP_TRY(hipMemsetAsync(n->state.as<float>() + (size_t)channel * NOTCH_STATE_FLOATS, 0, sizeof(float) * NOTCH_STATE_FLOATS, fe->stream_b));
diff --git a/dumphfdl_amd/csrc/kernels.h b/dumphfdl_amd/csrc/kernels.h
--- a/dumphfdl_amd/csrc/kernels.h
+++ b/dumphfdl_amd/csrc/kernels.h
@@ -1,6 +1,7 @@
 #pragma once
 #include <hip/hip_runtime.h>
 #include <stdint.h>
+#include "fold_domain.h"
 
 namespace hfdl {
 
@@ -40,6 +41,8 @@
 	int32_t nrx = 1;
 	int64_t spec_rx_stride = 0;
 	const int4 *grp_tab = nullptr;
+	int32_t mix_l1 = 0, mix_q = 0;
+	int64_t spec_row_stride = 0, spec_group_stride = 16;
 };
 constexpr int FOLD_GROUP_MAX = 16;
 
@@ -86,17 +89,22 @@
 
 enum { SFMT_CF32 = 0, SFMT_CS16 = 1, SFMT_CU8 = 2 };
 struct FftOutLayout { int row_log = 0; int64_t row_stride = 0; int kind = 0; int chan = 0; };
+enum { FFT_PASSES_ALL = 7, FFT_PASSES_12 = 3, FFT_PASS_3 = 4 };
+struct FftVariant { int passes = FFT_PASSES_ALL; float2 *mix_out = nullptr; int mix_q = 0; int64_t mix_rx_stride = 0; };
 void launch_fft_forward(const FftPlan &p, const float2 *hist, const FftInputs &in, int fmt, int split, float2 *hist_next,
 		float2 *work, float2 *out, bool shifted, hipStream_t st, FftOutLayout lay = FftOutLayout(), hipEvent_t done = nullptr,
-		NcoJob nco = NcoJob(), hipEvent_t input_read = nullptr, hipEvent_t start = nullptr);
+		NcoJob nco = NcoJob(), hipEvent_t input_read = nullptr, hipEvent_t start = nullptr, FftVariant var = FftVariant());
 inline void launch_fft_forward(const FftPlan &p, const float2 *hist, const void *fresh, int fmt, int split, float2 *hist_next,
 		float2 *work, float2 *out, bool shifted, hipStream_t st, FftOutLayout lay = FftOutLayout(), hipEvent_t done = nullptr,
-		NcoJob nco = NcoJob(), hipEvent_t input_read = nullptr, hipEvent_t start = nullptr)
+		NcoJob nco = NcoJob(), hipEvent_t input_read = nullptr, hipEvent_t start = nullptr, FftVariant var = FftVariant())
 {
 	FftInputs in;
 	in.fresh[0] = fresh;
-	launch_fft_forward(p, hist, in, fmt, split, hist_next, work, out, shifted, st, lay, done, nco, input_read, start);
+	launch_fft_forward(p, hist, in, fmt, split, hist_next, work, out, shifted, st, lay, done, nco, input_read, start, var);
 }
+void launch_mixed_tap_pack(const FftPlan &p, const Geometry &g, const float2 *plain, float2 *taps, int slot, hipStream_t st);
+void launch_mixed_tap_unpack(const FftPlan &p, const Geometry &g, const float2 *taps, int slot, float2 *plain, hipStream_t st);
+void launch_mixed_block_unpack(const FftPlan &p, const Geometry &g, const float2 *slot, float2 *plain, hipStream_t st);
 int fold_launch_blocks(const Geometry &g, int remaining, int nb_max);
 int launch_fold(const Geometry &g, const float2 *taps, const float2 *spectrum, size_t spec_stride, float2 *partial, size_t partial_stride,
 		int nb, hipStream_t st, hipEvent_t start = nullptr, hipEvent_t stop = nullptr);
```
